# alisher-turubayev/dl-normalizing-flows

Hardware: AMD Instinct MI355X
Metric: images/sec + bits/dim, RealNVP 64x64x3 training (higher is better)
Workload: dtype bf16; 1 GPU; config 1: RealNVP 64x64x3, res-blocks 4, base-dim 32, per-GPU batch 64, train step fwd+bwd+Adam; global_batch=64, image_size=64, res_blocks=4, base_dim=32, n_scales=5, parallelism=dp1, graph=True, side_stream=False

## Files before the change

dl-normalizing-flows_amd/csrc/conv.hip:

```cpp
#include <math.h>
#include <stdlib.h>

#include "common.h"
#include "conv_common.h"

#ifndef RNVP_SHARD_PX
#define RNVP_SHARD_PX 8192
#endif
extern "C" int rnvp_stat_shards(long long M) {
    long long s = M / RNVP_SHARD_PX;
    int r = 1;
    while (r < 32 && r * 2 <= s) r *= 2;
    return r;
}

namespace {

int conv_args_status(const rnvp_conv_args* a) {
    if (!a || !a->x || !a->w || !a->y) return RNVP_E_INVALID;
    if (a->variant < 0 || (a->variant > RNVP_VARIANT_DEEP && a->variant < RNVP_VARIANT_DEEP0) ||
        a->variant >= RNVP_VARIANT_DEEP0 + RNVP_DEEP_CFGS)
        return RNVP_E_INVALID;
    if (a->w_frag && !al16(a->w_frag)) return RNVP_E_INVALID;
    if (a->dtype != RNVP_F32 && a->dtype != RNVP_BF16) return RNVP_E_INVALID;
    if (a->ks != 1 && a->ks != 3) return RNVP_E_UNSUPPORTED;
    if (a->B < 0 || a->H <= 0 || a->W <= 0 || a->n <= 0 || a->cin <= 0) return RNVP_E_INVALID;
    if ((a->cs_in & 7) || (a->cs_out & 7) || a->cs_in < a->cin || a->cs_out < a->n) return RNVP_E_INVALID;
    if ((a->kp & 63) || a->kp < a->ks * a->ks * a->cs_in) return RNVP_E_INVALID;
    if (!al16(a->x) || !al16(a->w)) return RNVP_E_INVALID;
    if (a->epi_relu_bn_bwd && !a->epi_x) return RNVP_E_INVALID;
    auto tab_bad = [](const rnvp_bn_src& s) { return s.tab && (!s.sums || !al16(s.tab)); };
    if ((a->pro_bn_relu && tab_bad(a->pro)) || (a->epi_relu_bn_bwd && tab_bad(a->epi)) || (a->bp && tab_bad(a->bp_bn)))
        return RNVP_E_INVALID;
    if ((long long)a->B * a->H * a->W >= (1ll << 31)) return RNVP_E_UNSUPPORTED;
    if (a->bp) {
        if (!a->bp_x || !al16(a->bp_x) || (a->bp_out && !al16(a->bp_out))) return RNVP_E_INVALID;
        if (a->bp_bn.sums && (!a->bp_sums || a->bp_shards < 1 || a->bp_bn.count <= 0)) return RNVP_E_INVALID;
        if (!a->bp_bn.sums && (!a->bp_bn.mean || !a->bp_bn.var)) return RNVP_E_INVALID;
        if (a->pro_bn_relu) return RNVP_E_INVALID;
    }
    return RNVP_OK;
}

int bp_cfg_of(const rnvp_conv_args* a) {
    if (a->variant >= RNVP_VARIANT_DEEP0) {
        const int cfg = a->variant - RNVP_VARIANT_DEEP0;
        return (cfg == 0 || cfg == 4) ? cfg : -1;
    }
    if (a->variant != 0 && a->variant != RNVP_VARIANT_DEEP) return -1;
    const int cfg = rnvp_deep_auto_cfg(a);
    const long long M = (long long)a->B * a->H * a->W;
    if (cfg == 4 || (cfg == 0 && (a->ks == 3 || M <= 4096))) return cfg;
    return -1;
}

int dispatch_conv(const rnvp_conv_args* a, hipStream_t s, bool dry, int* fam) {
    auto ran = [&](int f, int r) {
        if (fam && r == RNVP_OK) *fam = f;
        return r;
    };
    if (a->variant >= RNVP_VARIANT_DEEP0)
        return ran(RNVP_FAMILY_DEEP, rnvp_deep_launch(a, s, a->variant - RNVP_VARIANT_DEEP0, dry));
    if (a->variant == 0 || a->variant == RNVP_VARIANT_DEEP) {
        const int cfg = rnvp_deep_auto_cfg(a);
        if (cfg >= 0) {
            const int r = rnvp_deep_launch(a, s, cfg, dry);
            if (r != RNVP_E_UNSUPPORTED) return ran(RNVP_FAMILY_DEEP, r);
        }
    }
    const bool tuned = a->variant != 1;
    if (tuned && a->dtype == RNVP_BF16 && a->ks == 1) {
        const int r = rnvp_conv_s1_launch(a, s, dry);
        if (r != RNVP_E_UNSUPPORTED) return ran(RNVP_FAMILY_S1, r);
    }
    if (tuned && rnvp_conv_band_ok(a)) {
        const int r = rnvp_conv_band2_launch(a, s, dry);
        if (r != RNVP_E_UNSUPPORTED) return ran(RNVP_FAMILY_BAND, r);
        if (dry) return ran(RNVP_FAMILY_OTHER, RNVP_OK);
        return rnvp_conv_band1_launch(a, s);
    }
    if (dry) return ran(RNVP_FAMILY_OTHER, RNVP_OK);
    {
        const int r = rnvp_conv_stream_launch(a, s);
        if (r != RNVP_E_UNSUPPORTED) return r;
    }
    if (tuned) {
        const int r = rnvp_conv_halo_launch(a, s);
        if (r != RNVP_E_UNSUPPORTED) return r;
    }
    return rnvp_conv_tiled_launch(a, s);
}

int route_conv(const rnvp_conv_args* a, hipStream_t s, bool dry, int* fam = nullptr) {
    if (a->bp) {
        const int cfg = bp_cfg_of(a);
        int r, f = RNVP_FAMILY_DEEP;
        if (cfg >= 0) {
            r = rnvp_deep_launch(a, s, cfg, dry);
        } else {
            if (a->variant != 0) return RNVP_E_UNSUPPORTED;
            f = RNVP_FAMILY_S1;
            r = rnvp_conv_s1_launch(a, s, dry);
            if (r == RNVP_E_UNSUPPORTED) {
                f = RNVP_FAMILY_BAND;
                r = rnvp_conv_band2_launch(a, s, dry);
            }
        }
        if (fam && r == RNVP_OK) *fam = f;
        return r;
    }
    return dispatch_conv(a, s, dry, fam);
}

}

extern "C" int rnvp_conv2d(const rnvp_conv_args* a, void* stream) {
    const int st = conv_args_status(a);
    if (st != RNVP_OK || a->B == 0) return st;
    return route_conv(a, (hipStream_t)stream, false);
}

extern "C" int rnvp_conv2d_family(const rnvp_conv_args* a) {
    const int st = conv_args_status(a);
    if (st != RNVP_OK) return st;
    int fam = RNVP_FAMILY_OTHER;
    const int r = route_conv(a, nullptr, true, &fam);
    return r == RNVP_OK ? fam : r;
}

extern "C" int rnvp_conv2d_check(const rnvp_conv_args* a) {
    const int st = conv_args_status(a);
    if (st != RNVP_OK || a->B == 0) return st;
    return route_conv(a, nullptr, true);
}
```

dl-normalizing-flows_amd/csrc/conv_band1.hip:

```cpp
#include <math.h>
#include <stdlib.h>

#include "common.h"
#include "conv_common.h"

namespace {

template <typename T>
size_t band_lds_bytes(int cs, int n, int W, int ks) {
    constexpr int CH = Mf<T>::CH, KS = 4 * CH, BM = 256;
    const int nc = n <= 16 ? 16 : (n <= 32 ? 32 : 64);
    const int K = ks * ks * cs;
    const int kpl = lds_mfma_pitch(((K + KS - 1) / KS) * KS, CH);
    const int R = BM + 2 * (ks / 2) * (W + 1);
    const int ntmp = cs > nc ? cs : nc;
    return 16 * (size_t)ntmp + 8 * (size_t)cs + 20 * (size_t)nc + 64 * (size_t)nc +
           ((size_t)nc * kpl + (size_t)(R + 1) * lds_mfma_pitch(cs, CH)) * sizeof(T);
}

template <typename T, int NT, int KSZ, bool PRO, int NH>
__global__ __launch_bounds__(256 * NH) void k_conv_band(rnvp_conv_args a, int shards) {
    constexpr int CH = Mf<T>::CH, KS = 4 * CH;
    constexpr int NC = 16 * NT;
    constexpr int TM = 4, BM = 64 * TM;
    constexpr int PAD = KSZ / 2;
    constexpr int SB = 12 / NH;
    constexpr int NTH = 256 * NH, NTW = NT / NH;
    static_assert(NT % NH == 0, "channel tiles split evenly");
    extern __shared__ double dsm[];
    const int tid = threadIdx.x, lane = tid & 63, g = lane >> 4, li = lane & 15;
    const int wid = (tid >> 6) & 3, hf = tid >> 8;
    const int M = a.B * a.H * a.W, W = a.W, H = a.H;
    const int N = a.n, cs = a.cs_in;
    const int K = KSZ * KSZ * cs;
    const int nsteps = (K + KS - 1) / KS;
    const int kpl = lds_mfma_pitch(nsteps * KS, CH);
    const bool epi_bn = a.epi_relu_bn_bwd != 0;
    const int ntmp = cs > NC ? cs : NC;
    const int hal = PAD * (W + 1), R = BM + 2 * hal;
    const int pitch = lds_mfma_pitch(cs, CH);

    double* tmp = dsm;
    float* bnp = (float*)(dsm + 2 * ntmp);
    float* etab = bnp + 2 * cs;
    float* btab = etab + 4 * NC;
    double* red = (double*)(btab + NC);
    T* Wl = (T*)(red + 8 * NC);
    T* zrow = Wl + NC * kpl;
    T* act = zrow + pitch;

    const int nb = gridDim.x, b = blockIdx.x;
    const int q8 = nb / 8, r8 = nb % 8, xcd = b % 8;
    const int m0 = ((xcd < r8 ? xcd * (q8 + 1) : r8 * (q8 + 1) + (xcd - r8) * q8) + b / 8) * BM;

    const T* __restrict__ X = (const T*)a.x;
    const int cpr = cs / CH;
    const int cfix = tid % cpr, rbase = tid / cpr, rstep = NTH / cpr;
    u32x4 sv[SB];
    auto stage_load = [&](int r0) {
#pragma unroll
        for (int u = 0; u < SB; ++u) {
            if (r0 + u * rstep >= R) break;
            const int r = r0 + rbase + u * rstep;
            const int p = m0 - hal + r;
            const bool ok = (r < R) & (p >= 0) & (p < M);
            sv[u] = *(const u32x4*)(X + (ok ? (long long)p * cs + cfix * CH : 0));
        }
    };
    float scv[CH], shv[CH];
    auto stage_store = [&](int r0) {
#pragma unroll
        for (int u = 0; u < SB; ++u) {
            const int r = r0 + rbase + u * rstep;
            if (r >= R) continue;
            const int p = m0 - hal + r;
            u32x4 w = sv[u];
            if (PRO) {
                if constexpr (sizeof(T) == 2) {
                    w = bn_relu_bf16x8(w, scv, shv);
                } else {
                    float f[CH];
                    unpack(w, f, T());
#pragma unroll
                    for (int e = 0; e < CH; ++e) f[e] = fmaxf(f[e] * scv[e] + shv[e], 0.f);
                    w = pack(f, T());
                }
            }
            const uint32_t keep = (p >= 0 && p < M) ? ~0u : 0u;
            *(u32x4*)(act + r * pitch + cfix * CH) = w & u32x4{keep, keep, keep, keep};
        }
    };
    stage_load(0);

    if (PRO) block_bn_table(a.pro, a.cin, 0, cs, bnp, bnp + cs, nullptr, nullptr, tmp);
    if (epi_bn) block_bn_table(a.epi, N, 0, NC, etab, etab + NC, etab + 2 * NC, etab + 3 * NC, tmp);
    {
        const T* Wg = (const T*)a.w;
        const int wcpr = kpl / CH, wtot = NC * wcpr, kv = nsteps * KS;
        const float rw = 1.0f / (float)wcpr;
        for (int q0 = 0; q0 < wtot; q0 += 4 * NTH) {
            u32x4 v[4];
            unsigned okm = 0;
#pragma unroll
            for (int u = 0; u < 4; ++u) {
                const int q = q0 + u * NTH + tid;
                const int r = fdiv_small(q, rw), c = q - r * wcpr;
                const bool ok = (q < wtot) & (r < N) & (c * CH < kv);
                v[u] = *(const u32x4*)(Wg + (ok ? (long long)r * a.kp + c * CH : 0));
                okm |= (unsigned)ok << u;
            }
#pragma unroll
            for (int u = 0; u < 4; ++u) {
                const int q = q0 + u * NTH + tid;
                if (q < wtot) {
                    const int r = fdiv_small(q, rw), c = q - r * wcpr;
                    const uint32_t keep = ((okm >> u) & 1u) ? ~0u : 0u;
                    *(u32x4*)(Wl + r * kpl + c * CH) = v[u] & u32x4{keep, keep, keep, keep};
                }
            }
        }
        for (int n = tid; n < NC; n += NTH) btab[n] = (a.bias && n < N) ? a.bias[n] : 0.f;
        for (int c = tid * CH; c < pitch; c += NTH * CH) *(u32x4*)(zrow + c) = u32x4{0u, 0u, 0u, 0u};
    }
    __syncthreads();
    if (PRO) {
#pragma unroll
        for (int e = 0; e < CH; ++e) {
            scv[e] = bnp[cfix * CH + e];
            shv[e] = bnp[cs + cfix * CH + e];
        }
    }

    stage_store(0);
    for (int r0 = rstep * SB; r0 < R; r0 += rstep * SB) {
        stage_load(r0);
        stage_store(r0);
    }
    __syncthreads();

    int rowoff[TM];
    unsigned tvm[TM];
    const float rW = 1.0f / (float)W, rH = 1.0f / (float)H;
#pragma unroll
    for (int i = 0; i < TM; ++i) {
        const int lp = wid * 64 + i * 16 + li, m = m0 + lp;
        rowoff[i] = (lp + hal) * pitch;
        const int mm = m < M ? m : 0;
        const int row = fdiv_small(mm, rW);
        const int x = mm - row * W, y = row - fdiv_small(row, rH) * H;
        tvm[i] = tap_mask<KSZ>(x, y, W, H, m < M);
    }

    floatx4 acc[TM][NTW];
#pragma unroll
    for (int i = 0; i < TM; ++i)
#pragma unroll
        for (int j = 0; j < NTW; ++j) acc[i][j] = floatx4{0.f, 0.f, 0.f, 0.f};

    int tap = 0, ci = g * CH;
#pragma unroll
    for (int w = 0; w < 4; ++w)
        if (ci >= cs) { ci -= cs; ++tap; }
    const T* wl = Wl + (hf * NTW * 16 + li) * kpl + g * CH;
    for (int st = 0; st < nsteps; ++st) {
        const int ty = tap / KSZ;
        const int toff = ((ty - PAD) * W + (tap - ty * KSZ - PAD)) * pitch + ci;
        const int tsh = tap < KSZ * KSZ ? tap : 31;
        u32x4 wv[NTW], av[TM];
#pragma unroll
        for (int j = 0; j < NTW; ++j) wv[j] = *(const u32x4*)(wl + j * 16 * kpl + st * KS);
#pragma unroll
        for (int i = 0; i < TM; ++i) {
            const bool ok = (tvm[i] >> tsh) & 1u;
            av[i] = *(const u32x4*)(ok ? act + rowoff[i] + toff : zrow);
        }
#pragma unroll
        for (int i = 0; i < TM; ++i)
#pragma unroll
            for (int j = 0; j < NTW; ++j) Mf<T>::step(wv[j], av[i], acc[i][j]);
        ci += KS;
#pragma unroll
        for (int w = 0; w < 4; ++w)
            if (ci >= cs) { ci -= cs; ++tap; }
    }

    const int cso = a.cs_out;
    double s1[NTW][4], s2[NTW][4];
#pragma unroll
    for (int j = 0; j < NTW; ++j)
#pragma unroll
        for (int r = 0; r < 4; ++r) s1[j][r] = s2[j][r] = 0.0;
#pragma unroll
    for (int i = 0; i < TM; ++i) {
        const int m = m0 + wid * 64 + i * 16 + li;
        if (m >= M) continue;
#pragma unroll
        for (int j = 0; j < NTW; ++j) {
            const int n0 = (hf * NTW + j) * 16 + 4 * g;
            if (n0 >= cso) continue;
            epi4<T>(a, (long long)m * cso + n0, acc[i][j], btab + n0, epi_bn, etab + n0, NC, s1[j], s2[j], N - n0);
        }
    }
    const bool want_sums = a.out_sums || (epi_bn && a.epi_sums);
    if (want_sums) {
#pragma unroll
        for (int j = 0; j < NTW; ++j)
#pragma unroll
            for (int r = 0; r < 4; ++r) {
                const double u1 = row_sum16(s1[j][r]), u2 = row_sum16(s2[j][r]);
                const int col = (hf * NTW + j) * 16 + 4 * g + r;
                if (li == 0) {
                    red[(wid * NC + col) * 2] = u1;
                    red[(wid * NC + col) * 2 + 1] = u2;
                }
            }
        __syncthreads();
        double* sums = shard_ptr(epi_bn ? a.epi_sums : a.out_sums, shards, N);
        for (int n = tid; n < N; n += NTH) {
            double t1 = 0.0, t2 = 0.0;
#pragma unroll
            for (int w = 0; w < 4; ++w) {
                t1 += red[(w * NC + n) * 2];
                t2 += red[(w * NC + n) * 2 + 1];
            }
            atomicAdd(&sums[n], t1);
            atomicAdd(&sums[N + n], t2);
        }
    }
}

template <typename T, int NT, int KSZ>
int launch_band(const rnvp_conv_args* a, hipStream_t s) {
    const long long M = (long long)a->B * a->H * a->W;
    const unsigned grid = (unsigned)((M + 255) / 256);
    const size_t shm = band_lds_bytes<T>(a->cs_in, a->n, a->W, KSZ);
    const int sh = rnvp_stat_shards(M);
    if constexpr ((NT == 4 || NT == 2) && KSZ == 3) {
        if (a->pro_bn_relu) k_conv_band<T, NT, KSZ, true, 2><<<grid, 512, shm, s>>>(*a, sh);
        else k_conv_band<T, NT, KSZ, false, 2><<<grid, 512, shm, s>>>(*a, sh);
    } else {
        if (a->pro_bn_relu) k_conv_band<T, NT, KSZ, true, 1><<<grid, 256, shm, s>>>(*a, sh);
        else k_conv_band<T, NT, KSZ, false, 1><<<grid, 256, shm, s>>>(*a, sh);
    }
    RNVP_LAUNCH_CHECK();
    return RNVP_OK;
}

template <typename T>
bool band_ok(const rnvp_conv_args* a) {
    const long long M = (long long)a->B * a->H * a->W;
    if (a->n > 64 || a->cs_in > 64 || a->ks != 3) return false;
    if (256 % (a->cs_in / Mf<T>::CH) != 0) return false;
    if (M < 32768 || M >= (1ll << 21)) return false;
    return band_lds_bytes<T>(a->cs_in, a->n, a->W, a->ks) <= 150 * 1024;
}

template <typename T>
int dispatch_band(const rnvp_conv_args* a, hipStream_t s) {
    if (a->n <= 16) return launch_band<T, 1, 3>(a, s);
    if (a->n <= 32) return launch_band<T, 2, 3>(a, s);
    return launch_band<T, 4, 3>(a, s);
}

}

bool rnvp_conv_band_ok(const rnvp_conv_args* a) {
    return a->dtype == RNVP_F32 ? band_ok<float>(a) : band_ok<bf16_t>(a);
}

int rnvp_conv_band1_launch(const rnvp_conv_args* a, hipStream_t s) {
    if (!rnvp_conv_band_ok(a)) return RNVP_E_UNSUPPORTED;
    return a->dtype == RNVP_F32 ? dispatch_band<float>(a, s) : dispatch_band<bf16_t>(a, s);
}
```

dl-normalizing-flows_amd/csrc/conv_common.h:

```cpp
#pragma once
#include <math.h>

#include "common.h"

namespace {

template <typename T> struct Mf;
template <> struct Mf<bf16_t> {
    static constexpr int CH = 8;
    __device__ static __forceinline__ void step(const u32x4& a, const u32x4& b, floatx4& c) {
        c = __builtin_amdgcn_mfma_f32_16x16x32_bf16(__builtin_bit_cast(bf16x8, a), __builtin_bit_cast(bf16x8, b), c, 0, 0, 0);
    }
};
template <> struct Mf<float> {
    static constexpr int CH = 4;
    __device__ static __forceinline__ void step(const u32x4& a, const u32x4& b, floatx4& c) {
        c = __builtin_amdgcn_mfma_f32_16x16x4f32(__uint_as_float(a.x), __uint_as_float(b.x), c, 0, 0, 0);
        c = __builtin_amdgcn_mfma_f32_16x16x4f32(__uint_as_float(a.y), __uint_as_float(b.y), c, 0, 0, 0);
        c = __builtin_amdgcn_mfma_f32_16x16x4f32(__uint_as_float(a.z), __uint_as_float(b.z), c, 0, 0, 0);
        c = __builtin_amdgcn_mfma_f32_16x16x4f32(__uint_as_float(a.w), __uint_as_float(b.w), c, 0, 0, 0);
    }
};

__device__ __forceinline__ int sw8(int row, int c) { return row * 8 + (c ^ ((row >> 1) & 7)); }

__device__ __forceinline__ double* shard_ptr(double* sums, int shards, int N) {
    return sums ? sums + (long long)(blockIdx.x % shards) * 2 * N : nullptr;
}

template <typename T>
__device__ __forceinline__ void epi4(const rnvp_conv_args& a, long long o, const floatx4& acc, const float* bias,
                                     bool epi_bn, const float* et, int pitch, double* s1, double* s2, int nvalid) {
    float v[4];
#pragma unroll
    for (int r = 0; r < 4; ++r) v[r] = acc[r] + bias[r];
    if (a.residual) {
        float t[4];
        ld4((const T*)a.residual + o, t);
#pragma unroll
        for (int r = 0; r < 4; ++r) v[r] += t[r];
    }
    if (a.accumulate) {
        float t[4];
        ld4((const T*)a.y + o, t);
#pragma unroll
        for (int r = 0; r < 4; ++r) v[r] += t[r];
    }
    if (epi_bn) {
        float xv[4];
        ld4((const T*)a.epi_x + o, xv);
#pragma unroll
        for (int r = 0; r < 4; ++r) {
            if (xv[r] * et[r] + et[pitch + r] <= 0.f) v[r] = 0.f;
            s1[r] += v[r];
            s2[r] += v[r] * (xv[r] - et[2 * pitch + r]) * et[3 * pitch + r];
        }
    } else {
#pragma unroll
        for (int r = 0; r < 4; ++r) {
            s1[r] += v[r];
            s2[r] += (double)v[r] * v[r];
        }
    }
#pragma unroll
    for (int r = 0; r < 4; ++r)
        if (r >= nvalid) v[r] = 0.f;
    st4((T*)a.y + o, v);
}

struct EpiPre {
    float r[4], y[4], x[4];
};

template <typename T>
__device__ __forceinline__ void epi_prefetch(const rnvp_conv_args& a, long long o, bool live, EpiPre& p) {
    const long long oo = live ? o : 0;
    if (a.residual) ld4((const T*)a.residual + oo, p.r);
    if (a.accumulate) ld4((const T*)a.y + oo, p.y);
    if (a.epi_relu_bn_bwd) ld4((const T*)a.epi_x + oo, p.x);
}

template <typename T>
__device__ __forceinline__ void epi4p(const rnvp_conv_args& a, long long o, const floatx4& acc, const float* bias,
                                      bool epi_bn, const float* et, int pitch, double* s1, double* s2, int nvalid,
                                      const EpiPre& p) {
    float v[4];
#pragma unroll
    for (int r = 0; r < 4; ++r) v[r] = acc[r] + bias[r];
    if (a.residual) {
#pragma unroll
        for (int r = 0; r < 4; ++r) v[r] += p.r[r];
    }
    if (a.accumulate) {
#pragma unroll
        for (int r = 0; r < 4; ++r) v[r] += p.y[r];
    }
    if (epi_bn) {
#pragma unroll
        for (int r = 0; r < 4; ++r) {
            if (p.x[r] * et[r] + et[pitch + r] <= 0.f) v[r] = 0.f;
            s1[r] += v[r];
            s2[r] += v[r] * (p.x[r] - et[2 * pitch + r]) * et[3 * pitch + r];
        }
    } else {
#pragma unroll
        for (int r = 0; r < 4; ++r) {
            s1[r] += v[r];
            s2[r] += (double)v[r] * v[r];
        }
    }
#pragma unroll
    for (int r = 0; r < 4; ++r)
        if (r >= nvalid) v[r] = 0.f;
    st4((T*)a.y + o, v);
}

template <int KSZ>
__device__ __forceinline__ unsigned tap_mask(int x, int y, int W, int H, bool valid) {
    static_assert(KSZ == 1 || KSZ == 3, "1x1 / 3x3");
    if constexpr (KSZ == 1) {
        return valid ? 1u : 0u;
    } else {
        const unsigned cb = (x > 0 ? 1u : 0u) | 2u | (x < W - 1 ? 4u : 0u);
        const unsigned mk = (y > 0 ? cb : 0u) | (cb << 3) | (y < H - 1 ? cb << 6 : 0u);
        return valid ? mk : 0u;
    }
}

typedef float f32x2_t __attribute__((ext_vector_type(2)));
typedef short i16x2_t __attribute__((ext_vector_type(2)));
typedef __bf16 bf16x2_t __attribute__((ext_vector_type(2)));
__device__ __forceinline__ u32x4 bn_relu_bf16x8(const u32x4& c, const float* sc, const float* sh) {
    const uint32_t w[4] = {c.x, c.y, c.z, c.w};
    uint32_t o[4];
#pragma unroll
    for (int i = 0; i < 4; ++i) {
        const f32x2_t x = {__uint_as_float(w[i] << 16), __uint_as_float(w[i] & 0xffff0000u)};
        const f32x2_t y = __builtin_elementwise_fma(x, f32x2_t{sc[2 * i], sc[2 * i + 1]}, f32x2_t{sh[2 * i], sh[2 * i + 1]});
        const uint32_t p = __builtin_bit_cast(uint32_t, __builtin_convertvector(y, bf16x2_t));
        o[i] = __builtin_bit_cast(uint32_t, __builtin_elementwise_max(__builtin_bit_cast(i16x2_t, p), i16x2_t{0, 0}));
    }
    return u32x4{o[0], o[1], o[2], o[3]};
}

__host__ __device__ constexpr int lds_mfma_pitch(int elems, int ch) {
    return (elems / ch + ((2 - elems / ch) & 3)) * ch;
}
template <typename T>
__host__ __device__ constexpr int halo_pitch(int cs) { return lds_mfma_pitch(cs, Mf<T>::CH); }


template <int CPT>
struct BnTab {
    double a1[CPT], a2[CPT], b1[CPT], b2[CPT];
    float gam[CPT], bet[CPT];
};

template <int CPT, int NT = 256>
__device__ __forceinline__ void tab_issue(const rnvp_bn_src& s, int C, int c0, int nc, BnTab<CPT>& t) {
#pragma unroll
    for (int j = 0; j < CPT; ++j) {
        const int c = threadIdx.x + NT * j;
        const int cc = (c < nc && c0 + c < C) ? c0 + c : 0;
        if (s.tab) {
            t.a1[j] = *(const double*)(s.tab + (long long)cc * 4);
            t.a2[j] = t.b1[j] = t.b2[j] = 0.0;
        } else if (s.sums) {
            t.a1[j] = s.sums[cc];
            t.a2[j] = s.sums[C + cc];
            if (s.shards > 1) {
                t.b1[j] = s.sums[2 * (long long)C + cc];
                t.b2[j] = s.sums[3 * (long long)C + cc];
            } else {
                t.b1[j] = t.b2[j] = 0.0;
            }
        } else {
            t.a1[j] = s.mean[cc];
            t.a2[j] = s.var[cc];
            t.b1[j] = t.b2[j] = 0.0;
// ... 127 lines not shown
                    if (var < 0) var = 0;
                } else {
                    mn = a.bn.mean[c];
                    var = a.bn.var[c];
                }
                rstd = (float)(1.0 / sqrt(var + (double)a.bn.eps));
                mean = (float)mn;
                coef = gam * rstd;
            }
            const double g1 = gs[c], g2 = gs[cs + c];
            if (a.bn.sums) {
                k1 = (float)(g1 / cnt);
                k2 = (float)(g2 / cnt);
            }
            if (blk == 0) {
                if (a.dbeta) a.dbeta[c] = (float)g1;
                if (a.dgamma) a.dgamma[c] = (float)g2;
            }
        }
        p[5 * c] = coef; p[5 * c + 1] = k1; p[5 * c + 2] = k2; p[5 * c + 3] = mean; p[5 * c + 4] = rstd;
    };
#pragma unroll
    for (int j = 0; j < 2; ++j) {
        const int c = threadIdx.x + j * blockDim.x;
        if (c < cs) entry(c, gpre[j], epre[j]);
    }
    for (int c = threadIdx.x + 2 * blockDim.x; c < cs; c += blockDim.x)
        entry(c, (GAM && c < C) ? a.bn.gamma[c] : 1.f, btab ? bn_tab_load(a.bn.tab, C, c, BN_TAB_DIV) : bn_f32x2{});
    __syncthreads();
    const bool fixed = qs % cpr == 0;
    int c0 = (int)(q0 % cpr) * CH;
    auto apply = [&](long long o, const u32x4& vg, const u32x4& vx, const u32x4& vr, const u32x4& vd) {
        float g[CH], x[CH], d[CH];
        unpack(vg, g, T());
        unpack(vx, x, T());
#pragma unroll
        for (int j = 0; j < CH; ++j) {
            const float* pp = p + 5 * (c0 + j);
            const float xh = (x[j] - pp[3]) * pp[4];
            d[j] = pp[0] * (g[j] - pp[1] - xh * pp[2]);
        }
        if (R) {
            float r[CH];
            unpack(vr, r, T());
#pragma unroll
            for (int j = 0; j < CH; ++j) d[j] += r[j];
        }
        if (a.accumulate) {
            float r[CH];
            unpack(vd, r, T());
#pragma unroll
            for (int j = 0; j < CH; ++j) d[j] += r[j];
        }
        *(u32x4*)(DX + o) = pack(d, T());
    };
    if (q0 < nch) apply(q0 * CH, fg, fx, fr, fd);
    for (long long q = q0 + qs; q < nch; q += qs) {
        const long long o = q * CH;
        if (!fixed) c0 = (int)(q % cpr) * CH;
        const u32x4 vg = *(const u32x4*)(G + o), vx = *(const u32x4*)(X + o);
        const u32x4 vr = R ? *(const u32x4*)(R + o) : vg;
        const u32x4 vd = a.accumulate ? *(const u32x4*)(DX + o) : vg;
        apply(o, vg, vx, vr, vd);
    }
}

template <typename T>
__device__ __forceinline__ void bn_bwd_body(const rnvp_bn_bwd_args& a, double* dsm, int blk, int nblk) {
    if (a.bn.gamma) bn_bwd_run<T, true>(a, dsm, blk, nblk);
    else bn_bwd_run<T, false>(a, dsm, blk, nblk);
}

inline bool al16(const void* p) { return (((uintptr_t)p) & 15) == 0; }

}

int rnvp_conv_tiled_launch(const rnvp_conv_args* a, hipStream_t s);

int rnvp_conv_stream_launch(const rnvp_conv_args* a, hipStream_t s);

int rnvp_conv_halo_launch(const rnvp_conv_args* a, hipStream_t s);

bool rnvp_conv_band_ok(const rnvp_conv_args* a);
int rnvp_conv_band1_launch(const rnvp_conv_args* a, hipStream_t s);

constexpr int RNVP_DEEP_CFGS = 7;
int rnvp_deep_launch(const rnvp_conv_args* a, hipStream_t s, int cfg, bool dry = false);
int rnvp_deep_auto_cfg(const rnvp_conv_args* a);

int rnvp_wgrad_tap_launch(rnvp_wgrad_group* g, hipStream_t s);
int rnvp_wgrad_tap_prepare(rnvp_wgrad_group* g);
int rnvp_wgrad_tap_multi_plan(const rnvp_wgrad_group* groups, int n_groups, int cls, rnvp_wgrad_multi_conv* convs,
                              int conv_cap, int* xcd_start, int* tasks, int task_cap, rnvp_wgrad_multi* m);
int rnvp_wgrad_tap_multi_launch(const rnvp_wgrad_multi* m, hipStream_t s);

int rnvp_conv_s1_launch(const rnvp_conv_args* a, hipStream_t s, bool dry = false);

struct rnvp_group_kargs {
    rnvp_conv_args conv[RNVP_NET_GROUP_MAX];
    int shards[RNVP_NET_GROUP_MAX], tiles[RNVP_NET_GROUP_MAX], xa[RNVP_NET_GROUP_MAX], xb[RNVP_NET_GROUP_MAX];
    int n;
};
rnvp_group_kargs group_kargs(const rnvp_net_step* steps, int n);

using GroupKernel = void (*)(const rnvp_group_kargs);
template <typename T, int CFG> int rnvp_deep_cfg_launch(const rnvp_conv_args* a, hipStream_t s, bool dry);
template <typename T, int CFG> GroupKernel rnvp_deep_cfg_group(int nc, bool fm);
int rnvp_s1_fanout_prepare(rnvp_net_step* steps, int n, int* klass, int* grid, int* lds_bytes);
int rnvp_s1_fanout_launch(const rnvp_group_kargs& g, int klass, int grid, int lds_bytes, hipStream_t s);

int rnvp_conv_band2_launch(const rnvp_conv_args* a, hipStream_t s, bool dry = false);
```

dl-normalizing-flows_amd/csrc/conv_deep.h:

```cpp
#pragma once
#include <stdlib.h>

#include "common.h"
#include "conv_common.h"

namespace {

constexpr int DEEP_BM = 64;

#ifdef RNVP_DEEP_STAMPS
__device__ unsigned long long* g_deep_stamps;
#define DEEP_STAMP(i) \
    do { if (threadIdx.x == 0) g_deep_stamps[blockIdx.x * 8 + (i)] = wall_clock64(); } while (0)
#else
#define DEEP_STAMP(i) do {} while (0)
#endif
constexpr int DEEP_MAX_CS = 1024;

template <typename T>
__host__ __device__ constexpr int deep_pitch(int cs) { return lds_mfma_pitch(cs, Mf<T>::CH); }

template <typename T, int BN, int NW, int WK, int BM = DEEP_BM>
size_t deep_lds_bytes(int cs, int W, int ks, bool bp = false) {
    constexpr int TM = BM / 16, WM = NW / WK;
    constexpr int G = WK > 1 ? TM : WM;
    const int hal = (ks / 2) * (W + 1), R = BM + 2 * hal;
    const size_t head = 4 * (5 * (size_t)BN) + 8 * (2 * (size_t)G * BN) + 4 * (bp ? 3 : 2) * (size_t)cs;
    const size_t zrow = (size_t)deep_pitch<T>(cs) * sizeof(T);
    size_t act = (size_t)R * deep_pitch<T>(cs) * sizeof(T);
    const size_t red = WK > 1 ? (size_t)WK * BM * (BN + 4) * 4 : 0;
    return head + zrow + (act > red ? act : red);
}

template <typename T, int BN, int KSZ, bool PRO, int NW, int WK, int DK, int NC, bool FM = false, int BM = DEEP_BM,
          bool BP = false>
__device__ __forceinline__ void deep_tile(const rnvp_conv_args& a, int shards, int xa, int xb, int vb, int nvb,
                                          char* lds) {
    constexpr int NT = 64 * NW;
    constexpr int CH = Mf<T>::CH, KS = 4 * CH;
    constexpr int TM = BM / 16, TN = BN / 16;
    constexpr int WM = NW / WK;
    constexpr int TMW = TM / WM;
    static_assert(WM * WK == NW && TMW * WM == TM, "wave layout");
    constexpr int PAD = KSZ / 2;
    constexpr int RP = BN + 4;
    constexpr int G = WK > 1 ? TM : WM;
    constexpr int FR = WK > 1 ? (TM * TN) / NW : 1;
    static_assert(WK == 1 || FR * NW == TM * TN, "final tiles");
    constexpr bool TALL = WK > 1 && TM > NW;
    static_assert(!TALL || TM % NW == 0, "row groups per wave");
    constexpr int CPT = (NC * WK * KS + NT - 1) / NT;
    static_assert(!(BP && PRO), "BatchNorm-backward prologue: data gradients only");
    constexpr int NSTEP = KSZ * KSZ * NC;
    const int tid = threadIdx.x, lane = tid & 63, g = lane >> 4, li = lane & 15;
    const int wid = __builtin_amdgcn_readfirstlane(tid >> 6);
    const int wk = wid % WK, wm = wid / WK;
    const int M = a.B * a.H * a.W, W = a.W, H = a.H;
    const int N = a.n, cs = a.cs_in;
    const int gm = (M + BM - 1) / BM;
    const int nb = nvb, b = vb;
    const int q8 = nb / 8, r8 = nb % 8, xcd = b % 8;
    const int t = (xcd < r8 ? xcd * (q8 + 1) : r8 * (q8 + 1) + (xcd - r8) * q8) + b / 8;
    int mt, nt;
    if (xa > 0) {
        const int per = xa * xb, bi = t / per, w = t - bi * per, gmb = gm / xa;
        const int bm = bi % gmb, bn = bi / gmb;
        mt = bm * xa + w % xa;
        nt = bn * xb + w / xa;
    } else if (xa == 0) {
        nt = t / gm;
        mt = t - nt * gm;
    } else {
        const int gn = nvb / gm;
        mt = t / gn;
        nt = t - mt * gn;
    }
    const int m0 = mt * BM, n0 = nt * BN;
    const T* __restrict__ X = (const T*)a.x;
    const T* __restrict__ Wt = (const T*)(FM ? a.w_frag : a.w);
    const bool epi_bn = a.epi_relu_bn_bwd != 0;
    static_assert(BN <= NT, "bias / table loads: one channel per thread");

    const int hal = PAD * (W + 1);
    const int R = BM + 2 * hal;
    const int pitch = deep_pitch<T>(cs);
    float* etab = (float*)lds;
    float* btab = etab + 4 * BN;
    double* sred = (double*)(btab + BN);
    float* bnp = (float*)(sred + G * BN * 2);
    T* zrow = (T*)(bnp + (BP ? 3 : 2) * cs);
    T* act = zrow + pitch;

    constexpr int CPR = NC * WK * 4;
    static_assert(NT % CPR == 0, "fixed chunk column per thread");
    constexpr int RSTEP = NT / CPR;
    constexpr int SBP = KSZ == 1 ? (BM + RSTEP - 1) / RSTEP : (BM + 2 * 17 + RSTEP - 1) / RSTEP;
    constexpr int SBC = NT == 256 ? 8 : 12;
    constexpr int SB = BP ? (SBP < SBC ? SBP : SBC) : 20 * 256 / NT;
    const int cfix = tid % CPR, rbase = tid / CPR;
    u32x4 sv[SB];
    u32x4 sx[BP ? SB : 1];
    const T* __restrict__ XT = (const T*)a.bp_x;
    auto stage_load = [&](int r0) {
#pragma unroll
        for (int u = 0; u < SB; ++u) {
            if (r0 + u * RSTEP >= R) break;
            const int r = r0 + rbase + u * RSTEP;
            const int p = m0 - hal + r;
            const bool ok = (r < R) & (p >= 0) & (p < M);
            const long long o = ok ? (long long)p * cs + cfix * CH : 0;
            sv[u] = *(const u32x4*)(X + o);
            if constexpr (BP) sx[u] = *(const u32x4*)(XT + o);
        }
    };
    float scv[CH], shv[CH];
    float bca[BP ? CH : 1], bcb[BP ? CH : 1], bcc[BP ? CH : 1];
    T* __restrict__ BPO = (T*)a.bp_out;
    const bool bp_store = BP && BPO != nullptr && nt == 0;
    auto stage_store = [&](int r0) {
#pragma unroll
        for (int u = 0; u < SB; ++u) {
            const int r = r0 + rbase + u * RSTEP;
            if (r >= R) continue;
            const int p = m0 - hal + r;
            u32x4 w = sv[u];
            if (PRO) {
                if constexpr (sizeof(T) == 2) {
                    w = bn_relu_bf16x8(w, scv, shv);
                } else {
                    float f[CH];
                    unpack(w, f, T());
#pragma unroll
                    for (int e = 0; e < CH; ++e) f[e] = fmaxf(f[e] * scv[e] + shv[e], 0.f);
                    w = pack(f, T());
                }
            }
            if constexpr (BP) {
                float gv[CH], xv[CH], d[CH];
                unpack(w, gv, T());
                unpack(sx[u], xv, T());
#pragma unroll
                for (int e = 0; e < CH; ++e) d[e] = fmaf(bca[e], gv[e], -fmaf(bcb[e], xv[e], bcc[e]));
                w = pack(d, T());
                if (bp_store && r >= hal && r < hal + BM && p < M)
                    *(u32x4*)(BPO + (long long)p * cs + cfix * CH) = w;
            }
            const uint32_t keep = (p >= 0 && p < M) ? ~0u : 0u;
            *(u32x4*)(act + r * pitch + cfix * CH) = w & u32x4{keep, keep, keep, keep};
        }
    };
    DEEP_STAMP(0);
    constexpr int NE = WK > 1 ? FR : TMW * TN;
    auto elem = [&](int e, int& m, int& col) {
        if constexpr (TALL) {
            m = m0 + (wid + NW * (e / TN)) * 16 + li;
            col = (e % TN) * 16 + 4 * g;
        } else if constexpr (WK > 1) {
            m = m0 + (wid % TM) * 16 + li;
            col = ((wid / TM) * FR + e) * 16 + 4 * g;
        } else {
            m = m0 + (wm * TMW + e / TN) * 16 + li;
            col = (e % TN) * 16 + 4 * g;
        }
    };
    const int cso = a.cs_out;
    BnTab<CPT> ptab;
    BnTab<1> etb;
    if (PRO) tab_issue<CPT, NT>(a.pro, a.cin, 0, cs, ptab);
    BnTab<BP ? CPT : 1> btb, gtb;
    rnvp_bn_src gsrc = {};
    if constexpr (BP) {
        gsrc.sums = a.bp_sums;
        gsrc.count = a.bp_bn.count;
        gsrc.shards = a.bp_shards;
        rnvp_bn_src bsrc = a.bp_bn;
        if (bsrc.tab) bsrc.tab += 2 * BN_TAB_DIV;
        tab_issue<CPT, NT>(bsrc, a.cin, 0, cs, btb);
        tab_issue<CPT, NT>(gsrc, a.cin, 0, cs, gtb);
    }
    if (epi_bn) tab_issue<1, NT>(a.epi, N, n0, BN, etb);
    const float bval = (tid < BN && a.bias && n0 + tid < N) ? a.bias[n0 + tid] : 0.f;
    EpiPre pre[NE];
#pragma unroll
    for (int e = 0; e < NE; ++e) {
        int m, col;
        elem(e, m, col);
        epi_prefetch<T>(a, (long long)m * cso + n0 + col, m < M && n0 + col < cso, pre[e]);
    }
    stage_load(0);
    const T* wrow[TN];
#pragma unroll
    for (int j = 0; j < TN; ++j) {
        if constexpr (FM) {
            static_assert(sizeof(T) == 2 && KS == 32, "fragment-major images are bf16");
            const int nb = (n0 >> 4) + j, nbl = (N + 15) >> 4;
            wrow[j] = Wt + (long long)(nb < nbl ? nb : 0) * (a.kp >> 5) * 512 + (li + 16 * g) * CH;
        } else {
            const int row = n0 + j * 16 + li;
            wrow[j] = Wt + (long long)(row < N ? row : 0) * a.kp + g * CH;
        }
    }
    u32x4 rb[DK][TN];
    auto bload = [&](int st) {
        const int tp = st / NC, ch = st - (st / NC) * NC;
        const int k = tp * cs + (ch * WK + wk) * KS;
#pragma unroll
        for (int j = 0; j < TN; ++j) rb[st % DK][j] = *(const u32x4*)(wrow[j] + (FM ? (k >> 5) * 512 : k));
    };
#pragma unroll
    for (int u = 0; u < DK; ++u)
        if (u < NSTEP) bload(u);
    if (PRO) tab_finish<CPT, NT>(a.pro, a.cin, 0, cs, ptab, bnp, bnp + cs, nullptr, nullptr);
    if constexpr (BP) {
#pragma unroll
        for (int j = 0; j < CPT; ++j) {
            const int c = tid + NT * j;
            if (c >= cs) continue;
            float coef = 0.f, k1 = 0.f, k2 = 0.f, mo = 0.f, ro = 1.f;
            if (c < a.cin) {
                if (a.bp_bn.tab) {
                    const unsigned long long u = (unsigned long long)__double_as_longlong(btb.a1[j]);
                    mo = __uint_as_float((unsigned)u);
                    ro = __uint_as_float((unsigned)(u >> 32));
                    coef = btb.gam[j] * ro;
                } else {
                    double mean, var;
                    if (a.bp_bn.sums) {
                        const double s1 = btb.a1[j] + (a.bp_bn.shards > 1 ? btb.b1[j] : 0.0);
                        const double s2 = btb.a2[j] + (a.bp_bn.shards > 1 ? btb.b2[j] : 0.0);
                        mean = s1 / a.bp_bn.count;
                        var = s2 / a.bp_bn.count - mean * mean;
                        if (var < 0) var = 0;
                    } else {
                        mean = btb.a1[j];
                        var = btb.a2[j];
                    }
                    ro = (float)(1.0 / sqrt(var + (double)a.bp_bn.eps));
                    mo = (float)mean;
                    coef = btb.gam[j] * ro;
                }
                const double g1 = gtb.a1[j] + (a.bp_shards > 1 ? gtb.b1[j] : 0.0);
                const double g2 = gtb.a2[j] + (a.bp_shards > 1 ? gtb.b2[j] : 0.0);
                if (a.bp_bn.sums) {
                    k1 = (float)(g1 / a.bp_bn.count);
                    k2 = (float)(g2 / a.bp_bn.count);
                }
                if (vb == 0) {
                    if (a.bp_dbeta) a.bp_dbeta[c] = (float)g1;
                    if (a.bp_dgamma) a.bp_dgamma[c] = (float)g2;
                }
            }
            const double rk2 = (double)ro * (double)k2;
            bnp[c] = coef;
            bnp[cs + c] = (float)((double)coef * rk2);
            bnp[2 * cs + c] = (float)((double)coef * ((double)k1 - rk2 * (double)mo));
        }
    }
    if (epi_bn) tab_finish<1, NT>(a.epi, N, n0, BN, etb, etab, etab + BN, etab + 2 * BN, etab + 3 * BN);
    if (tid < BN) btab[tid] = bval;
    for (int c = tid * CH; c < pitch; c += NT * CH) *(u32x4*)(zrow + c) = u32x4{0u, 0u, 0u, 0u};
    __syncthreads();
    DEEP_STAMP(1);
    if (PRO) {
#pragma unroll
        for (int e = 0; e < CH; ++e) {
            scv[e] = bnp[cfix * CH + e];
            shv[e] = bnp[cs + cfix * CH + e];
        }
    }
    if constexpr (BP) {
#pragma unroll
        for (int e = 0; e < CH; ++e) {
            bca[e] = bnp[cfix * CH + e];
            bcb[e] = bnp[cs + cfix * CH + e];
            bcc[e] = bnp[2 * cs + cfix * CH + e];
        }
    }

    stage_store(0);
    for (int r0 = RSTEP * SB; r0 < R; r0 += RSTEP * SB) {
        stage_load(r0);
        stage_store(r0);
    }
    __syncthreads();
    DEEP_STAMP(2);

    int rowoff[TMW];
    unsigned tvm[TMW];
    const float rW = 1.0f / (float)W, rH = 1.0f / (float)H;
#pragma unroll
    for (int i = 0; i < TMW; ++i) {
        const int lp = (wm * TMW + i) * 16 + li, m = m0 + lp;
        rowoff[i] = (lp + hal) * pitch + g * CH;
        const int mm = m < M ? m : 0;
        const int row = fdiv_small(mm, rW);
        const int x = mm - row * W, y = row - fdiv_small(row, rH) * H;
        tvm[i] = tap_mask<KSZ>(x, y, W, H, m < M);
    }
    floatx4 acc[TMW][TN];
#pragma unroll
    for (int i = 0; i < TMW; ++i)
#pragma unroll
        for (int j = 0; j < TN; ++j) acc[i][j] = floatx4{0.f, 0.f, 0.f, 0.f};

    constexpr bool DBUF = KSZ == 1 || (NW == 4 ? (BN == 32 || NC <= 4) : (BN == 32 ? NC <= 2 : NC == 1));
    auto aload = [&](int st, u32x4* dst) {
        const int tp = st / NC, ch = st - (st / NC) * NC;
        const int toff = ((tp / KSZ - PAD) * W + (tp % KSZ - PAD)) * pitch + wk * KS + ch * WK * KS;
#pragma unroll
        for (int i = 0; i < TMW; ++i)
            dst[i] = *(const u32x4*)(((tvm[i] >> tp) & 1u) ? act + rowoff[i] + toff : zrow + ch * WK * KS);
    };
    if constexpr (DBUF) {
        u32x4 avb[2][TMW];
        aload(0, avb[0]);
#pragma unroll
        for (int st = 0; st < NSTEP; ++st) {
            if (st + 1 < NSTEP) aload(st + 1, avb[(st + 1) & 1]);
            __builtin_amdgcn_sched_barrier(0);
#pragma unroll
            for (int i = 0; i < TMW; ++i)
#pragma unroll
                for (int j = 0; j < TN; ++j) Mf<T>::step(rb[st % DK][j], avb[st & 1][i], acc[i][j]);
            if (st + DK < NSTEP) bload(st + DK);
            __builtin_amdgcn_sched_barrier(0);
        }
    } else {
#pragma unroll
        for (int st = 0; st < NSTEP; ++st) {
            u32x4 av[TMW];
            aload(st, av);
#pragma unroll
            for (int i = 0; i < TMW; ++i)
#pragma unroll
                for (int j = 0; j < TN; ++j) Mf<T>::step(rb[st % DK][j], av[i], acc[i][j]);
            if (st + DK < NSTEP) bload(st + DK);
        }
    }

    DEEP_STAMP(3);
    const bool want_sums = a.out_sums || (epi_bn && a.epi_sums);
    constexpr int NS = (WK > 1 && !TALL) ? FR : TN;
    double s1[NS][4], s2[NS][4];
#pragma unroll
    for (int f = 0; f < NS; ++f)
#pragma unroll
        for (int r = 0; r < 4; ++r) s1[f][r] = s2[f][r] = 0.0;
    const int grp = TALL ? wid : (WK > 1 ? wid % TM : wm);
    constexpr int GU = TALL ? NW : G;
    if constexpr (WK > 1) {
        float* red = (float*)act;
        __syncthreads();
#pragma unroll
        for (int i = 0; i < TMW; ++i)
#pragma unroll
            for (int j = 0; j < TN; ++j)
                *(floatx4*)&red[(wk * BM + (wm * TMW + i) * 16 + li) * RP + j * 16 + 4 * g] = acc[i][j];
        __syncthreads();
        const int fi = wid % TM;
#pragma unroll
        for (int f = 0; f < FR; ++f) {
            int m, col;
            elem(f, m, col);
            const int n = n0 + col;
            if (m >= M || n >= cso) continue;
            const int ri = TALL ? wid + NW * (f / TN) : fi;
            const int sl = TALL ? f % TN : f;
            floatx4 v = *(const floatx4*)&red[(ri * 16 + li) * RP + col];
#pragma unroll
            for (int w = 1; w < WK; ++w) v += *(const floatx4*)&red[(w * BM + ri * 16 + li) * RP + col];
            epi4p<T>(a, (long long)m * cso + n, v, btab + col, epi_bn, etab + col, BN, s1[sl], s2[sl], N - n, pre[f]);
        }
    } else {
#pragma unroll
        for (int e = 0; e < NE; ++e) {
            int m, col;
            elem(e, m, col);
            const int n = n0 + col;
            if (m >= M || n >= cso) continue;
            epi4p<T>(a, (long long)m * cso + n, acc[e / TN][e % TN], btab + col, epi_bn, etab + col, BN, s1[e % TN],
                     s2[e % TN], N - n, pre[e]);
        }
    }
    DEEP_STAMP(4);
    if (want_sums) {
#pragma unroll
        for (int f = 0; f < NS; ++f)
#pragma unroll
            for (int r = 0; r < 4; ++r) {
                const double u1 = row_sum16(s1[f][r]), u2 = row_sum16(s2[f][r]);
                if (li == 0) {
                    const int cb = ((WK > 1 && !TALL) ? ((wid / TM) * FR + f) : f) * 16 + 4 * g;
                    sred[(grp * BN + cb + r) * 2] = u1;
                    sred[(grp * BN + cb + r) * 2 + 1] = u2;
                }
            }
        __syncthreads();
        double* sums = (epi_bn ? a.epi_sums : a.out_sums) + (long long)(vb % shards) * 2 * N;
        for (int col = tid; col < BN; col += NT) {
            const int n = n0 + col;
            if (n >= N) continue;
            double t1 = 0.0, t2 = 0.0;
#pragma unroll
            for (int q = 0; q < GU; ++q) {
                t1 += sred[(q * BN + col) * 2];
                t2 += sred[(q * BN + col) * 2 + 1];
            }
            atomicAdd(&sums[n], t1);
            atomicAdd(&sums[N + n], t2);
        }
    }
    DEEP_STAMP(5);
}

inline void xcd_blocks(const rnvp_conv_args* a, int gm, int gn, int bn, int esz, int* xa, int* xb, int bm = DEEP_BM) {
    *xa = -1;
    *xb = 1;
    const long long per = (long long)gm * gn / 8;
    const int hal = (a->ks / 2) * (a->W + 1);
    const double act = (double)(bm + 2 * hal) * a->cs_in * esz;
    const double wsl = (double)bn * a->ks * a->ks * a->cs_in * esz;
    double best = 1e300;
    for (int x = 1; x <= gm; ++x) {
        if (gm % x || per % x) continue;
        const long long y = per / x;
        if (y < 1 || gn % y) continue;
        const double bytes = x * act + y * wsl;
        if (bytes < best) { best = bytes; *xa = x; *xb = (int)y; }
    }
}

}
```

dl-normalizing-flows_amd/csrc/conv_deep_launch.h:

```cpp
#pragma once
#include "conv_deep.h"

namespace {

template <typename T, int BN, int KSZ, bool PRO, int NW, int WK, int DK, int NC, bool FM = false, int BM = DEEP_BM,
          bool BP = false>
__global__ __launch_bounds__(64 * NW) void k_conv_deep(rnvp_conv_args a, int shards, int xa, int xb) {
    extern __shared__ __attribute__((aligned(16))) char lds[];
    deep_tile<T, BN, KSZ, PRO, NW, WK, DK, NC, FM, BM, BP>(a, shards, xa, xb, blockIdx.x, gridDim.x, lds);
}

template <int BN, int NW, int WK, int BM>
constexpr bool bp_cfg() { return BN == 32 && WK == NW && BM == DEEP_BM; }

template <typename T, int BN, int NW, int WK, int DK, int NC, int KSZ, int BM = DEEP_BM>
int launch_deep_nc(const rnvp_conv_args* a, hipStream_t s, bool dry) {
    const long long M = (long long)a->B * a->H * a->W;
    const size_t shm = deep_lds_bytes<T, BN, NW, WK, BM>(a->cs_in, a->W, a->ks, a->bp != 0);
    if (shm > 160 * 1024) return RNVP_E_UNSUPPORTED;
    const long long gm = (M + BM - 1) / BM, gn = (a->n + BN - 1) / BN;
    const unsigned grid = (unsigned)(gm * gn);
    const int sh = rnvp_stat_shards(M);
    const dim3 blk(64 * NW);
    int xa, xb;
    xcd_blocks(a, (int)gm, (int)gn, BN, sizeof(T), &xa, &xb, BM);
    if (a->bp) {
        if constexpr (bp_cfg<BN, NW, WK, BM>()) {
            if (dry) return RNVP_OK;
            if constexpr (sizeof(T) == 2 && NC <= 4) {
                if (a->w_frag) {
                    k_conv_deep<T, BN, KSZ, false, NW, WK, DK, NC, true, BM, true><<<grid, blk, shm, s>>>(*a, sh, xa, xb);
                    RNVP_LAUNCH_CHECK();
                    return RNVP_OK;
                }
            }
            k_conv_deep<T, BN, KSZ, false, NW, WK, DK, NC, false, BM, true><<<grid, blk, shm, s>>>(*a, sh, xa, xb);
            RNVP_LAUNCH_CHECK();
            return RNVP_OK;
        } else {
            return RNVP_E_UNSUPPORTED;
        }
    }
    if (dry) return RNVP_OK;
    if constexpr (sizeof(T) == 2 && NC <= 4) {
        if (a->w_frag) {
            if (a->pro_bn_relu) k_conv_deep<T, BN, KSZ, true, NW, WK, DK, NC, true, BM><<<grid, blk, shm, s>>>(*a, sh, xa, xb);
            else k_conv_deep<T, BN, KSZ, false, NW, WK, DK, NC, true, BM><<<grid, blk, shm, s>>>(*a, sh, xa, xb);
            RNVP_LAUNCH_CHECK();
            return RNVP_OK;
        }
    }
    if (a->pro_bn_relu) k_conv_deep<T, BN, KSZ, true, NW, WK, DK, NC, false, BM><<<grid, blk, shm, s>>>(*a, sh, xa, xb);
    else k_conv_deep<T, BN, KSZ, false, NW, WK, DK, NC, false, BM><<<grid, blk, shm, s>>>(*a, sh, xa, xb);
    RNVP_LAUNCH_CHECK();
    return RNVP_OK;
}

template <typename T, int BN, int NW, int WK, int DK>
int launch_deep(const rnvp_conv_args* a, hipStream_t s, bool dry) {
    constexpr int KS = 4 * Mf<T>::CH;
    const long long M = (long long)a->B * a->H * a->W;
    if (M > 65536 || a->n < BN / 2 || a->cs_in % (WK * KS)) return RNVP_E_UNSUPPORTED;
    if (a->pro_bn_relu && a->pro.sums && a->pro.shards > 2) return RNVP_E_UNSUPPORTED;
    if (a->epi_relu_bn_bwd && a->epi.sums && a->epi.shards > 2) return RNVP_E_UNSUPPORTED;
    if (a->cs_in > DEEP_MAX_CS) return RNVP_E_UNSUPPORTED;
    if (a->bp && (a->pro_bn_relu || (a->bp_bn.sums && a->bp_bn.shards > 2) || a->bp_shards > 2)) return RNVP_E_UNSUPPORTED;
    const int nc = a->cs_in / (WK * KS);
    if (a->ks == 1) {
        switch (nc) {
            case 1: return launch_deep_nc<T, BN, NW, WK, DK, 1, 1>(a, s, dry);
            case 2: return launch_deep_nc<T, BN, NW, WK, DK, 2, 1>(a, s, dry);
            case 4: return launch_deep_nc<T, BN, NW, WK, DK, 4, 1>(a, s, dry);
            case 8: return launch_deep_nc<T, BN, NW, WK, DK, 8, 1>(a, s, dry);
            case 16: return launch_deep_nc<T, BN, NW, WK, DK, 16, 1>(a, s, dry);
        }
        return RNVP_E_UNSUPPORTED;
    }
    if constexpr (WK == NW) {
        switch (nc) {
            case 1: return launch_deep_nc<T, BN, NW, WK, DK, 1, 3>(a, s, dry);
            case 2: return launch_deep_nc<T, BN, NW, WK, DK, 2, 3>(a, s, dry);
            case 4: return launch_deep_nc<T, BN, NW, WK, DK, 4, 3>(a, s, dry);
            case 8: return launch_deep_nc<T, BN, NW, WK, DK, 8, 3>(a, s, dry);
        }
    }
    return RNVP_E_UNSUPPORTED;
}

template <typename T, int BN, int NW, int WK, int DK>
int launch_deep_tall(const rnvp_conv_args* a, hipStream_t s, bool dry) {
    constexpr int KS = 4 * Mf<T>::CH;
    if constexpr (sizeof(T) != 2) {
        return RNVP_E_UNSUPPORTED;
    } else {
        const long long M = (long long)a->B * a->H * a->W;
        if (a->ks != 3 || M > 65536 || a->n < BN / 2 || a->cs_in % (WK * KS)) return RNVP_E_UNSUPPORTED;
        if (a->pro_bn_relu && a->pro.sums && a->pro.shards > 2) return RNVP_E_UNSUPPORTED;
        if (a->epi_relu_bn_bwd && a->epi.sums && a->epi.shards > 2) return RNVP_E_UNSUPPORTED;
        switch (a->cs_in / (WK * KS)) {
            case 1: return launch_deep_nc<T, BN, NW, WK, DK, 1, 3, 128>(a, s, dry);
            case 2: return launch_deep_nc<T, BN, NW, WK, DK, 2, 3, 128>(a, s, dry);
            case 4: return launch_deep_nc<T, BN, NW, WK, DK, 4, 3, 128>(a, s, dry);
        }
        return RNVP_E_UNSUPPORTED;
    }
}

template <typename T, int BN, int NW, int WK, int DK, int NC, bool FM = false>
// ... 59 lines not shown
```

dl-normalizing-flows_amd/csrc/coupling.hip:

```cpp
#include "coupling_common.h"

namespace {

__global__ __launch_bounds__(256) void k_in_stats(rnvp_coupling_args a, int TP, int seg) {
    extern __shared__ double red[];
    const Geo g = geo(a);
    const Tile t = tile_of(g, TP);
    const int lane = threadIdx.x & 63;
    const int total = g.Cb * t.tp;
    auto xidx = [&](int e) {
        const int cb = e / t.tp, p = t.p0 + (e - cb * t.tp);
        const int c = (g.kind == 0) ? cb : g.off_base + cb;
        return ((long long)t.b * g.C + c) * g.HW + p;
    };
    float xp[CP_K];
#pragma unroll
    for (int k = 0; k < CP_K; ++k) {
        const int e = k * 256 + threadIdx.x;
        { const float v = a.x[xidx(e < total ? e : 0)]; xp[k] = e < total ? v : 0.f; }
    }
    lds_zero(red, 2 * g.Cb);
    __syncthreads();
    auto body = [&](int e0, float xv) {
        const int e = e0 + threadIdx.x;
// ... 441 lines not shown
#pragma unroll
    for (int k = 0; k < CP_K; ++k) {
        const int e = k * 256 + threadIdx.x;
        const long long idx = eidx(e < total ? e : 0);
        gzp[k] = a.gz[idx];
        up[k] = a.u[idx];
        xp[k] = a.x[idx];
        glp[k] = gl_ld(glo, idx, t.b);
    }
    for (int cb = threadIdx.x; cb < g.Cb; cb += blockDim.x) {
        float fm = 0.f, rstd = 1.f, kA = 0.f, kB = 0.f;
        if (a.coupling_bn) {
            out_bn_stats(a, g, cb, fm, rstd);
            if (a.training) {
                kA = (float)(csum(a.bwd_sums, 3 * g.Cb, cb) / cnt);
                kB = (float)((csum(a.bwd_sums, 3 * g.Cb, g.Cb + cb) + csum(a.bwd_sums, 3 * g.Cb, 2 * g.Cb + cb)) / cnt);
            }
        }
        tab[cb] = fm; tab[g.Cb + cb] = rstd; tab[2 * g.Cb + cb] = kA; tab[3 * g.Cb + cb] = kB;
    }
    tile_copy_in<T>(a.st, t.m0, t.tp, a.cs_st, st);
    for (int e = threadIdx.x; e < t.tp * a.cs_gst; e += blockDim.x) stv(&gs[e], 0.f);
    __syncthreads();
    const float sc = a.scale[0], ss = a.scale_shift[0];
    double gsc = 0.0, gss = 0.0;
    auto body = [&](int e, float gz, float uv, float xv, float glv) {
        const int c = e / t.tp, pl = e - c * t.tp, p = t.p0 + pl;
        const long long idx = ((long long)t.b * g.C + c) * g.HW + p;
        const bool chan_on = g.kind == 1 && c >= g.on_base && c < g.on_base + g.Cb;
        const int cb = g.kind == 0 ? c : c - g.on_base;
        const bool has_bn_chan = g.kind == 0 || chan_on;
        const bool tr = g.kind == 0 ? !ckbd_m(g, p) : chan_on;
        float gu;
        if (!a.coupling_bn || !has_bn_chan) {
            gu = gz;
        } else {
            const float fm = tab[cb], rstd = tab[g.Cb + cb], kA = tab[2 * g.Cb + cb], kB = tab[3 * g.Cb + cb];
            if (!tr) {
                gu = gz;
                if (a.training) gu += rstd * (-kA - (uv - fm) * rstd * kB);
            } else {
                gu = rstd * gz;
                if (a.training) gu = rstd * (gz - kA - (uv - fm) * rstd * kB);
            }
        }
        if (tr) {
            const float r = ldv(&st[pl * a.cs_st + g.Cb + cb]);
            const float th = tanhf(r);
            const float ex = expf(sc * th + ss);
            a.gx[idx] = gu * ex;
            const float glr = gu * xv * ex + glv;
            stv(&gs[pl * a.cs_gst + cb], gu);
            stv(&gs[pl * a.cs_gst + g.Cb + cb], glr * sc * (1.f - th * th));
            gsc += (double)glr * th;
            gss += glr;
        } else {
            a.gx[idx] = gu;
        }
    };
#pragma unroll
    for (int k = 0; k < CP_K; ++k) {
        const int e = k * 256 + threadIdx.x;
        if (e < total) body(e, gzp[k], up[k], xp[k], glp[k]);
    }
    for (int e = CP_K * 256 + threadIdx.x; e < total; e += 256) {
        const long long idx = eidx(e);
        body(e, a.gz[idx], a.u[idx], a.x[idx], gl_ld(glo, idx, t.b));
    }
    const float dsc = (float)block_sum(gsc, redl);
    const float dss = (float)block_sum(gss, redl);
    tile_copy_out<T>(gs, t.m0, t.tp, a.cs_gst, a.gst);
    if (threadIdx.x == 0 && (dsc != 0.f || dss != 0.f)) {
        if (a.gscale_part) {
            double* sp = a.gscale_part + 2 * (blockIdx.x % RNVP_COUPLING_SHARDS);
            atomicAdd(sp, (double)dsc);
            atomicAdd(sp + 1, (double)dss);
        } else {
            atomicAdd(a.g_scale, dsc);
            atomicAdd(a.g_scale_shift, dss);
        }
    }
}

__device__ __forceinline__ void fold_gscale(const rnvp_coupling_args& a) {
    const int l = threadIdx.x;
    double v0 = 0.0, v1 = 0.0;
    if (l < RNVP_COUPLING_SHARDS) {
        v0 = a.gscale_part[2 * l];
        v1 = a.gscale_part[2 * l + 1];
        a.gscale_part[2 * l] = 0.0;
        a.gscale_part[2 * l + 1] = 0.0;
    }
    v0 = wave_sum(v0);
    v1 = wave_sum(v1);
    if (l == 0) {
        *a.g_scale += (float)v0;
        *a.g_scale_shift += (float)v1;
    }
}

template <typename T>
__device__ __forceinline__ void in_bwd_vals(const rnvp_coupling_args& a, const Geo& g, const Tile& t, const T* gh,
                                            const float* tab, int cb, int pl, float v, float& gxa, float& xh) {
    const int p = t.p0 + pl;
    if (g.kind == 0 && !ckbd_m(g, p)) v = 0.f;
    const float xa = v * tab[cb] + tab[g.Cb + cb];
    const float g1 = ldv(&gh[pl * a.cs_gh0 + cb]);
    const float g2 = ldv(&gh[pl * a.cs_gh0 + g.Cb + cb]);
    gxa = (xa > 0.f ? g1 : 0.f) - (xa < 0.f ? g2 : 0.f);
    xh = (v - tab[2 * g.Cb + cb]) * tab[3 * g.Cb + cb];
}

template <typename T>
__global__ __launch_bounds__(256) void k_in_bwd_red(rnvp_coupling_args a, int TP, int seg) {
    extern __shared__ double dsm[];
    const Geo g = geo(a);
    const Tile t = tile_of(g, TP);
    const int lane = threadIdx.x & 63;
    const bool ext = a.in_bwd_ext != nullptr;
    double* red = dsm;
    float* tab = (float*)(dsm + (ext ? 4 : 2) * g.Cb);
    T* gh = (T*)(tab + 4 * ((g.Cb + 3) / 4 * 4));
    const int total = g.Cb * t.tp;
    auto xidx = [&](int e) {
        const int cb = e / t.tp, p = t.p0 + (e - cb * t.tp);
        const int c = (g.kind == 0) ? cb : g.off_base + cb;
        return ((long long)t.b * g.C + c) * g.HW + p;
    };
    float xp[CP_K];
#pragma unroll
    for (int k = 0; k < CP_K; ++k) {
        const int e = k * 256 + threadIdx.x;
        { const float v = a.x[xidx(e < total ? e : 0)]; xp[k] = e < total ? v : 0.f; }
    }
    tile_copy_in<T>(a.gh0, t.m0, t.tp, a.cs_gh0, gh);
    lds_zero(red, (ext ? 4 : 2) * g.Cb);
    if (a.training && a.in_tab) {
        for (int i = threadIdx.x; i < 4 * g.Cb; i += blockDim.x) tab[i] = a.in_tab[i];
    } else {
        in_bn_table(a, g, tab);
    }
    if (blockIdx.x == 0 && a.gscale_part && threadIdx.x < 64) fold_gscale(a);
    __syncthreads();
    auto body = [&](int e0, float xv) {
        const int e = e0 + threadIdx.x;
        const bool ok = e < total;
        const int cb = ok ? e / t.tp : 0, pl = ok ? e - cb * t.tp : 0;
        float gxa = 0.f, xh = 0.f;
        if (ok) in_bwd_vals<T>(a, g, t, gh, tab, cb, pl, xv, gxa, xh);
        const double s1 = seg_red((double)gxa, seg), s2 = seg_red((double)gxa * xh, seg);
        if (ok && (lane & seg_mask(seg)) == 0) {
            atomicAdd(&red[cb], s1);
            atomicAdd(&red[g.Cb + cb], s2);
        }
        if (ext) {
            const bool kept = ok && (g.kind != 0 || ckbd_m(g, t.p0 + pl));
            const double e1 = seg_red(kept ? (double)gxa : 0.0, seg), e2 = seg_red(kept ? (double)gxa * xv : 0.0, seg);
            if (ok && (lane & seg_mask(seg)) == 0) {
                atomicAdd(&red[2 * g.Cb + cb], e1);
                atomicAdd(&red[3 * g.Cb + cb], e2);
            }
        }
    };
#pragma unroll
    for (int k = 0; k < CP_K; ++k)
        if (k * 256 < total) body(k * 256, xp[k]);
    for (int e0 = CP_K * 256; e0 < total; e0 += 256) {
        const int e = e0 + threadIdx.x;
        { const float v = a.x[xidx(e < total ? e : 0)]; body(e0, e < total ? v : 0.f); }
    }
    __syncthreads();
    double* dst = cshard(a.in_bwd_sums, 2 * g.Cb);
    for (int c = threadIdx.x; c < 2 * g.Cb; c += blockDim.x) atomicAdd(&dst[c], red[c]);
    if (ext) {
        double* dx = cshard(a.in_bwd_ext, 2 * g.Cb);
        for (int c = threadIdx.x; c < 2 * g.Cb; c += blockDim.x) atomicAdd(&dx[c], red[2 * g.Cb + c]);
    }
}

template <typename T>
__global__ __launch_bounds__(256) void k_in_bwd_apply(rnvp_coupling_args a, int TP, int seg) {
    extern __shared__ double dsm[];
    const Geo g = geo(a);
    const Tile t = tile_of(g, TP);
    float* tab = (float*)dsm;
    const int tabn = 8 * ((g.Cb + 3) / 4 * 4);
    T* gh = (T*)(tab + tabn);
    const int total = g.Cb * t.tp;
    auto xidx = [&](int e) {
        const int cb = e / t.tp, p = t.p0 + (e - cb * t.tp);
        const int c = (g.kind == 0) ? cb : g.off_base + cb;
        return ((long long)t.b * g.C + c) * g.HW + p;
    };
    float xp[CP_K], gxp[CP_K];
#pragma unroll
    for (int k = 0; k < CP_K; ++k) {
        const int e = k * 256 + threadIdx.x;
        const long long idx = xidx(e < total ? e : 0);
        xp[k] = a.x[idx];
        gxp[k] = a.gx[idx];
    }
    in_bn_table(a, g, tab);
    const double cnt = (double)g.B * g.HW;
    for (int cb = threadIdx.x; cb < g.Cb; cb += blockDim.x) {
        const float gam = a.in_gamma ? a.in_gamma[cb] : 1.f;
        tab[4 * g.Cb + cb] = gam * tab[3 * g.Cb + cb];
        const double s1 = a.in_bwd_sums ? csum(a.in_bwd_sums, 2 * g.Cb, cb) : 0.0;
        const double s2 = a.in_bwd_sums ? csum(a.in_bwd_sums, 2 * g.Cb, g.Cb + cb) : 0.0;
        tab[5 * g.Cb + cb] = a.training ? (float)(s1 / cnt) : 0.f;
        tab[6 * g.Cb + cb] = a.training ? (float)(s2 / cnt) : 0.f;
        if (blockIdx.x == 0) {
            if (a.g_in_beta) a.g_in_beta[cb] = (float)s1;
            if (a.g_in_gamma) a.g_in_gamma[cb] = (float)s2;
        }
    }
    if (blockIdx.x == 0 && a.gscale_part && threadIdx.x < 64) fold_gscale(a);
    tile_copy_in<T>(a.gh0, t.m0, t.tp, a.cs_gh0, gh);
    __syncthreads();
    auto body = [&](int e, float xv, float gxv) {
        const int cb = e / t.tp, pl = e - cb * t.tp, p = t.p0 + pl;
        const int c = (g.kind == 0) ? cb : g.off_base + cb;
        const long long idx = ((long long)t.b * g.C + c) * g.HW + p;
        float gxa, xh;
        in_bwd_vals<T>(a, g, t, gh, tab, cb, pl, xv, gxa, xh);
        float gxm = tab[4 * g.Cb + cb] * (gxa - tab[5 * g.Cb + cb] - xh * tab[6 * g.Cb + cb]);
        if (g.kind == 0 && !ckbd_m(g, p)) gxm = 0.f;
        a.gx[idx] = gxv + gxm;
    };
#pragma unroll
    for (int k = 0; k < CP_K; ++k) {
        const int e = k * 256 + threadIdx.x;
        if (e < total) body(e, xp[k], gxp[k]);
    }
    for (int e = CP_K * 256 + threadIdx.x; e < total; e += 256) {
        const long long idx = xidx(e);
        body(e, a.x[idx], a.gx[idx]);
    }
}

int check(const rnvp_coupling_args* a) {
    if (!a || !a->x || a->B < 0 || a->C <= 0 || a->H <= 0 || a->W <= 0) return RNVP_E_INVALID;
    if (a->kind != 0 && a->kind != 1) return RNVP_E_INVALID;
    if (a->kind == 1 && (a->C & 1)) return RNVP_E_INVALID;
    if (a->dtype != RNVP_F32 && a->dtype != RNVP_BF16) return RNVP_E_INVALID;
    return RNVP_OK;
}

inline int cb_of(const rnvp_coupling_args* a) { return a->kind == 0 ? a->C : a->C / 2; }

struct TileCfg {
    int TP, seg, grid;
};
inline TileCfg tile_cfg(const rnvp_coupling_args* a) {
    const int HW = a->H * a->W;
    const int esz = a->dtype == RNVP_F32 ? 4 : 2;
    int cs = a->cs_h0;
    if (a->cs_st + a->cs_gst > cs) cs = a->cs_st + a->cs_gst;
    if (a->cs_gh0 > cs) cs = a->cs_gh0;
    if (cs < 8) cs = 8;
    TileCfg c;
    c.TP = HW < 256 ? HW : 256;
    while (c.TP > 16 && (long long)c.TP * cs * esz > 32 * 1024) c.TP /= 2;
    while (c.TP > 4 && c.TP % 2 == 0 && (long long)a->B * ((HW + c.TP - 1) / c.TP) < 512) c.TP /= 2;
    int seg = 1;
    while (seg < 64 && c.TP % (2 * seg) == 0 && HW % (2 * seg) == 0) seg *= 2;
    c.seg = seg;
    c.grid = a->B * ((HW + c.TP - 1) / c.TP);
    return c;
}
}

extern "C" int rnvp_coupling_in_fwd(const rnvp_coupling_args* a, void* stream) {
    int st = check(a);
    if (st) return st;
    if (!a->h0 || (a->training && !a->in_sums) || (!a->training && (!a->in_rmean || !a->in_rvar))) return RNVP_E_INVALID;
    const int Cb = cb_of(a);
    if (a->cs_h0 < (a->kind == 0 ? 2 * Cb + 1 : 2 * Cb)) return RNVP_E_INVALID;
    if (a->B == 0) return RNVP_OK;
    hipStream_t s = (hipStream_t)stream;
    const TileCfg tc = tile_cfg(a);
    const int esz = a->dtype == RNVP_F32 ? 4 : 2;
    if (a->training) {
        k_in_stats<<<tc.grid, 256, 16 * Cb, s>>>(*a, tc.TP, tc.seg);
        RNVP_LAUNCH_CHECK();
    }
    const size_t shm = 16 * r4(Cb) + (size_t)tc.TP * a->cs_h0 * esz;
    if (a->dtype == RNVP_F32) k_in_apply<float><<<tc.grid, 256, shm, s>>>(*a, tc.TP, tc.seg);
    else k_in_apply<bf16_t><<<tc.grid, 256, shm, s>>>(*a, tc.TP, tc.seg);
    RNVP_LAUNCH_CHECK();
    return RNVP_OK;
}

extern "C" int rnvp_coupling_in_apply(const rnvp_coupling_args* a, void* stream) {
    int st = check(a);
    if (st) return st;
    if (!a->h0 || (a->training && !a->in_sums) || (!a->training && (!a->in_rmean || !a->in_rvar))) return RNVP_E_INVALID;
    const int Cb = cb_of(a);
    if (a->cs_h0 < (a->kind == 0 ? 2 * Cb + 1 : 2 * Cb)) return RNVP_E_INVALID;
    if (a->B == 0) return RNVP_OK;
// ... 12 lines not shown
    if (st) return st;
    if (!a->st || !a->u || !a->z || !a->ldj_sample || !a->scale || !a->scale_shift) return RNVP_E_INVALID;
    if (a->coupling_bn && ((a->training && !a->out_sums) || (!a->training && (!a->out_rmean || !a->out_rvar))))
        return RNVP_E_INVALID;
    const int Cb = cb_of(a);
    if (a->cs_st < 2 * Cb) return RNVP_E_INVALID;
    if (a->B == 0) return RNVP_OK;
    hipStream_t s = (hipStream_t)stream;
    const TileCfg tc = tile_cfg(a);
    const int esz = a->dtype == RNVP_F32 ? 4 : 2;
    const size_t shm1 = 16 * ((Cb + 1) / 2 * 2) + (size_t)tc.TP * a->cs_st * esz;
    if (a->dtype == RNVP_F32) k_out1<float><<<tc.grid, 256, shm1, s>>>(*a, tc.TP, tc.seg);
    else k_out1<bf16_t><<<tc.grid, 256, shm1, s>>>(*a, tc.TP, tc.seg);
    RNVP_LAUNCH_CHECK();
    long long n = (long long)a->B * a->C * a->H * a->W;
    size_t shm = 3 * Cb * sizeof(float);
    const int nrun = (a->training && a->net_running) ? a->n_net_running : 0;
    if (nrun < 0 || (nrun > 0 && a->net_running_cmax <= 0)) return RNVP_E_INVALID;
    if (nrun > 0 && 16 * (size_t)a->net_running_cmax > shm) shm = 16 * (size_t)a->net_running_cmax;
    const int g2 = rnvp_grid(n, 256, 2048);
    if (a->dtype == RNVP_F32) k_out2<float><<<g2 + nrun, 256, shm, s>>>(*a, g2);
    else k_out2<bf16_t><<<g2 + nrun, 256, shm, s>>>(*a, g2);
    RNVP_LAUNCH_CHECK();
    return RNVP_OK;
}

extern "C" int rnvp_coupling_reverse(const rnvp_coupling_args* a, void* stream) {
    int st = check(a);
    if (st) return st;
    if (!a->st || !a->z || !a->scale || !a->scale_shift) return RNVP_E_INVALID;
    if (a->coupling_bn && (!a->out_rmean || !a->out_rvar)) return RNVP_E_INVALID;
    if (a->cs_st < 2 * cb_of(a)) return RNVP_E_INVALID;
    if (a->B == 0) return RNVP_OK;
    long long n = (long long)a->B * a->C * a->H * a->W;
    hipStream_t s = (hipStream_t)stream;
    if (a->dtype == RNVP_F32) k_reverse<float><<<rnvp_grid(n, 256, 2048), 256, 0, s>>>(*a);
    else k_reverse<bf16_t><<<rnvp_grid(n, 256, 2048), 256, 0, s>>>(*a);
    RNVP_LAUNCH_CHECK();
    return RNVP_OK;
}

extern "C" int rnvp_coupling_reverse_bwd(const rnvp_coupling_args* a, void* stream) {
    int st = check(a);
    if (st) return st;
    if (!a->st || !a->gz || !a->gx || !a->gst || !a->gscale_part || !a->scale || !a->scale_shift) return RNVP_E_INVALID;
    const int Cb = cb_of(a);
    if (a->cs_gst < 2 * Cb || a->cs_st < 2 * Cb) return RNVP_E_INVALID;
    if (a->coupling_bn && (!a->out_rmean || !a->out_rvar)) return RNVP_E_INVALID;
    if (a->B == 0) return RNVP_OK;
    const TileCfg tc = tile_cfg(a);
    const int esz = a->dtype == RNVP_F32 ? 4 : 2;
    const size_t shm = (size_t)tc.TP * (a->cs_st + a->cs_gst) * esz;
    hipStream_t s = (hipStream_t)stream;
    if (a->dtype == RNVP_F32) k_reverse_bwd<float><<<tc.grid, 256, shm, s>>>(*a, tc.TP);
    else k_reverse_bwd<bf16_t><<<tc.grid, 256, shm, s>>>(*a, tc.TP);
    RNVP_LAUNCH_CHECK();
    return RNVP_OK;
}

extern "C" int rnvp_coupling_out_bwd(const rnvp_coupling_args* a, void* stream) {
    int st = check(a);
    if (st) return st;
    if (!a->st || !a->u || !a->gz || !a->gx || !a->gst || !a->g_scale || !a->g_scale_shift) return RNVP_E_INVALID;
    const int Cb = cb_of(a);
    if (a->cs_gst < 2 * Cb || a->cs_st < 2 * Cb) return RNVP_E_INVALID;
    const bool stats = a->coupling_bn && a->training;
    if (stats && (!a->out_sums || !a->bwd_sums)) return RNVP_E_INVALID;
    if (a->coupling_bn && !a->training && (!a->out_rmean || !a->out_rvar)) return RNVP_E_INVALID;
    if (a->B == 0) return RNVP_OK;
    hipStream_t s = (hipStream_t)stream;
    const TileCfg tc = tile_cfg(a);
    const int esz = a->dtype == RNVP_F32 ? 4 : 2;
    if (stats) {
        k_out_bwd_red<<<tc.grid, 256, 24 * Cb + 8 * Cb, s>>>(*a, tc.TP, tc.seg);
        RNVP_LAUNCH_CHECK();
    }
    const size_t shm = 16 * r4(Cb) + (size_t)tc.TP * (a->cs_st + a->cs_gst) * esz;
    if (a->dtype == RNVP_F32) k_out_bwd_apply<float><<<tc.grid, 256, shm, s>>>(*a, tc.TP, tc.seg);
    else k_out_bwd_apply<bf16_t><<<tc.grid, 256, shm, s>>>(*a, tc.TP, tc.seg);
    RNVP_LAUNCH_CHECK();
    return RNVP_OK;
}

extern "C" int rnvp_coupling_in_bwd(const rnvp_coupling_args* a, void* stream) {
    int st = check(a);
    if (st) return st;
    if (!a->gh0 || (!a->gx && !(a->in_bwd_ext && a->training))) return RNVP_E_INVALID;
    if (a->training && (!a->in_sums || !a->in_bwd_sums)) return RNVP_E_INVALID;
    if (!a->training && (!a->in_rmean || !a->in_rvar)) return RNVP_E_INVALID;
    const int Cb = cb_of(a);
    if (a->cs_gh0 < 2 * Cb) return RNVP_E_INVALID;
    if (a->B == 0) return RNVP_OK;
    hipStream_t s = (hipStream_t)stream;
    const TileCfg tc = tile_cfg(a);
    const int esz = a->dtype == RNVP_F32 ? 4 : 2;
    const size_t gsh = (size_t)tc.TP * a->cs_gh0 * esz;
    if (a->training || a->g_in_gamma || a->g_in_beta) {
        if (!a->in_bwd_sums) return RNVP_E_INVALID;
        const size_t shm = (a->in_bwd_ext ? 32 : 16) * Cb + 16 * r4(Cb) + gsh;
        if (a->dtype == RNVP_F32) k_in_bwd_red<float><<<tc.grid, 256, shm, s>>>(*a, tc.TP, tc.seg);
        else k_in_bwd_red<bf16_t><<<tc.grid, 256, shm, s>>>(*a, tc.TP, tc.seg);
        RNVP_LAUNCH_CHECK();
    }
    if (!a->gx) return RNVP_OK;
    const size_t shm = 32 * r4(Cb) + gsh;
    if (a->dtype == RNVP_F32) k_in_bwd_apply<float><<<tc.grid, 256, shm, s>>>(*a, tc.TP, tc.seg);
    else k_in_bwd_apply<bf16_t><<<tc.grid, 256, shm, s>>>(*a, tc.TP, tc.seg);
    RNVP_LAUNCH_CHECK();
    return RNVP_OK;
}
```

dl-normalizing-flows_amd/csrc/coupling_common.h:

```cpp
#pragma once
#include <math.h>

#include "common.h"

namespace {

struct Geo {
    int kind, B, C, H, W, HW, Cb, cfg, on_base, off_base;
};

__device__ __forceinline__ Geo geo(const rnvp_coupling_args& a) {
    Geo g;
    g.kind = a.kind; g.B = a.B; g.C = a.C; g.H = a.H; g.W = a.W; g.HW = a.H * a.W;
    g.cfg = a.mask_config ? 1 : 0;
    if (a.kind == 0) {
        g.Cb = a.C; g.on_base = 0; g.off_base = 0;
    } else {
        g.Cb = a.C / 2;
        g.on_base = g.cfg ? 0 : g.Cb;
        g.off_base = g.cfg ? g.Cb : 0;
    }
    return g;
}

// ... 35 lines not shown
    return v;
}

__device__ __forceinline__ double seg_red(double v, int seg) { return seg >= 16 ? row_sum16(v) : seg_sum(v, seg); }
__device__ __forceinline__ int seg_mask(int seg) { return seg >= 16 ? 15 : seg - 1; }

template <typename T>
__device__ __forceinline__ void tile_copy_in(const void* src, long long m0, int tp, int cs, T* lds) {
    const int n16 = tp * cs * (int)sizeof(T) / 16;
    const u32x4* s = (const u32x4*)((const T*)src + m0 * cs);
    u32x4* d = (u32x4*)lds;
    for (int i = threadIdx.x; i < n16; i += blockDim.x) d[i] = s[i];
}

template <typename T>
__device__ __forceinline__ void tile_copy_out(const T* lds, long long m0, int tp, int cs, void* dst) {
    const int n16 = tp * cs * (int)sizeof(T) / 16;
    const u32x4* s = (const u32x4*)lds;
    u32x4* d = (u32x4*)((T*)dst + m0 * cs);
    for (int i = threadIdx.x; i < n16; i += blockDim.x) d[i] = s[i];
}

template <int R>
struct TileRegs {
    u32x4 v[R];
    int n16;
};
template <typename T, int R>
__device__ __forceinline__ void tile_issue(const void* src, long long m0, int tp, int cs, TileRegs<R>& r) {
    r.n16 = tp * cs * (int)sizeof(T) / 16;
    const u32x4* s = (const u32x4*)((const T*)src + m0 * cs);
#pragma unroll
    for (int k = 0; k < R; ++k) {
        const int i = (int)threadIdx.x + k * (int)blockDim.x;
        r.v[k] = s[i < r.n16 ? i : 0];
    }
}
template <typename T, int R>
__device__ __forceinline__ void tile_commit(const TileRegs<R>& r, const void* src, long long m0, int cs, T* lds) {
    u32x4* d = (u32x4*)lds;
#pragma unroll
    for (int k = 0; k < R; ++k) {
        const int i = (int)threadIdx.x + k * (int)blockDim.x;
        if (i < r.n16) d[i] = r.v[k];
    }
    const u32x4* s = (const u32x4*)((const T*)src + m0 * cs);
    for (int i = (int)threadIdx.x + R * (int)blockDim.x; i < r.n16; i += blockDim.x) d[i] = s[i];
}

__device__ __forceinline__ void lds_zero(double* p, int n) {
    for (int i = threadIdx.x; i < n; i += blockDim.x) p[i] = 0.0;
}

__device__ __forceinline__ double* cshard(double* sums, int width) {
    return sums + (long long)(blockIdx.x % RNVP_COUPLING_SHARDS) * width;
}
__device__ __forceinline__ double csum(const double* sums, int width, int i) {
    double v[RNVP_COUPLING_SHARDS];
#pragma unroll
    for (int h = 0; h < RNVP_COUPLING_SHARDS; ++h) v[h] = sums[(long long)h * width + i];
    double t = 0.0;
#pragma unroll
    for (int h = 0; h < RNVP_COUPLING_SHARDS; ++h) t += v[h];
    return t;
}

__device__ __forceinline__ void in_bn_table(const rnvp_coupling_args& a, const Geo& g, float* t) {
    for (int cb = threadIdx.x; cb < g.Cb; cb += blockDim.x) {
        rnvp_bn_src s;
        s.shards = RNVP_COUPLING_SHARDS;
        s.sums = a.training ? a.in_sums : nullptr;
        s.count = (double)g.B * g.HW;
        s.mean = a.in_rmean; s.var = a.in_rvar;
        s.gamma = a.in_gamma; s.beta = a.in_beta; s.eps = a.eps;
        float sc, sf, mean, rstd;
        bn_affine(s, g.Cb, cb, sc, sf, &mean, &rstd);
        t[cb] = sc;
        t[g.Cb + cb] = sf;
        t[2 * g.Cb + cb] = mean;
        t[3 * g.Cb + cb] = rstd;
    }
}

__device__ __forceinline__ float coupling_u(float x, float sh, float r, float sc, float ss, float& lr, float& th,
                                            float& ex) {
    th = tanhf(r);
    lr = fmaf(sc, th, ss);
    ex = expf(lr);
    return fmaf(x, ex, sh);
}

__host__ __device__ inline int r4(int x) { return (x + 3) / 4 * 4; }

}
```

dl-normalizing-flows_amd/csrc/coupling_link.hip:

```cpp
#include "coupling_common.h"

#ifdef RNVP_LINK_STAMPS
__device__ unsigned long long* g_link_stamps;
#define LINK_STAMP(i) \
    do { if (threadIdx.x == 0) g_link_stamps[blockIdx.x * 8 + (i)] = wall_clock64(); } while (0)
#else
#define LINK_STAMP(i) do {} while (0)
#endif

namespace {

constexpr float LOG_SQRT_2PI = 0.91893853320467274178f;

__device__ __forceinline__ int pcls(int nc, const Geo& g, int p) {
    if (nc == 1) return 0;
    const int i = p / g.W, j = p - i * g.W;
    return nc == 2 ? ((i + j) & 1) : ((i & 1) * 2 + (j & 1));
}

__device__ __forceinline__ double cls_count(int nc, const Geo& g, int q) {
    const long long H = g.H, W = g.W;
    if (nc == 1) return (double)(H * W);
    if (nc == 2) {
        const long long even = ((H & 1) && (W & 1)) ? (H * W + 1) / 2 : H * W / 2;
// ... 438 lines not shown
    double* red = isn + 2 * Cbn;
    float* ta = (float*)(red + 4 * ga.C);
    float* tn = ta + 4 * Cra;
    T* sta = (T*)(tn + 6 * Crn);
    T* gs = sta + TP * a.cs_st;
    T* gh = gs + TP * a.cs_gst;
    const int pn0 = LT == RNVP_LINK_SQUEEZE ? t.p0 / 4 : t.p0;
    const int tpn = LT == RNVP_LINK_SQUEEZE ? t.tp / 4 : t.tp;
    const int csg = TO_N ? n.cs_gh0 : 0;
    const int total = ga.C * t.tp;
    const double cnt_a = (double)ga.B * ga.HW, cnt_n = (double)gn.B * gn.HW;
    auto aidx = [&](int e) {
        const int c = e / t.tp, pl = e - c * t.tp;
        return ((long long)t.b * ga.C + c) * ga.HW + t.p0 + pl;
    };
    auto gn_ld = [&](int e) -> float {
        if (!TO_N) return 0.f;
        const int c = e / t.tp, pl = e - c * t.tp;
        const Dst d = link_dst<LT>(ga, gn, c, t.p0 + pl);
        const long long i = ((long long)t.b * gn.C + (d.to_prior ? 0 : d.c)) * gn.HW + (d.to_prior ? 0 : d.p);
        const float v = n.gx[i];
        return d.to_prior ? 0.f : v;
    };
    float xp[CP_K], gp[CP_K];
#pragma unroll
    for (int k = 0; k < CP_K; ++k) {
        const int e = k * 256 + threadIdx.x;
        const int ec = e < total ? e : 0;
        xp[k] = a.x[aidx(ec)];
        gp[k] = gn_ld(ec);
    }
    const int tid = (int)threadIdx.x;
    const float glp = a.gl_sample ? a.gl_sample[t.b] : 0.f;
    const float gpr = (PRIOR && l.g_lp) ? l.g_lp[t.b] : 0.f;
    const float sc = a.scale[0], ss = a.scale_shift[0];
    float glv[4];
#pragma unroll
    for (int k = 0; k < 4; ++k) {
        const int b = tid + 64 * k;
        const float v = a.gl_sample ? a.gl_sample[b < ga.B ? b : 0] : 0.f;
        glv[k] = (tid < 64 && b < ga.B) ? v : 0.f;
    }
    const int nta = 2 * Cba, ntn = 4 * Cbn, nsn = 2 * Cbn;
    float tav[2], tnv[2];
    double snv[2];
#pragma unroll
    for (int k = 0; k < 2; ++k) {
        const int i = tid + 256 * k;
        tav[k] = a.out_tab[i < nta ? i : 0];
        tnv[k] = TO_N ? n.in_tab[i < ntn ? i : 0] : 0.f;
        snv[k] = TO_N ? n.in_sums[i < nsn ? i : 0] : 0.0;
    }
    TileRegs<2> rst, rgh;
    tile_issue<T, 2>(a.st, t.m0, t.tp, a.cs_st, rst);
    if (TO_N) tile_issue<T, 2>(n.gh0, (long long)t.b * gn.HW + pn0, tpn, csg, rgh);
    {
        const ShardArr arrs[4] = {{PRIOR ? a.prior_sums : a.cls_sums, W2p, psa},
                                  {TO_N ? n.outp_sums : a.cls_sums, 4 * Cn, osn},
                                  {TO_N ? n.in_bwd_sums : a.cls_sums, 2 * Cbn, ibn},
                                  {TO_N ? n.in_bwd_ext : a.cls_sums, 2 * Cbn, iex}};
        lds_shard_reduce_multi(arrs);
    }
    tile_commit<T, 2>(rst, a.st, t.m0, a.cs_st, sta);
    if (TO_N) tile_commit<T, 2>(rgh, n.gh0, (long long)t.b * gn.HW + pn0, csg, gh);
#pragma unroll
    for (int k = 0; k < 2; ++k) {
        const int i = tid + 256 * k;
        if (i < nta) ta[(i / Cba) * Cra + i % Cba] = tav[k];
        if constexpr (TO_N) {
            if (i < ntn) tn[(i / Cbn) * Crn + i % Cbn] = tnv[k];
        }
        if (i < nsn) isn[i] = snv[k];
    }
    if constexpr (TO_N) {
        for (int i = tid + 512; i < ntn; i += blockDim.x) tn[(i / Cbn) * Crn + i % Cbn] = n.in_tab[i];
    }
    if (tid < 64) {
        double s = (double)glv[0] + (double)glv[1] + (double)glv[2] + (double)glv[3];
        if (a.gl_sample)
            for (int b = tid + 256; b < ga.B; b += 64) s += (double)a.gl_sample[b];
        s = wave_sum(s);
        if (tid == 0) gls_sh = s;
    }
    lds_zero(red, 4 * ga.C);
    for (int e = tid; e < t.tp * a.cs_gst; e += blockDim.x) stv(&gs[e], 0.f);
    __syncthreads();
    LINK_STAMP(1);
    for (int cb = tid; cb < Cbn; cb += blockDim.x) {
        tn[4 * Crn + cb] = (float)(ibn[cb] / cnt_n);
        tn[5 * Crn + cb] = (float)(ibn[Cbn + cb] / cnt_n);
        if (blockIdx.x == 0) {
            if (n.g_in_beta) n.g_in_beta[cb] = (float)ibn[cb];
            if (n.g_in_gamma) n.g_in_gamma[cb] = (float)ibn[Cbn + cb];
        }
    }
    for (int cb = tid; cb < Cba; cb += blockDim.x) {
        const int ca = ga.kind == 0 ? cb : ga.on_base + cb;
        double A = 0.0, Bs = 0.0;
        for (int q = 0; q < nc; ++q) {
            if (!cls_tr(ga, nc, ca, q)) continue;
            const Dst d = link_dst<LT>(ga, gn, ca, 0);
            const bool prior_cls = PRIOR && (LT == RNVP_LINK_FINAL || d.to_prior);
            if (prior_cls) {
                A += psa[(2 * q) * ga.C + ca];
                Bs += psa[(2 * q + 1) * ga.C + ca];
                continue;
            }
            int cn, qn;
            if (LT == RNVP_LINK_SAME) {
                cn = ca;
                qn = gn.kind == 0 ? q : -1;
            } else if (LT == RNVP_LINK_SQUEEZE) {
                cn = 4 * ca + q;
                qn = -1;
            } else {
                cn = (ca & 3) == 0 ? (ca >> 2) : gn.C / 2 + (ca >> 2);
                qn = q;
            }
            for (int k = 0; k < 2; ++k)
                if (qn < 0 || qn == k) {
                    A += osn[(2 * k) * Cn + cn];
                    Bs += osn[(2 * k + 1) * Cn + cn];
                }
            const int cbn = in_bn_channel(gn, cn);
            if (cbn >= 0 && (gn.kind == 1 || qn == ((gn.cfg + 1) & 1))) {
                const double NS = (double)gn.B * (gn.kind == 0 ? (double)gn.HW - n_transformed(gn) : (double)gn.HW);
                const double GA = iex[cbn], GAV = iex[Cbn + cbn], SV = isn[cbn], SV2 = isn[Cbn + cbn];
                const double coef = tn[cbn], mi = tn[2 * Crn + cbn], ri = tn[3 * Crn + cbn];
                const double k1 = (float)(ibn[cbn] / cnt_n), k2 = (float)(ibn[Cbn + cbn] / cnt_n);
                const double Sxh = ri * (SV - NS * mi), Sxhv = ri * (SV2 - mi * SV);
                A += coef * (GA - NS * k1 - k2 * Sxh);
                Bs += coef * (GAV - k1 * SV - k2 * Sxhv);
            }
        }
        const double G = gls_sh * n_transformed(ga);
        ta[2 * Cra + cb] = (float)(A / cnt_a);
        ta[3 * Cra + cb] = (float)((Bs + G) / cnt_a);
    }
    __syncthreads();
    LINK_STAMP(2);
    double gsc = 0.0, gss = 0.0;
    auto body = [&](int e0, float xv, float gnv) {
        const int e = e0 + threadIdx.x;
        const bool ok = e < total;
        const int c = ok ? e / t.tp : 0, pl = ok ? e - c * t.tp : 0, p = t.p0 + pl;
        const bool chan_on = ga.kind == 1 && c >= ga.on_base && c < ga.on_base + Cba;
        const int cb = ga.kind == 0 ? c : (chan_on ? c - ga.on_base : 0);
        const bool has_bn = ga.kind == 0 || chan_on;
        const bool tr = ok && (ga.kind == 0 ? !ckbd_m(ga, p) : chan_on);
        float v = xv, th = 0.f, ex = 1.f;
        if (tr) {
            float lr;
            const float u = coupling_u(xv, ldv(&sta[pl * a.cs_st + cb]), ldv(&sta[pl * a.cs_st + Cba + cb]), sc, ss, lr,
                                       th, ex);
            v = (u - ta[cb]) * ta[Cra + cb];
        }
        float gz = 0.f;
        if (ok) {
            const Dst d = link_dst<LT>(ga, gn, c, p);
            if (d.to_prior) {
                gz = -v * gpr;
            } else {
                gz = gnv;
                const int cbn = in_bn_channel(gn, d.c);
                if (cbn >= 0 && (gn.kind != 0 || ckbd_m(gn, d.p))) {
                    const int pnl = d.p - pn0;
// ... 226 lines not shown
```

dl-normalizing-flows_amd/csrc/flow_ops.hip:

```cpp
#include <math.h>

#include "coupling_common.h"

extern "C" int rnvp_version(void) { return 112; }

extern "C" int rnvp_struct_size(int which) {
    switch (which) {
        case 0: return (int)sizeof(rnvp_bn_src);
        case 1: return (int)sizeof(rnvp_bn_running);
        case 2: return (int)sizeof(rnvp_conv_args);
        case 3: return (int)sizeof(rnvp_wgrad_conv);
        case 4: return (int)sizeof(rnvp_wgrad_group);
        case 5: return (int)sizeof(rnvp_bn_bwd_args);
        case 6: return (int)sizeof(rnvp_wn_desc);
        case 7: return (int)sizeof(rnvp_adam_args);
        case 8: return (int)sizeof(rnvp_coupling_args);
        case 9: return (int)sizeof(rnvp_net_step);
        case 10: return (int)sizeof(rnvp_range);
        case 11: return (int)sizeof(rnvp_link_args);
        case 12: return (int)sizeof(rnvp_step_ctl);
    }
    return -1;
}

extern "C" const char* rnvp_status_string(int s) {
    if (s == RNVP_OK) return "ok";
    if (s == RNVP_E_INVALID) return "invalid argument";
    if (s == RNVP_E_UNSUPPORTED) return "unsupported configuration";
    return hipGetErrorString((hipError_t)s);
}

__global__ void k_marker(int tag) { (void)tag; }

extern "C" int rnvp_marker(int tag, void* stream) {
    k_marker<<<1, 1, 0, (hipStream_t)stream>>>(tag);
    RNVP_LAUNCH_CHECK();
    return RNVP_OK;
}

__global__ void k_mask(float* m, int S, int cfg) {
    int i = blockIdx.x * blockDim.x + threadIdx.x;
    if (i < S * S) m[i] = (float)((cfg + i / S + i % S) & 1);
}

extern "C" int rnvp_checkerboard_mask(float* mask, int size, int config, void* stream) {
    if (!mask || size <= 0) return RNVP_E_INVALID;
    k_mask<<<rnvp_grid((long long)size * size, 256, 1 << 20), 256, 0, (hipStream_t)stream>>>(mask, size, config & 1);
    RNVP_LAUNCH_CHECK();
    return RNVP_OK;
}

__global__ void k_squeeze(const float* __restrict__ x, float* __restrict__ y, int C, int H, int W, long long n) {
    const int h2 = H >> 1, w2 = W >> 1;
    for (long long e = blockIdx.x * (long long)blockDim.x + threadIdx.x; e < n; e += (long long)gridDim.x * blockDim.x) {
        int xx = (int)(e % W);
        long long t = e / W;
        int yy = (int)(t % H);
        t /= H;
        int c = (int)(t % C);
        long long b = t / C;
        int i = yy & 1, j = xx & 1;
        long long o = (((b * 4 * C + 4 * c + 2 * i + j) * h2 + (yy >> 1)) * w2 + (xx >> 1));
        y[o] = x[e];
    }
}
__global__ void k_undo_squeeze(const float* __restrict__ y, float* __restrict__ x, int C, int H, int W, long long n) {
    const int h2 = H >> 1, w2 = W >> 1;
    for (long long e = blockIdx.x * (long long)blockDim.x + threadIdx.x; e < n; e += (long long)gridDim.x * blockDim.x) {
        int xx = (int)(e % W);
        long long t = e / W;
        int yy = (int)(t % H);
        t /= H;
        int c = (int)(t % C);
        long long b = t / C;
        int i = yy & 1, j = xx & 1;
        x[e] = y[(((b * 4 * C + 4 * c + 2 * i + j) * h2 + (yy >> 1)) * w2 + (xx >> 1))];
    }
}

extern "C" int rnvp_squeeze(const float* x, float* y, int B, int C, int H, int W, void* stream) {
    if (!x || !y || B < 0 || C <= 0 || (H & 1) || (W & 1)) return RNVP_E_INVALID;
    long long n = (long long)B * C * H * W;
    if (n == 0) return RNVP_OK;
    k_squeeze<<<rnvp_grid(n, 256), 256, 0, (hipStream_t)stream>>>(x, y, C, H, W, n);
    RNVP_LAUNCH_CHECK();
    return RNVP_OK;
}
// ... 484 lines not shown
```

dl-normalizing-flows_amd/realnvp_hip/_lib.py:

```python
import ctypes as C
import os

_HERE = os.path.dirname(os.path.abspath(__file__))
LIB_PATH = os.environ.get("RNVP_LIB_PATH") or os.path.join(_HERE, "librealnvp_hip.so")
if os.environ.get("RNVP_LIB_PATH"):
    import sys as _sys
    print("realnvp_hip: RNVP_LIB_PATH=%s replaces the in-tree library" % LIB_PATH, file=_sys.stderr)

RNVP_F32, RNVP_BF16 = 0, 1

vp = C.c_void_p
i32 = C.c_int
i64 = C.c_longlong
f32 = C.c_float
f64 = C.c_double


class BNSrc(C.Structure):
    _fields_ = [("sums", vp), ("count", f64), ("mean", vp), ("var", vp), ("gamma", vp), ("beta", vp), ("eps", f32),
                ("shards", i32), ("tab", vp)]


def bn_tab_floats(c):
    return 4 * int(c)


class BNRunning(C.Structure):
    _fields_ = [("sums", vp), ("count", f64), ("C", i32), ("shards", i32), ("rmean", vp), ("rvar", vp), ("nbt", vp),
                ("eps", f32), ("tab", vp)]


class ConvArgs(C.Structure):
    _fields_ = [("dtype", i32), ("B", i32), ("H", i32), ("W", i32), ("ks", i32),
                ("x", vp), ("cs_in", i32), ("cin", i32),
                ("w", vp), ("kp", i32),
                ("y", vp), ("cs_out", i32), ("n", i32),
                ("bias", vp), ("residual", vp), ("accumulate", i32),
                ("pro_bn_relu", i32), ("pro", BNSrc),
                ("out_sums", vp),
                ("epi_relu_bn_bwd", i32), ("epi_x", vp), ("epi", BNSrc), ("epi_sums", vp),
                ("ws", vp), ("ws_elems", i64), ("variant", i32), ("w_frag", vp),
                ("bp", i32), ("bp_x", vp), ("bp_bn", BNSrc), ("bp_sums", vp), ("bp_shards", i32),
                ("bp_out", vp), ("bp_dgamma", vp), ("bp_dbeta", vp)]


class BNBwdArgs(C.Structure):
    _fields_ = [("dtype", i32), ("M", i64), ("C", i32), ("cs", i32),
                ("g", vp), ("x", vp), ("bn", BNSrc), ("sums", vp), ("sum_shards", i32),
                ("dx", vp), ("residual", vp), ("accumulate", i32),
                ("dgamma", vp), ("dbeta", vp)]


RNVP_STEP_CONV, RNVP_STEP_BN_BWD = 0, 1
NET_GROUP_MAX = 8


class NetStep(C.Structure):
    _fields_ = [("kind", i32), ("conv", ConvArgs), ("bn", BNBwdArgs), ("dgamma_off", i64), ("dbeta_off", i64),
                ("cfg", i32), ("nc", i32), ("shards", i32), ("xa", i32), ("xb", i32), ("tiles", i32)]


class WNDesc(C.Structure):
    _fields_ = [("v", vp), ("g", vp), ("wf", vp), ("wd", vp), ("norm", vp),
                ("dw", vp), ("dv_off", i64), ("dg_off", i64),
                ("cout", i32), ("cin", i32), ("ks", i32), ("cs_in", i32), ("kp_f", i32),
                ("cs_out", i32), ("kp_d", i32), ("row0", i32), ("tile0", i32),
                ("nz", i32), ("dbp", vp), ("db_off", i64), ("zero_after", i32), ("blk0", i32),
                ("wf_frag", vp), ("wd_frag", vp)]


class Range(C.Structure):
    _fields_ = [("p", vp), ("bytes", i64)]


RNVP_DECAY_NONE, RNVP_DECAY_EXP, RNVP_DECAY_COSINE = 0, 1, 2


class StepCtl(C.Structure):
    _fields_ = [("base_lr", f32), ("warmup_start", f32), ("warmup_steps", i64),
                ("decay", i32), ("decay_rate", f64), ("decay_steps", i64),
                ("max_norm", f32),
                ("lr", f32), ("grad_scale", f32), ("grad_norm", f32), ("skip", i32),
                ("n_clipped", i64), ("n_skipped", i64),
                ("accum_steps", i32), ("micro", i32), ("hold", i32)]


class AdamArgs(C.Structure):
    _fields_ = [("param", vp), ("grad", vp), ("exp_avg", vp), ("exp_avg_sq", vp), ("mask", vp),
                ("step", vp), ("step_add", i64),
                ("lr", f32), ("beta1", f32), ("beta2", f32), ("eps", f32), ("weight_decay", f32),
                ("reg_coef", f32), ("ctl", vp)]


class EmaCtl(C.Structure):
    _fields_ = [("decay", f32), ("warmup", i32), ("applied", f32), ("pad", i32), ("n_updates", i64)]


WGRAD_GROUP_MAX = 24


class WgradConv(C.Structure):
    _fields_ = [("x", vp), ("dy", vp), ("ws", vp), ("wsb", vp), ("pro", BNSrc),
                ("cs_in", i32), ("cin", i32), ("ks", i32), ("cs_dy", i32), ("n", i32), ("kp", i32),
                ("pro_bn_relu", i32), ("nz", i32), ("nrep", i32), ("m_per_slab", i64), ("task0", i32),
                ("tk", i32), ("cls", i32)]


class WgradGroup(C.Structure):
    _fields_ = [("dtype", i32), ("B", i32), ("H", i32), ("W", i32), ("n_conv", i32),
                ("conv", WgradConv * WGRAD_GROUP_MAX)]


class WgradMultiConv(C.Structure):
    _fields_ = [("x", vp), ("dy", vp), ("ws", vp), ("wsb", vp), ("pro", BNSrc),
                ("cs_in", i32), ("cin", i32), ("cs_dy", i32), ("n", i32), ("kp", i32), ("pro_bn_relu", i32),
                ("nz", i32), ("nrep", i32), ("B", i32), ("H", i32), ("W", i32), ("cls", i32),
                ("tco", i32), ("tci", i32), ("m_per_slab", i64)]


class WgradMulti(C.Structure):
    _fields_ = [("cls", i32), ("ko", i32), ("n_conv", i32), ("n_task", i32), ("grid", i32), ("lds_bytes", i32),
                ("xcd_cost", i64 * 8), ("convs", vp), ("xcd_start", vp), ("tasks", vp)]


class CouplingArgs(C.Structure):
    _fields_ = [("kind", i32), ("B", i32), ("C", i32), ("H", i32), ("W", i32), ("mask_config", i32),
                ("coupling_bn", i32), ("training", i32), ("dtype", i32),
                ("momentum", f32), ("eps", f32),
                ("x", vp),
                ("in_gamma", vp), ("in_beta", vp), ("in_rmean", vp), ("in_rvar", vp), ("in_nbt", vp),
                ("in_sums", vp),
                ("h0", vp), ("cs_h0", i32),
                ("st", vp), ("cs_st", i32),
                ("scale", vp), ("scale_shift", vp),
                ("u", vp), ("z", vp), ("out_sums", vp),
                ("out_rmean", vp), ("out_rvar", vp), ("out_nbt", vp),
                ("ldj_sample", vp), ("ldj_full", vp),
                ("gz", vp), ("gl_full", vp), ("gl_sample", vp), ("gx", vp),
                ("gst", vp), ("cs_gst", i32),
                ("bwd_sums", vp), ("g_scale", vp), ("g_scale_shift", vp),
                ("gh0", vp), ("cs_gh0", i32),
                ("in_bwd_sums", vp), ("g_in_gamma", vp), ("g_in_beta", vp),
                ("net_running", vp), ("n_net_running", i32), ("net_running_cmax", i32),
                ("gscale_part", vp),
                ("nclass", i32), ("cls_sums", vp), ("prior_sums", vp), ("outp_sums", vp), ("in_bwd_ext", vp),
                ("out_tab", vp), ("in_tab", vp)]


RNVP_LINK_SAME, RNVP_LINK_SQUEEZE, RNVP_LINK_UNFACTOR, RNVP_LINK_FINAL = 0, 1, 2, 3


class LinkArgs(C.Structure):
    _fields_ = [("type", i32), ("g_lp", vp), ("prior", vp), ("off", vp), ("z", vp)]


class TensorRef(C.Structure):
    _fields_ = [("p", vp), ("g", vp), ("n", i64)]


_SIGS = {
    "rnvp_version": (i32, []),
    "rnvp_struct_size": (i32, [i32]),
    "rnvp_status_string": (C.c_char_p, [i32]),
    "rnvp_marker": (i32, [i32, vp]),
    "rnvp_checkerboard_mask": (i32, [vp, i32, i32, vp]),
    "rnvp_squeeze": (i32, [vp, vp, i32, i32, i32, i32, vp]),
    "rnvp_undo_squeeze": (i32, [vp, vp, i32, i32, i32, i32, vp]),
    "rnvp_factor_out": (i32, [vp, vp, vp, i32, i32, i32, i32, vp]),
    "rnvp_restore": (i32, [vp, vp, vp, i32, i32, i32, i32, vp]),
    "rnvp_logit_fwd": (i32, [vp, vp, C.c_uint64, C.c_uint64, vp, f32, vp, vp, i32, i32, vp]),
    "rnvp_logit_inv": (i32, [vp, vp, f32, i64, vp]),
    "rnvp_u8_to_unit": (i32, [vp, vp, i64, vp]),
    "rnvp_nchw_to_nhwc": (i32, [vp, vp, i32, i32, i32, i32, i32, i32, vp]),
    "rnvp_nhwc_to_nchw": (i32, [vp, vp, i32, i32, i32, i32, i32, i32, vp]),
    "rnvp_prior_logprob": (i32, [vp, vp, vp, i32, i32, vp]),
    "rnvp_prior_logprob_bwd": (i32, [vp, vp, vp, i32, i32, vp]),
    "rnvp_bn_running_update": (i32, [vp, i32, i32, f32, vp]),
    "rnvp_stat_shards": (i32, [i64]),
    "rnvp_conv2d": (i32, [C.POINTER(ConvArgs), vp]),
    "rnvp_conv2d_check": (i32, [C.POINTER(ConvArgs)]),
    "rnvp_conv2d_family": (i32, [C.POINTER(ConvArgs)]),
    "rnvp_wgrad_slabs": (i32, [i64]),
    "rnvp_wgrad_replicas": (i32, [i32]),
    "rnvp_conv2d_wgrad_grouped": (i32, [C.POINTER(WgradGroup), vp]),
    "rnvp_wgrad_class": (i32, [C.POINTER(WgradGroup), i32]),
    "rnvp_wgrad_multi_plan": (i32, [C.POINTER(WgradGroup), i32, i32, C.POINTER(WgradMultiConv), i32, C.POINTER(i32),
                                    C.POINTER(i32), i32, C.POINTER(WgradMulti)]),
    "rnvp_conv2d_wgrad_multi": (i32, [C.POINTER(WgradMulti), vp]),
    "rnvp_wgrad_multi_struct_size": (i32, [i32]),
    "rnvp_bn_bwd_apply": (i32, [C.POINTER(BNBwdArgs), vp]),
    "rnvp_weight_norm_fwd": (i32, [vp, i32, i32, i32, i32, vp]),
    "rnvp_weight_norm_tiles": (i32, [i32, i32, i32]),
    "rnvp_weight_norm_bwd": (i32, [vp, i32, i32, vp, vp, i64, vp, i64, vp]),
    "rnvp_weight_norm_opt_blocks": (i32, [i32, i32, i32]),
    "rnvp_weight_norm_bwd_adam": (i32, [vp, i32, i32, i32, i32, C.POINTER(AdamArgs), vp, i64, vp, i64, vp]),
    "rnvp_adam_gather": (i32, [C.POINTER(AdamArgs), vp, i64, vp]),
    "rnvp_weight_norm_transpose": (i32, [vp, i32, i32, i32, vp]),
    "rnvp_zero_ranges": (i32, [vp, i32, i64, vp]),
    "rnvp_coupling_in_fwd": (i32, [C.POINTER(CouplingArgs), vp]),
    "rnvp_coupling_out_fwd": (i32, [C.POINTER(CouplingArgs), vp]),
    "rnvp_coupling_reverse": (i32, [C.POINTER(CouplingArgs), vp]),
    "rnvp_coupling_reverse_bwd": (i32, [C.POINTER(CouplingArgs), vp]),
    "rnvp_coupling_out_bwd": (i32, [C.POINTER(CouplingArgs), vp]),
    "rnvp_coupling_in_bwd": (i32, [C.POINTER(CouplingArgs), vp]),
    "rnvp_link_nclass": (i32, [i32, i32]),
    "rnvp_coupling_out_u": (i32, [C.POINTER(CouplingArgs), vp]),
    "rnvp_coupling_link_fwd": (i32, [C.POINTER(CouplingArgs), C.POINTER(CouplingArgs), C.POINTER(LinkArgs), vp]),
    "rnvp_coupling_link_bwd": (i32, [C.POINTER(CouplingArgs), C.POINTER(CouplingArgs), C.POINTER(LinkArgs), vp]),
    "rnvp_coupling_in_apply": (i32, [C.POINTER(CouplingArgs), vp]),
    "rnvp_flow_in_fwd": (i32, [vp, C.c_uint64, vp, f32, vp, vp, C.POINTER(CouplingArgs), i32, i32, i32, i32, vp]),
    "rnvp_flow_lp_finish": (i32, [vp, vp, vp, i32, vp, vp, i32, vp]),
    "rnvp_sumsq_multi": (i32, [vp, i32, vp, vp]),
    "rnvp_sumsq_bwd_multi": (i32, [vp, i32, vp, f32, vp]),
    "rnvp_adam_step": (i32, [vp, vp, vp, vp, i64, vp, f32, f32, f32, f32, f32, vp, f32, vp]),
    "rnvp_adam_update": (i32, [vp, vp, vp, vp, i64, vp, i64, f32, f32, f32, f32, f32, vp, f32, vp]),
    "rnvp_step_increment": (i32, [vp, vp]),
    "rnvp_grad_sumsq_parts": (i32, [i64]),
    "rnvp_grad_sumsq": (i32, [C.POINTER(AdamArgs), i64, vp, i32, vp]),
    "rnvp_grad_accumulate": (i32, [C.POINTER(AdamArgs), vp, i64, vp, vp, i32, vp]),
    "rnvp_step_control": (i32, [vp, vp, vp, i32, vp]),
    "rnvp_adam_range": (i32, [C.POINTER(AdamArgs), i64, vp]),
    "rnvp_step_advance": (i32, [vp, vp, vp]),
    "rnvp_ema_struct_size": (i32, []),
    "rnvp_ema_update": (i32, [vp, vp, i64, vp, vp, i64, vp, vp]),
    "rnvp_ema_swap": (i32, [vp, vp, i64, vp]),
    "rnvp_fill_f64": (i32, [vp, i64, f64, vp]),
    "rnvp_net_group_prepare": (i32, [vp, i32, C.POINTER(i32), C.POINTER(i32), C.POINTER(i32)]),
    "rnvp_net_group": (i32, [vp, i32, i32, i32, i32, i32, vp]),
}

EXPORTED = sorted(_SIGS)


class _Lib:
    def __init__(self, path=LIB_PATH):
        if not os.path.exists(path):
            raise RuntimeError("librealnvp_hip.so not built (%s); run __graft_entry__.build()" % path)
        self.dll = C.CDLL(path)
        for name, (res, args) in _SIGS.items():
            fn = getattr(self.dll, name)
            fn.restype = res
            fn.argtypes = args
            raw = name in ("rnvp_version", "rnvp_struct_size", "rnvp_stat_shards", "rnvp_wgrad_slabs", "rnvp_wgrad_replicas",
                           "rnvp_link_nclass", "rnvp_conv2d_check", "rnvp_conv2d_family", "rnvp_wgrad_class", "rnvp_wgrad_multi_plan", "rnvp_wgrad_multi_struct_size",
                           "rnvp_grad_sumsq_parts", "rnvp_ema_struct_size",
                           "rnvp_weight_norm_tiles", "rnvp_weight_norm_opt_blocks",
                           "rnvp_net_group_prepare") or res is not i32
            setattr(self, name[len("rnvp_"):], fn if raw else self._wrap(name, fn))
        mirrors = (BNSrc, BNRunning, ConvArgs, WgradConv, WgradGroup, BNBwdArgs, WNDesc, AdamArgs, CouplingArgs,
                   NetStep, Range, LinkArgs, StepCtl)
        for i, m in enumerate(mirrors):
            if self.dll.rnvp_struct_size(i) != C.sizeof(m):
                raise RuntimeError("%s: struct %s is %d bytes in the library, %d in the binding (stale build?)"
                                   % (path, m.__name__, self.dll.rnvp_struct_size(i), C.sizeof(m)))
        for i, m in enumerate((WgradMultiConv, WgradMulti)):
            if self.dll.rnvp_wgrad_multi_struct_size(i) != C.sizeof(m):
                raise RuntimeError("%s: struct %s is %d bytes in the library, %d in the binding (stale build?)"
                                   % (path, m.__name__, self.dll.rnvp_wgrad_multi_struct_size(i), C.sizeof(m)))
        if self.dll.rnvp_ema_struct_size() != C.sizeof(EmaCtl):
            raise RuntimeError("%s: struct %s is %d bytes in the library, %d in the binding (stale build?)"
                               % (path, EmaCtl.__name__, self.dll.rnvp_ema_struct_size(), C.sizeof(EmaCtl)))

    def _wrap(self, name, fn):
        dll = self.dll

        def call(*args):
            st = fn(*args)
            if st != 0:
                msg = dll.rnvp_status_string(st)
                raise RuntimeError("%s failed: status %d (%s)" % (name, st, msg.decode() if msg else "?"))
        call.__name__ = name
        return call


_lib = None


def lib() -> _Lib:
    global _lib
    if _lib is None:
        _lib = _Lib()
    return _lib
```

dl-normalizing-flows_amd/realnvp_hip/engine.py:

```python
import ctypes as C
from collections import OrderedDict

import torch

from . import _lib
from ._lib import (BNBwdArgs, BNRunning, BNSrc, ConvArgs, CouplingArgs, NetStep, WgradConv, WgradGroup, WgradMulti,
                   WgradMultiConv, WNDesc, bn_tab_floats, NET_GROUP_MAX, RNVP_BF16, RNVP_F32, RNVP_STEP_BN_BWD,
                   RNVP_STEP_CONV, WGRAD_GROUP_MAX)
from .net import backward_program, build_program, chan_stride, round_up

BN_EPS = 1e-5
COUPLING_SHARDS = 16
BN_MOMENTUM = 0.1

DTYPES = {"fp32": (RNVP_F32, 4, torch.float32), "bf16": (RNVP_BF16, 2, torch.bfloat16)}
CONV_VARIANT = 0
NET_GROUP = True
FOLD_BN = True
BN_TABLES = True
WGRAD_MULTI = True


def stream_ptr():
    return torch.cuda.current_stream().cuda_stream


def upload(raw, device):
    host = torch.frombuffer(bytearray(raw), dtype=torch.uint8)
    device = torch.device(device)
    if device.type != "cuda":
        return host
    return host.pin_memory().to(device, non_blocking=True)


PROFILE = None
MARKERS = False
MARKER_FAMILIES = []


def _launch(family, nbytes, flops, fn, *args):
    if PROFILE is None and not MARKERS:
        return fn(*args)
    if MARKERS:
        _lib.lib().marker(len(MARKER_FAMILIES), stream_ptr())
        MARKER_FAMILIES.append(family)
    if PROFILE is None:
        fn(*args)
    else:
        e0 = torch.cuda.Event(enable_timing=True)
        e1 = torch.cuda.Event(enable_timing=True)
        e0.record()
        fn(*args)
        e1.record()
        PROFILE.append((family, nbytes, flops, e0, e1))
    if MARKERS:
        _lib.lib().marker(-1, stream_ptr())


def plan_wgrad_multi(groups, device):
    L = _lib.lib()
    arr = (WgradGroup * len(groups))()
    for i, g in enumerate(groups):
        C.memmove(C.addressof(arr[i]), C.addressof(g), C.sizeof(WgradGroup))
    out = []
    for cls in range(4):
        m = WgradMulti()
        if L.wgrad_multi_plan(arr, len(groups), cls, None, 0, None, None, 0, C.byref(m)) != 0:
            return None
        if m.n_conv == 0:
            continue
        convs = (WgradMultiConv * m.n_conv)()
        xs = (C.c_int * 9)()
        tasks = (C.c_int * (2 * m.n_task))()
        if L.wgrad_multi_plan(arr, len(groups), cls, convs, m.n_conv, xs, tasks, m.n_task, C.byref(m)) != 0:
            return None
        raw = bytes(convs)
        o_x = round_up(len(raw), 64)
        raw += b"\0" * (o_x - len(raw)) + bytes(xs) + b"\0" * (64 - 36) + bytes(tasks)
        t = upload(raw, device)
        m.convs, m.xcd_start, m.tasks = t.data_ptr(), t.data_ptr() + o_x, t.data_ptr() + o_x + 64
        out.append((m, t))
    return out


class Arena:

    def __init__(self):
        self.slots = OrderedDict()
        self.total = 0
        self.buf = None

    def add(self, name, nbytes):
        assert name not in self.slots, name
        self.slots[name] = (self.total, int(nbytes))
        self.total = round_up(self.total + int(nbytes), 256)

    def alloc(self, device, zero=False):
        n = max(self.total, 256)
        self.buf = (torch.zeros if zero else torch.empty)(n, dtype=torch.uint8, device=device)
        self.base = self.buf.data_ptr()
        return self

    def ptr(self, name):
# ... 401 lines not shown
            if op.pro_bn:
                a.pro_bn_relu = 1
                a.pro = self._bn(T, op.pro_bn, training, ar.ptr("s:" + op.pro_bn), M)
            a.out_sums = ar.ptr("s:" + op.stats_bn) if (op.stats_bn and training) else None
            if sc["ws"] is not None:
                a.ws, a.ws_elems = sc["ws"].data_ptr(), sc["ws_elems"]
            a.variant = CONV_VARIANT
            esz = DTYPES[sv["dtype"]][1]
            nb = esz * (M * cs_in + spec.cout * kp_f + M * cs_out * (1 + int(bool(op.residual)) + int(op.accumulate)))
            out.append((a, nb, 2.0 * M * spec.cout * spec.ks * spec.ks * spec.cin))
        return out

    def chains_into(self, nxt):
        return (nxt.kind == self.kind and nxt.C == self.C and nxt.cfg != self.cfg and
                bool(self.hp.coupling_bn))

    def forward(self, x, training, dtype, full_ldj, saved=None, prepare=True, ldj_sample=None, z_out=None,
                zero_sums=True):
        L = _lib.lib()
        B, Cc, H, W = x.shape
        assert Cc == self.C, "channel mismatch"
        dev = x.device
        s = stream_ptr()
        ws = self.prepare_weights(dtype) if prepare else self.weights(dtype)
        sv = saved if saved is not None else self.alloc_saved(B, H, W, dtype, dev, training)
        ar = sv["arena"]
        T = self._tensors()
        z = torch.empty_like(x) if z_out is None else z_out
        if ldj_sample is None:
            ldj_sample = torch.zeros(B, device=dev, dtype=torch.float32)
        ldj_full = torch.empty_like(x) if full_ldj else None
        if training and zero_sums:
            s0, e0 = ar.range_bytes("in_sums", list(ar.slots)[-1])
            ar.buf[s0:e0].zero_()
        a = self._coupling_args(T, x, B, H, W, dtype, training)
        a.in_sums = ar.ptr("in_sums")
        a.h0 = ar.ptr("h0")
        n_el, esz = x.numel(), DTYPES[dtype][1]
        cs_h0, cs_st = chan_stride(self.P.buf_ch["h0"]), chan_stride(self.P.buf_ch["st"])
        _launch("coupling", (8 if training else 4) * n_el + esz * B * H * W * cs_h0, 0.0, L.coupling_in_fwd,
                C.byref(a), s)
        self._net_forward(T, sv, ws, training, s)
        if training and "bn_table" in sv:
            a.net_running, a.n_net_running, a.net_running_cmax = (sv["bn_table"].data_ptr(), sv["bn_n"],
                                                                  sv["bn_cmax"])
        a.st = ar.ptr("st")
        a.u, a.z = ar.ptr("u"), z.data_ptr()
        a.out_sums = ar.ptr("out_sums")
        a.ldj_sample = ldj_sample.data_ptr()
        a.ldj_full = ldj_full.data_ptr() if full_ldj else None
        _launch("coupling", 16 * n_el + esz * B * H * W * cs_st, 0.0, L.coupling_out_fwd, C.byref(a), s)
        sv["x"] = x
        return z, (ldj_full if full_ldj else ldj_sample), sv

    def reverse(self, x, training, dtype, saved=None, out=None, want_ldj=True, prepare=True):
        L = _lib.lib()
        B, Cc, H, W = x.shape
        s = stream_ptr()
        ws = self.prepare_weights(dtype) if prepare else self.weights(dtype)
        sv = saved if saved is not None else self.alloc_saved(B, H, W, dtype, x.device, training)
        ar = sv["arena"]
        T = self._tensors()
        if training:
            s0, e0 = ar.range_bytes("in_sums", list(ar.slots)[-1])
            ar.buf[s0:e0].zero_()
        a = self._coupling_args(T, x, B, H, W, dtype, training)
        a.in_sums = ar.ptr("in_sums")
        a.h0 = ar.ptr("h0")
        L.coupling_in_fwd(C.byref(a), s)
        self._net_forward(T, sv, ws, training, s)
        if training and "bn_table" in sv:
            L.bn_running_update(sv["bn_table"].data_ptr(), sv["bn_n"], sv["bn_cmax"], BN_MOMENTUM, s)
        if out is None:
            out = torch.empty_like(x)
        ldj = torch.empty_like(x) if want_ldj else None
        a.st = ar.ptr("st")
        a.z = out.data_ptr()
        a.ldj_full = ldj.data_ptr() if want_ldj else None
        L.coupling_reverse(C.byref(a), s)
        sv["x"] = x
        return out, ldj


    def _net_backward(self, sv, sc, ws, T, training, gp, s):
        L = _lib.lib()
        x = sv["x"]
        dt = DTYPES[sv["dtype"]][0]
        key = (ws["key"], id(sc), bool(training), FOLD_BN, BN_TABLES)
        plan = sv.get("bwd_plan")
        if plan is None or plan[0] != key:
            plan = (key, self._bwd_args(T, sv, sc, ws, training))
            sv["bwd_plan"] = plan
        items, groups, wg_bytes, wg_flops = plan[1]
        if len(plan) < 3:
            steps = []
            for kind, c, nb, fl, bn, rw in items:
                st = NetStep()
                st.dgamma_off = st.dbeta_off = -1
                if kind == "dgrad":
                    st.kind = RNVP_STEP_CONV
                    st.conv = c
                else:
                    st.kind = RNVP_STEP_BN_BWD
                    st.bn = c
                    st.dgamma_off = self.layout[bn + "weight"][0]
                    st.dbeta_off = self.layout[bn + "bias"][0]
                steps.append(st)
            plan = plan + (plan_launches(steps, x.device, [it[5] for it in items]),)
            sv["bwd_plan"] = plan
        for g in plan[2]:
            if g[0] == "single":
                kind, c, nb, fl, bn, _ = items[g[1]]
                if kind == "dgrad":
                    if bn is not None:
                        c.bp_dgamma, c.bp_dbeta = gp(bn + "weight"), gp(bn + "bias")
                    _launch("conv_dgrad", nb, fl, L.conv2d, C.byref(c), s)
                else:
                    c.dgamma, c.dbeta = gp(bn + "weight"), gp(bn + "bias")
                    _launch("bn_bwd", nb, 0.0, L.bn_bwd_apply, C.byref(c), s)
            else:
                _, i0, i1, klass, grid, lds, tab = g
                nb = sum(items[i][2] for i in range(i0, i1))
                fl = sum(items[i][3] for i in range(i0, i1))
                _launch("conv_dgrad", nb, fl, L.net_group, C.addressof(tab), i1 - i0, dt, klass, grid, lds, s)

    def _wgrad_multi_ok(self, sv, sc, groups, multi):
        if not WGRAD_MULTI or sv["dtype"] != "bf16" or any(it[4] == id(sc) for it in multi):
            return False
        key = sv["bwd_plan"][0]
        ok = sv.get("wg_multi_ok")
        if ok is None or ok[0] != key:
            L = _lib.lib()
            m = WgradMulti()
            ok = (key, all(L.wgrad_multi_plan(C.byref(g), 1, 0, None, 0, None, None, 0, C.byref(m)) == 0
                           for g in groups))
            sv["wg_multi_ok"] = ok
        return ok[1]

    def _weight_grads(self, sv, sc, ws, zero_at_end, opt, after, gbase, multi=None):
        L = _lib.lib()
        ar, sar = sv["arena"], sc["arena"]
        z0, z1 = sc["zero"]
        dt = DTYPES[sv["dtype"]][0]
        items, groups, wg_bytes, wg_flops = sv["bwd_plan"][1]

        def weight_grads():
            ss = stream_ptr()
            if multi is not None and opt == "defer" and self._wgrad_multi_ok(sv, sc, groups, multi):
                multi.append((groups, wg_bytes, wg_flops, (sv["bwd_plan"][0], ar.base), id(sc)))
            else:
                for grp in groups:
                    _launch("conv_wgrad", wg_bytes / len(groups), wg_flops / len(groups), L.conv2d_wgrad_grouped,
                            C.byref(grp), ss)
            if zero_at_end:
                f0, f1 = ar.range_bytes("in_sums", list(ar.slots)[-1])
                zr = (ar.base + f0, f1 - f0, sar.base + z0, z1 - z0)
            else:
                zr = (None, 0, sar.base + z0, z1 - z0)
            if isinstance(opt, str):
                pass
            elif opt is not None:
                L.weight_norm_bwd_adam(sc["wn_table"].data_ptr(), sc["n_wn"], sc["wn_blocks"], 1, dt, C.byref(opt),
                                       *zr, ss)
            else:
                L.weight_norm_bwd(sc["wn_table"].data_ptr(), sc["n_wn"], sc["wn_rows"], gbase, *zr, ss)
            if after is not None:
                after()

        return weight_grads

    def _bwd_args(self, T, sv, sc, ws, training):
        B, H, W, dtype = sv["B"], sv["H"], sv["W"], sv["dtype"]
        M = B * H * W
        dt = DTYPES[dtype][0]
        esz = DTYPES[dtype][1]
        ar, sar, war = sv["arena"], sc["arena"], ws["arena"]
        items, groups = [], []

        def tab(bn):
            ok = BN_TABLES and training and "bn_table" in sv and ar.has("t:" + bn)
            return ar.ptr("t:" + bn) if ok else None

        ent = []
        wg_bytes = wg_flops = 0.0
        wbase = sc["wg_ws"].data_ptr()
        for st in self.steps:
            op = st.op
            spec = self.P.convs[op.conv]
            cs_in, cs_out, kp_f, kp_d = ws["geo"][op.conv]
            if st.kind == "dgrad":
                c = ConvArgs()
                c.dtype, c.B, c.H, c.W, c.ks = dt, B, H, W, spec.ks
                c.x, c.cs_in, c.cin = sar.ptr(st.gy), cs_out, spec.cout
                c.w, c.kp = war.ptr("wd:" + op.conv), kp_d
                c.w_frag = war.ptr("wdf:" + op.conv) if war.has("wdf:" + op.conv) else None
                c.y = sar.ptr(st.tmp if st.tmp else st.gx)
                c.cs_out, c.n = cs_in, spec.cin
                c.residual = sar.ptr(st.residual) if st.residual else None
                c.accumulate = int(st.accumulate)
                if op.pro_bn:
                    c.epi_relu_bn_bwd = 1
                    c.epi_x = ar.ptr(op.x)
                    c.epi = self._bn(T, op.pro_bn, training, ar.ptr("s:" + op.pro_bn), M, tab(op.pro_bn))
                    c.epi_sums = sar.ptr("e:" + op.pro_bn)
                if sc["ws"] is not None:
                    c.ws, c.ws_elems = sc["ws"].data_ptr(), sc["ws_elems"]
                c.variant = CONV_VARIANT
# ... 140 lines not shown
            weight_grads()
        else:
            ev = torch.cuda.Event()
            ev.record()
            side.wait_event(ev)
            with torch.cuda.stream(side):
                weight_grads()

    def link_args(self, sv, x, grad_block=None, gx=None):
        B, H, W, dtype = sv["B"], sv["H"], sv["W"], sv["dtype"]
        T = self._tensors()
        ar = sv["arena"]
        sar = self.scratch_checked(B, H, W, dtype, x.device)["arena"]
        a = self._coupling_args(T, x, B, H, W, dtype, True)
        a.in_sums, a.h0, a.st = ar.ptr("in_sums"), ar.ptr("h0"), ar.ptr("st")
        a.cls_sums, a.prior_sums = ar.ptr("cls_sums"), ar.ptr("prior_sums")
        a.out_tab, a.in_tab = ar.ptr("out_tab"), ar.ptr("in_tab")
        a.gst, a.cs_gst = sar.ptr("g:st"), chan_stride(self.P.buf_ch["st"])
        a.gh0, a.cs_gh0 = sar.ptr("g:h0"), chan_stride(self.P.buf_ch["h0"])
        a.in_bwd_sums, a.in_bwd_ext = sar.ptr("in_bwd_sums"), sar.ptr("in_bwd_ext")
        a.outp_sums, a.gscale_part = sar.ptr("outp_sums"), sar.ptr("gscale_part")
        if grad_block is not None:
            gb = grad_block.data_ptr()
            gp = lambda n: gb + 4 * self.layout[n][0]
            a.g_scale, a.g_scale_shift = gp("scale"), gp("scale_shift")
            a.g_in_gamma, a.g_in_beta = gp("in_bn.weight"), gp("in_bn.bias")
        if gx is not None:
            a.gx = gx.data_ptr()
        return a

    def forward_link(self, x, sv, ldj_sample, link):
        L = _lib.lib()
        s = stream_ptr()
        dtype = sv["dtype"]
        ws = self.weights(dtype)
        T = self._tensors()
        B, H, W = sv["B"], sv["H"], sv["W"]
        self._net_forward(T, sv, ws, True, s)
        a = self.link_args(sv, x)
        a.nclass = link["nclass"]
        a.ldj_sample = ldj_sample.data_ptr()
        a.gl_sample = link["args"].g_lp
        if "bn_table" in sv:
            a.net_running, a.n_net_running, a.net_running_cmax = sv["bn_table"].data_ptr(), sv["bn_n"], sv["bn_cmax"]
        n_el, esz = x.numel(), DTYPES[dtype][1]
        cs_st = chan_stride(self.P.buf_ch["st"])
        _launch("coupling", 4 * n_el + esz * B * H * W * cs_st, 0.0, L.coupling_out_u, C.byref(a), s)
        nb = 8 * n_el + esz * B * H * W * cs_st
        if link["nxt"] is not None:
            neng, nsv, nx = link["nxt"]
            n = neng.link_args(nsv, nx)
            nb += esz * nsv["B"] * nsv["H"] * nsv["W"] * chan_stride(neng.P.buf_ch["h0"])
            _launch("coupling", nb, 0.0, L.coupling_link_fwd, C.byref(a), C.byref(n), C.byref(link["args"]), s)
        else:
            _launch("coupling", nb, 0.0, L.coupling_link_fwd, C.byref(a), None, C.byref(link["args"]), s)
        sv["x"] = x

    def backward_link(self, sv, link, grad_block, gx, gl_sample, first, defer, opt=None, after=None, multi=None):
        L = _lib.lib()
        x = sv["x"]
        B, H, W, dtype = sv["B"], sv["H"], sv["W"], sv["dtype"]
        s = stream_ptr()
        T = self._tensors()
        ws = self.weights(dtype)
        sc = self.scratch_checked(B, H, W, dtype, x.device)
        gbase = grad_block.data_ptr()

        def gp(name):
            return gbase + 4 * self.layout[name][0]

        a = self.link_args(sv, x, grad_block, gx)
        a.nclass = link["nclass"]
        a.gl_sample = gl_sample.data_ptr()
        n_el, esz = x.numel(), DTYPES[dtype][1]
        cs_st = chan_stride(self.P.buf_ch["st"])
        nb = 12 * n_el + 2 * esz * B * H * W * cs_st
        if link["nxt"] is not None:
            neng, nsv, nx, ngx, nblock = link["nxt"]
            n = neng.link_args(nsv, nx, nblock, ngx)
            nb += esz * nsv["B"] * nsv["H"] * nsv["W"] * chan_stride(neng.P.buf_ch["h0"])
            _launch("coupling", nb, 0.0, L.coupling_link_bwd, C.byref(a), C.byref(n), C.byref(link["args"]), s)
        else:
            _launch("coupling", nb, 0.0, L.coupling_link_bwd, C.byref(a), None, C.byref(link["args"]), s)
        self._net_backward(sv, sc, ws, T, True, gp, s)
        if not first:
            a.gx = None
        cs_h0 = chan_stride(self.P.buf_ch["h0"])
        _launch("coupling", (8 if first else 4) * n_el + (2 if first else 1) * esz * B * H * W * cs_h0, 0.0,
                L.coupling_in_bwd, C.byref(a), s)
        self._issue_weight_grads(self._weight_grads(sv, sc, ws, True, opt, after, gbase, multi), defer, None)
```

include/realnvp_hip.h:

```cpp
#ifndef REALNVP_HIP_H
#define REALNVP_HIP_H

#include <stdint.h>

#ifdef __cplusplus
extern "C" {
#endif

enum { RNVP_F32 = 0, RNVP_BF16 = 1 };
enum { RNVP_OK = 0, RNVP_E_INVALID = -1, RNVP_E_UNSUPPORTED = -2 };

int rnvp_version(void);
int rnvp_struct_size(int which);
const char* rnvp_status_string(int status);
int rnvp_marker(int tag, void* stream);

int rnvp_checkerboard_mask(float* mask, int size, int config, void* stream);
int rnvp_squeeze(const float* x, float* y, int B, int C, int H, int W, void* stream);
int rnvp_undo_squeeze(const float* y, float* x, int B, int C, int H, int W, void* stream);
int rnvp_factor_out(const float* x, float* on, float* off, int B, int C, int H, int W, void* stream);
int rnvp_restore(const float* on, const float* off, float* x, int B, int C, int H, int W, void* stream);

int rnvp_logit_fwd(const float* x, const float* noise, uint64_t seed, uint64_t offset, const long long* epoch,
                   float constraint, float* y, float* logdet, int B, int n_per_sample, void* stream);
int rnvp_logit_inv(const float* x, float* y, float constraint, long long n, void* stream);

int rnvp_u8_to_unit(const uint8_t* x, float* y, long long n, void* stream);

int rnvp_nchw_to_nhwc(const float* x, void* y, int B, int C, int H, int W, int cs, int dtype, void* stream);
int rnvp_nhwc_to_nchw(const void* x, float* y, int B, int C, int H, int W, int cs, int dtype, void* stream);

int rnvp_prior_logprob(const float* z, const float* ldj, float* out, int B, int n_per_sample, void* stream);
int rnvp_prior_logprob_bwd(const float* z, const float* gout, float* gz, int B, int n_per_sample, void* stream);

typedef struct rnvp_bn_src {
    const double* sums;
    double count;
    const float* mean;
    const float* var;
    const float* gamma;
    const float* beta;
    float eps;
    int shards;
    const float* tab;
} rnvp_bn_src;
#define RNVP_BN_TAB_FLOATS(C) (4 * (C))
int rnvp_stat_shards(long long M);

typedef struct rnvp_bn_running {
    const double* sums; double count; int C; int shards;
    float* rmean; float* rvar; long long* nbt;
    float eps; float* tab;
} rnvp_bn_running;
int rnvp_bn_running_update(const rnvp_bn_running* descs_device, int n, int max_c, float momentum, void* stream);

#define RNVP_VARIANT_DEEP 2
#define RNVP_VARIANT_DEEP0 16
typedef struct rnvp_conv_args {
    int dtype;
    int B, H, W, ks;
    const void* x; int cs_in; int cin;
    const void* w; int kp;
    void* y; int cs_out; int n;
    const float* bias;
    const void* residual;
    int accumulate;
    int pro_bn_relu; rnvp_bn_src pro;
    double* out_sums;
    int epi_relu_bn_bwd; const void* epi_x; rnvp_bn_src epi; double* epi_sums;
    float* ws; long long ws_elems;
    int variant;
    const void* w_frag;
    int bp; const void* bp_x; rnvp_bn_src bp_bn; const double* bp_sums; int bp_shards;
    void* bp_out; float* bp_dgamma; float* bp_dbeta;
} rnvp_conv_args;
int rnvp_conv2d(const rnvp_conv_args* a, void* stream);
int rnvp_conv2d_check(const rnvp_conv_args* a);
enum { RNVP_FAMILY_OTHER = 0, RNVP_FAMILY_DEEP = 1, RNVP_FAMILY_S1 = 2, RNVP_FAMILY_BAND = 3 };
int rnvp_conv2d_family(const rnvp_conv_args* a);

#define RNVP_WGRAD_GROUP_MAX 24
typedef struct rnvp_wgrad_conv {
    const void* x; const void* dy;
    float* ws;
    float* wsb;
    rnvp_bn_src pro;
    int cs_in, cin, ks, cs_dy, n, kp, pro_bn_relu, nz, nrep;
    long long m_per_slab;
    int task0, tk, cls;
} rnvp_wgrad_conv;
typedef struct rnvp_wgrad_group {
    int dtype, B, H, W, n_conv;
    rnvp_wgrad_conv conv[RNVP_WGRAD_GROUP_MAX];
} rnvp_wgrad_group;
int rnvp_wgrad_slabs(long long M);
int rnvp_wgrad_replicas(int nz);
int rnvp_conv2d_wgrad_grouped(const rnvp_wgrad_group* g, void* stream);
int rnvp_wgrad_class(const rnvp_wgrad_group* g, int c);

typedef struct rnvp_wgrad_multi_conv {
    const void* x; const void* dy; float* ws; float* wsb;
    rnvp_bn_src pro;
    int cs_in, cin, cs_dy, n, kp, pro_bn_relu, nz, nrep;
    int B, H, W, cls;
    int tco, tci;
    long long m_per_slab;
} rnvp_wgrad_multi_conv;
typedef struct rnvp_wgrad_multi {
    int cls, ko, n_conv, n_task, grid, lds_bytes;
    long long xcd_cost[8];
    const rnvp_wgrad_multi_conv* convs;
    const int* xcd_start;
    const int* tasks;
} rnvp_wgrad_multi;
int rnvp_wgrad_multi_plan(const rnvp_wgrad_group* groups, int n_groups, int cls, rnvp_wgrad_multi_conv* convs,
                          int conv_cap, int* xcd_start, int* tasks, int task_cap, rnvp_wgrad_multi* m);
int rnvp_conv2d_wgrad_multi(const rnvp_wgrad_multi* m, void* stream);
int rnvp_wgrad_multi_struct_size(int which);

typedef struct rnvp_bn_bwd_args {
    int dtype; long long M; int C; int cs;
    const void* g; const void* x; rnvp_bn_src bn;
    const double* sums; int sum_shards;
    void* dx; const void* residual; int accumulate;
    float* dgamma; float* dbeta;
} rnvp_bn_bwd_args;
int rnvp_bn_bwd_apply(const rnvp_bn_bwd_args* a, void* stream);

typedef struct rnvp_wn_desc {
    const float* v; const float* g;
    void* wf; void* wd; float* norm;
    float* dw;
    long long dv_off; long long dg_off;
    int cout, cin, ks, cs_in, kp_f, cs_out, kp_d;
    int row0;
    int tile0;
    int nz;
    float* dbp;
    long long db_off;
    int zero_after;
    int blk0;
    void* wf_frag; void* wd_frag;
} rnvp_wn_desc;
int rnvp_weight_norm_tiles(int cout, int cin, int ks);
int rnvp_weight_norm_fwd(const rnvp_wn_desc* descs_device, int n_desc, int total_rows, int total_tiles, int dtype,
                         void* stream);
int rnvp_weight_norm_bwd(const rnvp_wn_desc* descs_device, int n_desc, int total_rows, float* grad_base,
                         void* zero0, long long zero0_bytes, void* zero1, long long zero1_bytes, void* stream);

enum { RNVP_DECAY_NONE = 0, RNVP_DECAY_EXP = 1, RNVP_DECAY_COSINE = 2 };
typedef struct rnvp_step_ctl {
    float base_lr; float warmup_start; long long warmup_steps;
    int decay; double decay_rate; long long decay_steps;
    float max_norm;
    float lr, grad_scale, grad_norm; int skip;
    long long n_clipped, n_skipped;
    int accum_steps;
    int micro;
    int hold;
} rnvp_step_ctl;
typedef struct rnvp_adam_args {
    float* param; float* grad; float* exp_avg; float* exp_avg_sq; const uint8_t* mask;
    const long long* step; long long step_add;
    float lr, beta1, beta2, eps, weight_decay, reg_coef;
    const rnvp_step_ctl* ctl;
} rnvp_adam_args;
int rnvp_weight_norm_opt_blocks(int cout, int cin, int ks);
int rnvp_weight_norm_bwd_adam(const rnvp_wn_desc* descs_device, int n_desc, int total_blocks, int from_slabs,
                              int dtype, const rnvp_adam_args* adam, void* zero0, long long zero0_bytes,
                              void* zero1, long long zero1_bytes, void* stream);
int rnvp_weight_norm_transpose(const rnvp_wn_desc* descs_device, int n_desc, int total_tiles, int dtype,
                               void* stream);
typedef struct rnvp_range { void* p; long long bytes; } rnvp_range;
int rnvp_zero_ranges(const rnvp_range* ranges_device, int n, long long max_bytes, void* stream);
int rnvp_adam_gather(const rnvp_adam_args* adam, const long long* idx, long long n, void* stream);

#ifndef RNVP_COUPLING_SHARDS
#define RNVP_COUPLING_SHARDS 16
#endif
typedef struct rnvp_coupling_args {
    int kind, B, C, H, W, mask_config, coupling_bn, training, dtype;
    float momentum, eps;
    const float* x;
    const float* in_gamma; const float* in_beta;
    float* in_rmean; float* in_rvar; long long* in_nbt;
    double* in_sums;
    void* h0; int cs_h0;
    const void* st; int cs_st;
    const float* scale; const float* scale_shift;
    float* u;
    float* z;
    double* out_sums;
    float* out_rmean; float* out_rvar; long long* out_nbt;
    float* ldj_sample;
    float* ldj_full;
    const float* gz;
    const float* gl_full;
    const float* gl_sample;
    float* gx;
    void* gst; int cs_gst;
    double* bwd_sums;
    float* g_scale; float* g_scale_shift;
    const void* gh0; int cs_gh0;
    double* in_bwd_sums;
    float* g_in_gamma; float* g_in_beta;
    const rnvp_bn_running* net_running; int n_net_running; int net_running_cmax;
    double* gscale_part;
    int nclass;
    double* cls_sums;
    double* prior_sums;
    double* outp_sums;
    double* in_bwd_ext;
    float* out_tab;
    float* in_tab;
} rnvp_coupling_args;
int rnvp_coupling_in_fwd(const rnvp_coupling_args* a, void* stream);
int rnvp_coupling_out_fwd(const rnvp_coupling_args* a, void* stream);
int rnvp_coupling_reverse(const rnvp_coupling_args* a, void* stream);
int rnvp_coupling_reverse_bwd(const rnvp_coupling_args* a, void* stream);
int rnvp_coupling_out_bwd(const rnvp_coupling_args* a, void* stream);
int rnvp_coupling_in_bwd(const rnvp_coupling_args* a, void* stream);

enum { RNVP_LINK_SAME = 0, RNVP_LINK_SQUEEZE = 1, RNVP_LINK_UNFACTOR = 2, RNVP_LINK_FINAL = 3 };
typedef struct rnvp_link_args {
    int type;
    const float* g_lp;
    double* prior;
    float* off;
    float* z;
} rnvp_link_args;
int rnvp_link_nclass(int type, int kind);
int rnvp_coupling_out_u(const rnvp_coupling_args* a, void* stream);
int rnvp_coupling_link_fwd(const rnvp_coupling_args* a, const rnvp_coupling_args* n, const rnvp_link_args* l,
                           void* stream);
int rnvp_coupling_link_bwd(const rnvp_coupling_args* a, const rnvp_coupling_args* n, const rnvp_link_args* l,
                           void* stream);
int rnvp_coupling_in_apply(const rnvp_coupling_args* a, void* stream);
int rnvp_flow_in_fwd(const float* x, uint64_t seed, const long long* epoch, float constraint, float* y,
                     float* logdet, const rnvp_coupling_args* first, int B, int C, int H, int W, void* stream);
int rnvp_flow_lp_finish(double* prior, float* ldj, float* logdet, int zero_logdet, float* lp, double* ll_acc, int B,
                        void* stream);

typedef struct rnvp_tensor_ref { float* p; float* g; long long n; } rnvp_tensor_ref;
int rnvp_sumsq_multi(const rnvp_tensor_ref* refs_device, int n_refs, float* out, void* stream);
int rnvp_sumsq_bwd_multi(const rnvp_tensor_ref* refs_device, int n_refs, const float* gout, float coef, void* stream);

int rnvp_adam_step(float* param, float* grad, float* exp_avg, float* exp_avg_sq, long long n,
                   long long* step, float lr, float beta1, float beta2, float eps, float weight_decay,
                   const uint8_t* mask, float reg_coef, void* stream);

int rnvp_adam_update(float* param, float* grad, float* exp_avg, float* exp_avg_sq, long long n,
                     const long long* step, long long step_add, float lr, float beta1, float beta2, float eps,
                     float weight_decay, const uint8_t* mask, float reg_coef, void* stream);
int rnvp_step_increment(long long* step, void* stream);

int rnvp_grad_sumsq_parts(long long n);
int rnvp_grad_sumsq(const rnvp_adam_args* ad, long long n, double* partials, int n_parts, void* stream);
int rnvp_grad_accumulate(const rnvp_adam_args* ad, float* acc, long long n, const rnvp_step_ctl* ctl,
                         double* partials, int n_parts, void* stream);
int rnvp_step_control(rnvp_step_ctl* ctl, const long long* step, const double* partials, int n_parts, void* stream);
int rnvp_adam_range(const rnvp_adam_args* ad, long long n, void* stream);
int rnvp_step_advance(long long* step, const rnvp_step_ctl* ctl, void* stream);

typedef struct rnvp_ema_ctl {
    float decay;
    int warmup;
    float applied;
    int pad;
    long long n_updates;
} rnvp_ema_ctl;
int rnvp_ema_struct_size(void);
int rnvp_ema_update(float* ema, const float* param, long long n, rnvp_ema_ctl* ectl, const long long* step,
                    long long step_add, const rnvp_step_ctl* ctl , void* stream);
int rnvp_ema_swap(float* a, float* b, long long n, void* stream);

enum { RNVP_STEP_CONV = 0, RNVP_STEP_BN_BWD = 1 };
typedef struct rnvp_net_step {
    int kind;
    rnvp_conv_args conv;
    rnvp_bn_bwd_args bn;
    long long dgamma_off, dbeta_off;
    int cfg, nc, shards, xa, xb, tiles;
} rnvp_net_step;

#define RNVP_NET_GROUP_MAX 8
int rnvp_net_group_prepare(rnvp_net_step* steps_host, int n, int* klass, int* grid, int* lds_bytes);
int rnvp_net_group(const rnvp_net_step* steps_host, int n, int dtype, int klass, int grid, int lds_bytes,
                   void* stream);

int rnvp_fill_f64(double* p, long long n, double v, void* stream);

#ifdef __cplusplus
}
#endif
#endif
```

Before: 3474 images/sec.

## Fuse coupling input-BN backward statistics into the final data-gradient conv epilogue

```diff
diff --git a/dl-normalizing-flows_amd/csrc/conv.hip b/dl-normalizing-flows_amd/csrc/conv.hip
--- a/dl-normalizing-flows_amd/csrc/conv.hip
+++ b/dl-normalizing-flows_amd/csrc/conv.hip
@@ -38,6 +38,13 @@
         if (a->bp_bn.sums && (!a->bp_sums || a->bp_shards < 1 || a->bp_bn.count <= 0)) return RNVP_E_INVALID;
         if (!a->bp_bn.sums && (!a->bp_bn.mean || !a->bp_bn.var)) return RNVP_E_INVALID;
         if (a->pro_bn_relu) return RNVP_E_INVALID;
+    }
+    if (a->ib) {
+        if (!a->ib_x || !a->ib_tab || !a->ib_sums) return RNVP_E_INVALID;
+        if ((a->ib_kind != 0 && a->ib_kind != 1) || a->ib_C <= 0 || (a->ib_kind == 1 && (a->ib_C & 1))) return RNVP_E_INVALID;
+        const int Cb = a->ib_kind == 0 ? a->ib_C : a->ib_C / 2;
+        if (a->n != (a->ib_kind == 0 ? 2 * Cb + 1 : 2 * Cb)) return RNVP_E_INVALID;
+        if (a->bp || a->pro_bn_relu || a->epi_relu_bn_bwd || a->out_sums) return RNVP_E_INVALID;
     }
     return RNVP_OK;
 }
@@ -92,6 +99,23 @@
 }
 
 int route_conv(const rnvp_conv_args* a, hipStream_t s, bool dry, int* fam = nullptr) {
+    if (a->ib) {
+        rnvp_conv_args p = *a;
+        p.ib = 0;
+        int f = RNVP_FAMILY_OTHER;
+        int r = dispatch_conv(&p, nullptr, true, &f);
+        if (r != RNVP_OK) return r;
+        if (f == RNVP_FAMILY_DEEP) {
+            const int cfg = a->variant >= RNVP_VARIANT_DEEP0 ? a->variant - RNVP_VARIANT_DEEP0 : rnvp_deep_auto_cfg(a);
+            r = rnvp_deep_launch(a, s, cfg, dry);
+        } else if (f == RNVP_FAMILY_OTHER && a->variant != 1 && rnvp_conv_band_ok(a)) {
+            r = rnvp_conv_band1_launch(a, s, dry);
+        } else {
+            r = RNVP_E_UNSUPPORTED;
+        }
+        if (fam && r == RNVP_OK) *fam = f;
+        return r;
+    }
     if (a->bp) {
         const int cfg = bp_cfg_of(a);
         int r, f = RNVP_FAMILY_DEEP;
diff --git a/dl-normalizing-flows_amd/csrc/conv_band1.hip b/dl-normalizing-flows_amd/csrc/conv_band1.hip
--- a/dl-normalizing-flows_amd/csrc/conv_band1.hip
+++ b/dl-normalizing-flows_amd/csrc/conv_band1.hip
@@ -3,22 +3,23 @@
 
 #include "common.h"
 #include "conv_common.h"
+#include "conv_in_bwd.h"
 
 namespace {
 
 template <typename T>
-size_t band_lds_bytes(int cs, int n, int W, int ks) {
+size_t band_lds_bytes(int cs, int n, int W, int ks, bool ib = false) {
     constexpr int CH = Mf<T>::CH, KS = 4 * CH, BM = 256;
     const int nc = n <= 16 ? 16 : (n <= 32 ? 32 : 64);
     const int K = ks * ks * cs;
     const int kpl = lds_mfma_pitch(((K + KS - 1) / KS) * KS, CH);
     const int R = BM + 2 * (ks / 2) * (W + 1);
     const int ntmp = cs > nc ? cs : nc;
-    return 16 * (size_t)ntmp + 8 * (size_t)cs + 20 * (size_t)nc + 64 * (size_t)nc +
+    return 16 * (size_t)ntmp + 8 * (size_t)cs + 20 * (size_t)nc + (ib ? 128 : 64) * (size_t)nc +
            ((size_t)nc * kpl + (size_t)(R + 1) * lds_mfma_pitch(cs, CH)) * sizeof(T);
 }
 
-template <typename T, int NT, int KSZ, bool PRO, int NH>
+template <typename T, int NT, int KSZ, bool PRO, int NH, bool IB = false>
 __global__ __launch_bounds__(256 * NH) void k_conv_band(rnvp_conv_args a, int shards) {
     constexpr int CH = Mf<T>::CH, KS = 4 * CH;
     constexpr int NC = 16 * NT;
@@ -27,6 +28,8 @@
     constexpr int SB = 12 / NH;
     constexpr int NTH = 256 * NH, NTW = NT / NH;
     static_assert(NT % NH == 0, "channel tiles split evenly");
+    static_assert(!IB || (!PRO && NH == 1), "in-part sums: the in conv's plain data gradient, four waves");
+    constexpr int SW = IB ? 4 : 2;
     extern __shared__ double dsm[];
     const int tid = threadIdx.x, lane = tid & 63, g = lane >> 4, li = lane & 15;
     const int wid = (tid >> 6) & 3, hf = tid >> 8;
@@ -45,7 +48,7 @@
     float* etab = bnp + 2 * cs;
     float* btab = etab + 4 * NC;
     double* red = (double*)(btab + NC);
-    T* Wl = (T*)(red + 8 * NC);
+    T* Wl = (T*)(red + 4 * SW * NC);
     T* zrow = Wl + NC * kpl;
     T* act = zrow + pitch;
 
@@ -91,6 +94,16 @@
         }
     };
     stage_load(0);
+    float xq[IB ? TM : 1][IB ? NTW : 1][4];
+    floatx4 ibt = {};
+    if constexpr (IB) {
+#pragma unroll
+        for (int i = 0; i < TM; ++i)
+#pragma unroll
+            for (int j = 0; j < NTW; ++j)
+                ib_prefetch(a, m0 + wid * 64 + i * 16 + li, M, (hf * NTW + j) * 16 + 4 * g, xq[i][j]);
+        ibt = ib_tab_load(a, tid < NC ? tid : 0);
+    }
 
     if (PRO) block_bn_table(a.pro, a.cin, 0, cs, bnp, bnp + cs, nullptr, nullptr, tmp);
     if (epi_bn) block_bn_table(a.epi, N, 0, NC, etab, etab + NC, etab + 2 * NC, etab + 3 * NC, tmp);
@@ -120,6 +133,11 @@
             }
         }
         for (int n = tid; n < NC; n += NTH) btab[n] = (a.bias && n < N) ? a.bias[n] : 0.f;
+        if constexpr (IB) {
+            if (tid < NC) {
+                etab[tid] = ibt.x; etab[NC + tid] = ibt.y; etab[2 * NC + tid] = ibt.z; etab[3 * NC + tid] = ibt.w;
+            }
+        }
         for (int c = tid * CH; c < pitch; c += NTH * CH) *(u32x4*)(zrow + c) = u32x4{0u, 0u, 0u, 0u};
     }
     __syncthreads();
@@ -190,6 +208,13 @@
     for (int j = 0; j < NTW; ++j)
 #pragma unroll
         for (int r = 0; r < 4; ++r) s1[j][r] = s2[j][r] = 0.0;
+    double x1[IB ? NTW : 1][4], x2[IB ? NTW : 1][4];
+    if constexpr (IB) {
+#pragma unroll
+        for (int j = 0; j < NTW; ++j)
+#pragma unroll
+            for (int r = 0; r < 4; ++r) x1[j][r] = x2[j][r] = 0.0;
+    }
 #pragma unroll
     for (int i = 0; i < TM; ++i) {
         const int m = m0 + wid * 64 + i * 16 + li;
@@ -198,11 +223,52 @@
         for (int j = 0; j < NTW; ++j) {
             const int n0 = (hf * NTW + j) * 16 + 4 * g;
             if (n0 >= cso) continue;
-            epi4<T>(a, (long long)m * cso + n0, acc[i][j], btab + n0, epi_bn, etab + n0, NC, s1[j], s2[j], N - n0);
+            if constexpr (IB) {
+                const long long o = (long long)m * cso + n0;
+                EpiPre pre;
+                if (a.residual) ld4((const T*)a.residual + o, pre.r);
+                if (a.accumulate) ld4((const T*)a.y + o, pre.y);
+#pragma unroll
+                for (int r = 0; r < 4; ++r) pre.x[r] = xq[i][j][r];
+                epi4p_ib<T>(a, o, acc[i][j], btab + n0, etab + n0, NC, s1[j], s2[j], x1[j], x2[j], n0, m, M, pre);
+            } else {
+                epi4<T>(a, (long long)m * cso + n0, acc[i][j], btab + n0, epi_bn, etab + n0, NC, s1[j], s2[j], N - n0);
+            }
         }
     }
     const bool want_sums = a.out_sums || (epi_bn && a.epi_sums);
-    if (want_sums) {
+    if constexpr (IB) {
+        const int Cb = ib_cb(a);
+#pragma unroll
+        for (int j = 0; j < NTW; ++j)
+#pragma unroll
+            for (int r = 0; r < 4; ++r) {
+                const double u1 = row_sum16(s1[j][r]), u2 = row_sum16(s2[j][r]);
+                const double u3 = a.ib_kind == 0 ? row_sum16(x1[j][r]) : u1, u4 = row_sum16(x2[j][r]);
+                const int col = (hf * NTW + j) * 16 + 4 * g + r;
+                if (li == 0) {
+                    double* d = red + (wid * NC + col) * 4;
+                    d[0] = u1; d[1] = u2; d[2] = u3; d[3] = u4;
+                }
+            }
+        __syncthreads();
+        double* sums = ib_shard(a.ib_sums, blockIdx.x, Cb);
+        double* ext = a.ib_ext ? ib_shard(a.ib_ext, blockIdx.x, Cb) : nullptr;
+        for (int n = tid; n < 2 * Cb && n < NC; n += NTH) {
+            double t[4] = {0.0, 0.0, 0.0, 0.0};
+#pragma unroll
+            for (int w = 0; w < 4; ++w)
+#pragma unroll
+                for (int k = 0; k < 4; ++k) t[k] += red[(w * NC + n) * 4 + k];
+            const int cb = ib_chan(n, Cb);
+            atomicAdd(&sums[cb], t[0]);
+            atomicAdd(&sums[Cb + cb], t[1]);
+            if (ext) {
+                atomicAdd(&ext[cb], t[2]);
+                atomicAdd(&ext[Cb + cb], t[3]);
+            }
+        }
+    } else if (want_sums) {
 #pragma unroll
         for (int j = 0; j < NTW; ++j)
 #pragma unroll
@@ -230,11 +296,24 @@
 }
 
 template <typename T, int NT, int KSZ>
-int launch_band(const rnvp_conv_args* a, hipStream_t s) {
+int launch_band(const rnvp_conv_args* a, hipStream_t s, bool dry) {
     const long long M = (long long)a->B * a->H * a->W;
     const unsigned grid = (unsigned)((M + 255) / 256);
-    const size_t shm = band_lds_bytes<T>(a->cs_in, a->n, a->W, KSZ);
+    const size_t shm = band_lds_bytes<T>(a->cs_in, a->n, a->W, KSZ, a->ib != 0);
     const int sh = rnvp_stat_shards(M);
+    if (a->ib) {
+        if constexpr (NT == 1) {
+            if (a->bp || a->pro_bn_relu || a->epi_relu_bn_bwd || a->out_sums || shm > 150 * 1024) return RNVP_E_UNSUPPORTED;
+            if (M > 65536) return RNVP_E_UNSUPPORTED;
+            if (dry) return RNVP_OK;
+            k_conv_band<T, NT, KSZ, false, 1, true><<<grid, 256, shm, s>>>(*a, sh);
+            RNVP_LAUNCH_CHECK();
+            return RNVP_OK;
+        } else {
+            return RNVP_E_UNSUPPORTED;
+        }
+    }
+    if (dry) return RNVP_OK;
     if constexpr ((NT == 4 || NT == 2) && KSZ == 3) {
         if (a->pro_bn_relu) k_conv_band<T, NT, KSZ, true, 2><<<grid, 512, shm, s>>>(*a, sh);
         else k_conv_band<T, NT, KSZ, false, 2><<<grid, 512, shm, s>>>(*a, sh);
@@ -256,10 +335,10 @@
 }
 
 template <typename T>
-int dispatch_band(const rnvp_conv_args* a, hipStream_t s) {
-    if (a->n <= 16) return launch_band<T, 1, 3>(a, s);
-    if (a->n <= 32) return launch_band<T, 2, 3>(a, s);
-    return launch_band<T, 4, 3>(a, s);
+int dispatch_band(const rnvp_conv_args* a, hipStream_t s, bool dry) {
+    if (a->n <= 16) return launch_band<T, 1, 3>(a, s, dry);
+    if (a->n <= 32) return launch_band<T, 2, 3>(a, s, dry);
+    return launch_band<T, 4, 3>(a, s, dry);
 }
 
 }
@@ -268,7 +347,7 @@
     return a->dtype == RNVP_F32 ? band_ok<float>(a) : band_ok<bf16_t>(a);
 }
 
-int rnvp_conv_band1_launch(const rnvp_conv_args* a, hipStream_t s) {
+int rnvp_conv_band1_launch(const rnvp_conv_args* a, hipStream_t s, bool dry) {
     if (!rnvp_conv_band_ok(a)) return RNVP_E_UNSUPPORTED;
-    return a->dtype == RNVP_F32 ? dispatch_band<float>(a, s) : dispatch_band<bf16_t>(a, s);
-}
+    return a->dtype == RNVP_F32 ? dispatch_band<float>(a, s, dry) : dispatch_band<bf16_t>(a, s, dry);
+}
diff --git a/dl-normalizing-flows_amd/csrc/conv_common.h b/dl-normalizing-flows_amd/csrc/conv_common.h
--- a/dl-normalizing-flows_amd/csrc/conv_common.h
+++ b/dl-normalizing-flows_amd/csrc/conv_common.h
@@ -80,21 +80,26 @@
     if (a.epi_relu_bn_bwd) ld4((const T*)a.epi_x + oo, p.x);
 }
 
+__device__ __forceinline__ void epi_vals(const rnvp_conv_args& a, const floatx4& acc, const float* bias, const EpiPre& p,
+                                         float* v) {
+#pragma unroll
+    for (int r = 0; r < 4; ++r) v[r] = acc[r] + bias[r];
+    if (a.residual) {
+#pragma unroll
+        for (int r = 0; r < 4; ++r) v[r] += p.r[r];
+    }
+    if (a.accumulate) {
+#pragma unroll
+        for (int r = 0; r < 4; ++r) v[r] += p.y[r];
+    }
+}
+
 template <typename T>
 __device__ __forceinline__ void epi4p(const rnvp_conv_args& a, long long o, const floatx4& acc, const float* bias,
                                       bool epi_bn, const float* et, int pitch, double* s1, double* s2, int nvalid,
                                       const EpiPre& p) {
     float v[4];
-#pragma unroll
-    for (int r = 0; r < 4; ++r) v[r] = acc[r] + bias[r];
-    if (a.residual) {
-#pragma unroll
-        for (int r = 0; r < 4; ++r) v[r] += p.r[r];
-    }
-    if (a.accumulate) {
-#pragma unroll
-        for (int r = 0; r < 4; ++r) v[r] += p.y[r];
-    }
+    epi_vals(a, acc, bias, p, v);
     if (epi_bn) {
 #pragma unroll
         for (int r = 0; r < 4; ++r) {
@@ -388,7 +393,7 @@
 int rnvp_conv_halo_launch(const rnvp_conv_args* a, hipStream_t s);
 
 bool rnvp_conv_band_ok(const rnvp_conv_args* a);
-int rnvp_conv_band1_launch(const rnvp_conv_args* a, hipStream_t s);
+int rnvp_conv_band1_launch(const rnvp_conv_args* a, hipStream_t s, bool dry = false);
 
 constexpr int RNVP_DEEP_CFGS = 7;
 int rnvp_deep_launch(const rnvp_conv_args* a, hipStream_t s, int cfg, bool dry = false);
diff --git a/dl-normalizing-flows_amd/csrc/conv_deep.h b/dl-normalizing-flows_amd/csrc/conv_deep.h
--- a/dl-normalizing-flows_amd/csrc/conv_deep.h
+++ b/dl-normalizing-flows_amd/csrc/conv_deep.h
@@ -3,6 +3,7 @@
 
 #include "common.h"
 #include "conv_common.h"
+#include "conv_in_bwd.h"
 
 namespace {
 
@@ -21,11 +22,11 @@
 __host__ __device__ constexpr int deep_pitch(int cs) { return lds_mfma_pitch(cs, Mf<T>::CH); }
 
 template <typename T, int BN, int NW, int WK, int BM = DEEP_BM>
-size_t deep_lds_bytes(int cs, int W, int ks, bool bp = false) {
+size_t deep_lds_bytes(int cs, int W, int ks, bool bp = false, bool ib = false) {
     constexpr int TM = BM / 16, WM = NW / WK;
     constexpr int G = WK > 1 ? TM : WM;
     const int hal = (ks / 2) * (W + 1), R = BM + 2 * hal;
-    const size_t head = 4 * (5 * (size_t)BN) + 8 * (2 * (size_t)G * BN) + 4 * (bp ? 3 : 2) * (size_t)cs;
+    const size_t head = 4 * (5 * (size_t)BN) + 8 * ((ib ? 4 : 2) * (size_t)G * BN) + 4 * (bp ? 3 : 2) * (size_t)cs;
     const size_t zrow = (size_t)deep_pitch<T>(cs) * sizeof(T);
     size_t act = (size_t)R * deep_pitch<T>(cs) * sizeof(T);
     const size_t red = WK > 1 ? (size_t)WK * BM * (BN + 4) * 4 : 0;
@@ -33,7 +34,7 @@
 }
 
 template <typename T, int BN, int KSZ, bool PRO, int NW, int WK, int DK, int NC, bool FM = false, int BM = DEEP_BM,
-          bool BP = false>
+          bool BP = false, bool IB = false>
 __device__ __forceinline__ void deep_tile(const rnvp_conv_args& a, int shards, int xa, int xb, int vb, int nvb,
                                           char* lds) {
     constexpr int NT = 64 * NW;
@@ -51,6 +52,8 @@
     static_assert(!TALL || TM % NW == 0, "row groups per wave");
     constexpr int CPT = (NC * WK * KS + NT - 1) / NT;
     static_assert(!(BP && PRO), "BatchNorm-backward prologue: data gradients only");
+    static_assert(!(IB && (PRO || BP)), "in-part sums: the in conv's plain data gradient");
+    constexpr int SW = IB ? 4 : 2;
     constexpr int NSTEP = KSZ * KSZ * NC;
     const int tid = threadIdx.x, lane = tid & 63, g = lane >> 4, li = lane & 15;
     const int wid = __builtin_amdgcn_readfirstlane(tid >> 6);
@@ -87,7 +90,7 @@
     float* etab = (float*)lds;
     float* btab = etab + 4 * BN;
     double* sred = (double*)(btab + BN);
-    float* bnp = (float*)(sred + G * BN * 2);
+    float* bnp = (float*)(sred + G * BN * SW);
     T* zrow = (T*)(bnp + (BP ? 3 : 2) * cs);
     T* act = zrow + pitch;
 
@@ -186,7 +189,10 @@
         int m, col;
         elem(e, m, col);
         epi_prefetch<T>(a, (long long)m * cso + n0 + col, m < M && n0 + col < cso, pre[e]);
-    }
+        if constexpr (IB) ib_prefetch(a, m, M, n0 + col, pre[e].x);
+    }
+    floatx4 ibt = {};
+    if constexpr (IB) ibt = ib_tab_load(a, n0 + (tid < BN ? tid : 0));
     stage_load(0);
     const T* wrow[TN];
 #pragma unroll
@@ -258,6 +264,11 @@
     }
     if (epi_bn) tab_finish<1, NT>(a.epi, N, n0, BN, etb, etab, etab + BN, etab + 2 * BN, etab + 3 * BN);
     if (tid < BN) btab[tid] = bval;
+    if constexpr (IB) {
+        if (tid < BN) {
+            etab[tid] = ibt.x; etab[BN + tid] = ibt.y; etab[2 * BN + tid] = ibt.z; etab[3 * BN + tid] = ibt.w;
+        }
+    }
     for (int c = tid * CH; c < pitch; c += NT * CH) *(u32x4*)(zrow + c) = u32x4{0u, 0u, 0u, 0u};
     __syncthreads();
     DEEP_STAMP(1);
@@ -342,10 +353,17 @@
     const bool want_sums = a.out_sums || (epi_bn && a.epi_sums);
     constexpr int NS = (WK > 1 && !TALL) ? FR : TN;
     double s1[NS][4], s2[NS][4];
+    double x1[IB ? NS : 1][4], x2[IB ? NS : 1][4];
 #pragma unroll
     for (int f = 0; f < NS; ++f)
 #pragma unroll
         for (int r = 0; r < 4; ++r) s1[f][r] = s2[f][r] = 0.0;
+    if constexpr (IB) {
+#pragma unroll
+        for (int f = 0; f < NS; ++f)
+#pragma unroll
+            for (int r = 0; r < 4; ++r) x1[f][r] = x2[f][r] = 0.0;
+    }
     const int grp = TALL ? wid : (WK > 1 ? wid % TM : wm);
     constexpr int GU = TALL ? NW : G;
     if constexpr (WK > 1) {
@@ -369,7 +387,11 @@
             floatx4 v = *(const floatx4*)&red[(ri * 16 + li) * RP + col];
 #pragma unroll
             for (int w = 1; w < WK; ++w) v += *(const floatx4*)&red[(w * BM + ri * 16 + li) * RP + col];
-            epi4p<T>(a, (long long)m * cso + n, v, btab + col, epi_bn, etab + col, BN, s1[sl], s2[sl], N - n, pre[f]);
+            if constexpr (IB)
+                epi4p_ib<T>(a, (long long)m * cso + n, v, btab + col, etab + col, BN, s1[sl], s2[sl], x1[sl], x2[sl], n, m,
+                            M, pre[f]);
+            else
+                epi4p<T>(a, (long long)m * cso + n, v, btab + col, epi_bn, etab + col, BN, s1[sl], s2[sl], N - n, pre[f]);
         }
     } else {
 #pragma unroll
@@ -378,12 +400,49 @@
             elem(e, m, col);
             const int n = n0 + col;
             if (m >= M || n >= cso) continue;
-            epi4p<T>(a, (long long)m * cso + n, acc[e / TN][e % TN], btab + col, epi_bn, etab + col, BN, s1[e % TN],
-                     s2[e % TN], N - n, pre[e]);
+            if constexpr (IB)
+                epi4p_ib<T>(a, (long long)m * cso + n, acc[e / TN][e % TN], btab + col, etab + col, BN, s1[e % TN],
+                            s2[e % TN], x1[e % TN], x2[e % TN], n, m, M, pre[e]);
+            else
+                epi4p<T>(a, (long long)m * cso + n, acc[e / TN][e % TN], btab + col, epi_bn, etab + col, BN, s1[e % TN],
+                         s2[e % TN], N - n, pre[e]);
         }
     }
     DEEP_STAMP(4);
-    if (want_sums) {
+    if constexpr (IB) {
+        const int Cb = ib_cb(a);
+#pragma unroll
+        for (int f = 0; f < NS; ++f)
+#pragma unroll
+            for (int r = 0; r < 4; ++r) {
+                const double u1 = row_sum16(s1[f][r]), u2 = row_sum16(s2[f][r]);
+                const double u3 = a.ib_kind == 0 ? row_sum16(x1[f][r]) : u1, u4 = row_sum16(x2[f][r]);
+                if (li == 0) {
+                    const int cb = ((WK > 1 && !TALL) ? ((wid / TM) * FR + f) : f) * 16 + 4 * g;
+                    double* d = sred + (grp * BN + cb + r) * 4;
+                    d[0] = u1; d[1] = u2; d[2] = u3; d[3] = u4;
+                }
+            }
+        __syncthreads();
+        double* sums = ib_shard(a.ib_sums, vb, Cb);
+        double* ext = a.ib_ext ? ib_shard(a.ib_ext, vb, Cb) : nullptr;
+        for (int col = tid; col < BN; col += NT) {
+            const int n = n0 + col;
+            if (n >= 2 * Cb) continue;
+            double t[4] = {0.0, 0.0, 0.0, 0.0};
+#pragma unroll
+            for (int q = 0; q < GU; ++q)
+#pragma unroll
+                for (int k = 0; k < 4; ++k) t[k] += sred[(q * BN + col) * 4 + k];
+            const int cb = ib_chan(n, Cb);
+            atomicAdd(&sums[cb], t[0]);
+            atomicAdd(&sums[Cb + cb], t[1]);
+            if (ext) {
+                atomicAdd(&ext[cb], t[2]);
+                atomicAdd(&ext[Cb + cb], t[3]);
+            }
+        }
+    } else if (want_sums) {
 #pragma unroll
         for (int f = 0; f < NS; ++f)
 #pragma unroll
diff --git a/dl-normalizing-flows_amd/csrc/conv_deep_launch.h b/dl-normalizing-flows_amd/csrc/conv_deep_launch.h
--- a/dl-normalizing-flows_amd/csrc/conv_deep_launch.h
+++ b/dl-normalizing-flows_amd/csrc/conv_deep_launch.h
@@ -4,11 +4,14 @@
 namespace {
 
 template <typename T, int BN, int KSZ, bool PRO, int NW, int WK, int DK, int NC, bool FM = false, int BM = DEEP_BM,
-          bool BP = false>
+          bool BP = false, bool IB = false>
 __global__ __launch_bounds__(64 * NW) void k_conv_deep(rnvp_conv_args a, int shards, int xa, int xb) {
     extern __shared__ __attribute__((aligned(16))) char lds[];
-    deep_tile<T, BN, KSZ, PRO, NW, WK, DK, NC, FM, BM, BP>(a, shards, xa, xb, blockIdx.x, gridDim.x, lds);
+    deep_tile<T, BN, KSZ, PRO, NW, WK, DK, NC, FM, BM, BP, IB>(a, shards, xa, xb, blockIdx.x, gridDim.x, lds);
 }
+
+template <int BN, int NW, int WK, int BM, int KSZ>
+constexpr bool ib_cfg() { return BN == 32 && WK == NW && BM == DEEP_BM && KSZ == 3; }
 
 template <int BN, int NW, int WK, int BM>
 constexpr bool bp_cfg() { return BN == 32 && WK == NW && BM == DEEP_BM; }
@@ -16,7 +19,7 @@
 template <typename T, int BN, int NW, int WK, int DK, int NC, int KSZ, int BM = DEEP_BM>
 int launch_deep_nc(const rnvp_conv_args* a, hipStream_t s, bool dry) {
     const long long M = (long long)a->B * a->H * a->W;
-    const size_t shm = deep_lds_bytes<T, BN, NW, WK, BM>(a->cs_in, a->W, a->ks, a->bp != 0);
+    const size_t shm = deep_lds_bytes<T, BN, NW, WK, BM>(a->cs_in, a->W, a->ks, a->bp != 0, a->ib != 0);
     if (shm > 160 * 1024) return RNVP_E_UNSUPPORTED;
     const long long gm = (M + BM - 1) / BM, gn = (a->n + BN - 1) / BN;
     const unsigned grid = (unsigned)(gm * gn);
@@ -24,6 +27,24 @@
     const dim3 blk(64 * NW);
     int xa, xb;
     xcd_blocks(a, (int)gm, (int)gn, BN, sizeof(T), &xa, &xb, BM);
+    if (a->ib) {
+        if constexpr (ib_cfg<BN, NW, WK, BM, KSZ>()) {
+            if (a->bp || a->pro_bn_relu || a->epi_relu_bn_bwd || a->out_sums) return RNVP_E_UNSUPPORTED;
+            if (dry) return RNVP_OK;
+            if constexpr (sizeof(T) == 2 && NC <= 4) {
+                if (a->w_frag) {
+                    k_conv_deep<T, BN, KSZ, false, NW, WK, DK, NC, true, BM, false, true><<<grid, blk, shm, s>>>(*a, sh, xa, xb);
+                    RNVP_LAUNCH_CHECK();
+                    return RNVP_OK;
+                }
+            }
+            k_conv_deep<T, BN, KSZ, false, NW, WK, DK, NC, false, BM, false, true><<<grid, blk, shm, s>>>(*a, sh, xa, xb);
+            RNVP_LAUNCH_CHECK();
+            return RNVP_OK;
+        } else {
+            return RNVP_E_UNSUPPORTED;
+        }
+    }
     if (a->bp) {
         if constexpr (bp_cfg<BN, NW, WK, BM>()) {
             if (dry) return RNVP_OK;
diff --git a/dl-normalizing-flows_amd/csrc/conv_in_bwd.h b/dl-normalizing-flows_amd/csrc/conv_in_bwd.h
--- /dev/null
+++ b/dl-normalizing-flows_amd/csrc/conv_in_bwd.h
@@ -0,0 +1,76 @@
+#pragma once
+#include "conv_common.h"
+#include "coupling_common.h"
+
+namespace {
+
+__device__ __forceinline__ int ib_cb(const rnvp_conv_args& a) { return a.ib_kind == 0 ? a.ib_C : a.ib_C / 2; }
+
+__device__ __forceinline__ int ib_chan(int n, int Cb) {
+    const int cb = n < Cb ? n : n - Cb;
+    return cb < Cb ? cb : 0;
+}
+
+struct IbPix {
+    int b, p, mk;
+};
+__device__ __forceinline__ IbPix ib_pix(const rnvp_conv_args& a, int m, int M) {
+    const int mm = m < M ? m : 0;
+    const int row = fdiv_small(mm, 1.0f / (float)a.W);
+    const int x = mm - row * a.W;
+    IbPix q;
+    q.b = fdiv_small(row, 1.0f / (float)a.H);
+    const int y = row - q.b * a.H;
+    q.p = y * a.W + x;
+    q.mk = ((a.ib_mask_config ? 1 : 0) + y + x) & 1;
+    return q;
+}
+
+__device__ __forceinline__ void ib_prefetch(const rnvp_conv_args& a, int m, int M, int n, float* xv) {
+    const int Cb = ib_cb(a), HW = a.H * a.W;
+    const IbPix q = ib_pix(a, m, M);
+    const int off = (a.ib_kind != 0 && a.ib_mask_config) ? Cb : 0;
+#pragma unroll
+    for (int r = 0; r < 4; ++r)
+        xv[r] = a.ib_x[((long long)q.b * a.ib_C + off + ib_chan(n + r, Cb)) * HW + q.p];
+}
+
+__device__ __forceinline__ floatx4 ib_tab_load(const rnvp_conv_args& a, int n) {
+    const int Cb = ib_cb(a), cb = ib_chan(n, Cb);
+    return floatx4{a.ib_tab[cb], a.ib_tab[Cb + cb], a.ib_tab[2 * Cb + cb], a.ib_tab[3 * Cb + cb]};
+}
+
+template <typename T>
+__device__ __forceinline__ void epi4p_ib(const rnvp_conv_args& a, long long o, const floatx4& acc, const float* bias,
+                                         const float* et, int pitch, double* s1, double* s2, double* e1, double* e2,
+                                         int n, int m, int M, const EpiPre& p) {
+    float v[4];
+    epi_vals(a, acc, bias, p, v);
+#pragma unroll
+    for (int r = 0; r < 4; ++r)
+        if (n + r >= a.n) v[r] = 0.f;
+    st4((T*)a.y + o, v);
+    const int Cb = ib_cb(a);
+    const IbPix q = ib_pix(a, m, M);
+    const bool kept = a.ib_kind != 0 || q.mk;
+#pragma unroll
+    for (int r = 0; r < 4; ++r) {
+        float g = v[r];
+        if constexpr (sizeof(T) == 2) g = bf2f(f2bf(g));
+        const float xv = p.x[r];
+        float xa, xh;
+        in_bn_xa(kept ? xv : 0.f, et[r], et[pitch + r], et[2 * pitch + r], et[3 * pitch + r], xa, xh);
+        float term = n + r < Cb ? crelu_pos(xa, g) : 0.f - crelu_neg(xa, g);
+        if (n + r >= 2 * Cb) term = 0.f;
+        s1[r] += (double)term;
+        s2[r] += (double)term * xh;
+        if (a.ib_kind == 0) e1[r] += kept ? (double)term : 0.0;
+        e2[r] += kept ? (double)term * xv : 0.0;
+    }
+}
+
+__device__ __forceinline__ double* ib_shard(double* sums, int vb, int Cb) {
+    return sums + (long long)(vb % RNVP_COUPLING_SHARDS) * 2 * Cb;
+}
+
+}
diff --git a/dl-normalizing-flows_amd/csrc/coupling.hip b/dl-normalizing-flows_amd/csrc/coupling.hip
--- a/dl-normalizing-flows_amd/csrc/coupling.hip
+++ b/dl-normalizing-flows_amd/csrc/coupling.hip
@@ -547,35 +547,6 @@
     }
 }
 
-__device__ __forceinline__ void fold_gscale(const rnvp_coupling_args& a) {
-    const int l = threadIdx.x;
-    double v0 = 0.0, v1 = 0.0;
-    if (l < RNVP_COUPLING_SHARDS) {
-        v0 = a.gscale_part[2 * l];
-        v1 = a.gscale_part[2 * l + 1];
-        a.gscale_part[2 * l] = 0.0;
-        a.gscale_part[2 * l + 1] = 0.0;
-    }
-    v0 = wave_sum(v0);
-    v1 = wave_sum(v1);
-    if (l == 0) {
-        *a.g_scale += (float)v0;
-        *a.g_scale_shift += (float)v1;
-    }
-}
-
-template <typename T>
-__device__ __forceinline__ void in_bwd_vals(const rnvp_coupling_args& a, const Geo& g, const Tile& t, const T* gh,
-                                            const float* tab, int cb, int pl, float v, float& gxa, float& xh) {
-    const int p = t.p0 + pl;
-    if (g.kind == 0 && !ckbd_m(g, p)) v = 0.f;
-    const float xa = v * tab[cb] + tab[g.Cb + cb];
-    const float g1 = ldv(&gh[pl * a.cs_gh0 + cb]);
-    const float g2 = ldv(&gh[pl * a.cs_gh0 + g.Cb + cb]);
-    gxa = (xa > 0.f ? g1 : 0.f) - (xa < 0.f ? g2 : 0.f);
-    xh = (v - tab[2 * g.Cb + cb]) * tab[3 * g.Cb + cb];
-}
-
 template <typename T>
 __global__ __launch_bounds__(256) void k_in_bwd_red(rnvp_coupling_args a, int TP, int seg) {
     extern __shared__ double dsm[];
@@ -605,7 +576,7 @@
     } else {
         in_bn_table(a, g, tab);
     }
-    if (blockIdx.x == 0 && a.gscale_part && threadIdx.x < 64) fold_gscale(a);
+    if (blockIdx.x == 0 && a.gscale_part && threadIdx.x < 64) fold_gscale(a, threadIdx.x);
     __syncthreads();
     auto body = [&](int e0, float xv) {
         const int e = e0 + threadIdx.x;
@@ -679,7 +650,7 @@
             if (a.g_in_gamma) a.g_in_gamma[cb] = (float)s2;
         }
     }
-    if (blockIdx.x == 0 && a.gscale_part && threadIdx.x < 64) fold_gscale(a);
+    if (blockIdx.x == 0 && a.gscale_part && threadIdx.x < 64) fold_gscale(a, threadIdx.x);
     tile_copy_in<T>(a.gh0, t.m0, t.tp, a.cs_gh0, gh);
     __syncthreads();
     auto body = [&](int e, float xv, float gxv) {
@@ -858,10 +829,11 @@
     return RNVP_OK;
 }
 
-extern "C" int rnvp_coupling_in_bwd(const rnvp_coupling_args* a, void* stream) {
+namespace {
+int in_bwd(const rnvp_coupling_args* a, void* stream, bool red) {
     int st = check(a);
     if (st) return st;
-    if (!a->gh0 || (!a->gx && !(a->in_bwd_ext && a->training))) return RNVP_E_INVALID;
+    if (!a->gh0 || (!a->gx && !(a->in_bwd_ext && a->training && red))) return RNVP_E_INVALID;
     if (a->training && (!a->in_sums || !a->in_bwd_sums)) return RNVP_E_INVALID;
     if (!a->training && (!a->in_rmean || !a->in_rvar)) return RNVP_E_INVALID;
     const int Cb = cb_of(a);
@@ -871,7 +843,7 @@
     const TileCfg tc = tile_cfg(a);
     const int esz = a->dtype == RNVP_F32 ? 4 : 2;
     const size_t gsh = (size_t)tc.TP * a->cs_gh0 * esz;
-    if (a->training || a->g_in_gamma || a->g_in_beta) {
+    if (red && (a->training || a->g_in_gamma || a->g_in_beta)) {
         if (!a->in_bwd_sums) return RNVP_E_INVALID;
         const size_t shm = (a->in_bwd_ext ? 32 : 16) * Cb + 16 * r4(Cb) + gsh;
         if (a->dtype == RNVP_F32) k_in_bwd_red<float><<<tc.grid, 256, shm, s>>>(*a, tc.TP, tc.seg);
@@ -885,3 +857,11 @@
     RNVP_LAUNCH_CHECK();
     return RNVP_OK;
 }
+}
+
+extern "C" int rnvp_coupling_in_bwd(const rnvp_coupling_args* a, void* stream) { return in_bwd(a, stream, true); }
+
+extern "C" int rnvp_coupling_in_bwd_apply(const rnvp_coupling_args* a, void* stream) {
+    if (!a || !a->gx || !a->in_bwd_sums) return RNVP_E_INVALID;
+    return in_bwd(a, stream, false);
+}
diff --git a/dl-normalizing-flows_amd/csrc/coupling_common.h b/dl-normalizing-flows_amd/csrc/coupling_common.h
--- a/dl-normalizing-flows_amd/csrc/coupling_common.h
+++ b/dl-normalizing-flows_amd/csrc/coupling_common.h
@@ -141,6 +141,41 @@
     }
 }
 
+__device__ __forceinline__ void in_bn_xa(float v, float sc, float sf, float mean, float rstd, float& xa, float& xh) {
+    xa = v * sc + sf;
+    xh = (v - mean) * rstd;
+}
+__device__ __forceinline__ float crelu_pos(float xa, float g1) { return xa > 0.f ? g1 : 0.f; }
+__device__ __forceinline__ float crelu_neg(float xa, float g2) { return xa < 0.f ? g2 : 0.f; }
+
+template <typename T>
+__device__ __forceinline__ void in_bwd_vals(const rnvp_coupling_args& a, const Geo& g, const Tile& t, const T* gh,
+                                            const float* tab, int cb, int pl, float v, float& gxa, float& xh) {
+    const int p = t.p0 + pl;
+    if (g.kind == 0 && !ckbd_m(g, p)) v = 0.f;
+    float xa;
+    in_bn_xa(v, tab[cb], tab[g.Cb + cb], tab[2 * g.Cb + cb], tab[3 * g.Cb + cb], xa, xh);
+    const float g1 = ldv(&gh[pl * a.cs_gh0 + cb]);
+    const float g2 = ldv(&gh[pl * a.cs_gh0 + g.Cb + cb]);
+    gxa = crelu_pos(xa, g1) - crelu_neg(xa, g2);
+}
+
+__device__ __forceinline__ void fold_gscale(const rnvp_coupling_args& a, int l) {
+    double v0 = 0.0, v1 = 0.0;
+    if (l < RNVP_COUPLING_SHARDS) {
+        v0 = a.gscale_part[2 * l];
+        v1 = a.gscale_part[2 * l + 1];
+        a.gscale_part[2 * l] = 0.0;
+        a.gscale_part[2 * l + 1] = 0.0;
+    }
+    v0 = wave_sum(v0);
+    v1 = wave_sum(v1);
+    if (l == 0) {
+        *a.g_scale += (float)v0;
+        *a.g_scale_shift += (float)v1;
+    }
+}
+
 __device__ __forceinline__ float coupling_u(float x, float sh, float r, float sc, float ss, float& lr, float& th,
                                             float& ex) {
     th = tanhf(r);
diff --git a/dl-normalizing-flows_amd/csrc/coupling_link.hip b/dl-normalizing-flows_amd/csrc/coupling_link.hip
--- a/dl-normalizing-flows_amd/csrc/coupling_link.hip
+++ b/dl-normalizing-flows_amd/csrc/coupling_link.hip
@@ -544,6 +544,7 @@
         s = wave_sum(s);
         if (tid == 0) gls_sh = s;
     }
+    if (TO_N && blockIdx.x == 0 && tid < 64 && n.gscale_part && n.g_scale && n.g_scale_shift) fold_gscale(n, tid);
     lds_zero(red, 4 * ga.C);
     for (int e = tid; e < t.tp * a.cs_gst; e += blockDim.x) stv(&gs[e], 0.f);
     __syncthreads();
diff --git a/dl-normalizing-flows_amd/csrc/flow_ops.hip b/dl-normalizing-flows_amd/csrc/flow_ops.hip
--- a/dl-normalizing-flows_amd/csrc/flow_ops.hip
+++ b/dl-normalizing-flows_amd/csrc/flow_ops.hip
@@ -2,7 +2,7 @@
 
 #include "coupling_common.h"
 
-extern "C" int rnvp_version(void) { return 112; }
+extern "C" int rnvp_version(void) { return 113; }
 
 extern "C" int rnvp_struct_size(int which) {
     switch (which) {
diff --git a/dl-normalizing-flows_amd/realnvp_hip/_lib.py b/dl-normalizing-flows_amd/realnvp_hip/_lib.py
--- a/dl-normalizing-flows_amd/realnvp_hip/_lib.py
+++ b/dl-normalizing-flows_amd/realnvp_hip/_lib.py
@@ -41,7 +41,9 @@
                 ("epi_relu_bn_bwd", i32), ("epi_x", vp), ("epi", BNSrc), ("epi_sums", vp),
                 ("ws", vp), ("ws_elems", i64), ("variant", i32), ("w_frag", vp),
                 ("bp", i32), ("bp_x", vp), ("bp_bn", BNSrc), ("bp_sums", vp), ("bp_shards", i32),
-                ("bp_out", vp), ("bp_dgamma", vp), ("bp_dbeta", vp)]
+                ("bp_out", vp), ("bp_dgamma", vp), ("bp_dbeta", vp),
+                ("ib", i32), ("ib_kind", i32), ("ib_C", i32), ("ib_mask_config", i32),
+                ("ib_x", vp), ("ib_tab", vp), ("ib_sums", vp), ("ib_ext", vp)]
 
 
 class BNBwdArgs(C.Structure):
@@ -203,6 +205,7 @@
     "rnvp_coupling_reverse_bwd": (i32, [C.POINTER(CouplingArgs), vp]),
     "rnvp_coupling_out_bwd": (i32, [C.POINTER(CouplingArgs), vp]),
     "rnvp_coupling_in_bwd": (i32, [C.POINTER(CouplingArgs), vp]),
+    "rnvp_coupling_in_bwd_apply": (i32, [C.POINTER(CouplingArgs), vp]),
     "rnvp_link_nclass": (i32, [i32, i32]),
     "rnvp_coupling_out_u": (i32, [C.POINTER(CouplingArgs), vp]),
     "rnvp_coupling_link_fwd": (i32, [C.POINTER(CouplingArgs), C.POINTER(CouplingArgs), C.POINTER(LinkArgs), vp]),
diff --git a/dl-normalizing-flows_amd/realnvp_hip/engine.py b/dl-normalizing-flows_amd/realnvp_hip/engine.py
--- a/dl-normalizing-flows_amd/realnvp_hip/engine.py
+++ b/dl-normalizing-flows_amd/realnvp_hip/engine.py
@@ -19,6 +19,7 @@
 FOLD_BN = True
 BN_TABLES = True
 WGRAD_MULTI = True
+COUPLING_EPILOGUE = True
 
 
 def stream_ptr():
@@ -586,7 +587,7 @@
         return out, ldj
 
 
-    def _net_backward(self, sv, sc, ws, T, training, gp, s):
+    def _net_backward(self, sv, sc, ws, T, training, gp, s, ib=None):
         L = _lib.lib()
         x = sv["x"]
         dt = DTYPES[sv["dtype"]][0]
@@ -612,9 +613,25 @@
                 steps.append(st)
             plan = plan + (plan_launches(steps, x.device, [it[5] for it in items]),)
             sv["bwd_plan"] = plan
+        host = None
+        if plan[2] and plan[2][-1][0] == "single" and items[plan[2][-1][1]][0] == "dgrad":
+            host = items[plan[2][-1][1]][1]
+            host.ib = 0
+            if ib is not None and host.y == sc["arena"].ptr("g:h0"):
+                host.ib, host.ib_kind, host.ib_C, host.ib_mask_config = 1, ib.kind, ib.C, ib.mask_config
+                host.ib_x, host.ib_tab, host.ib_sums, host.ib_ext = ib.x, ib.in_tab, ib.in_bwd_sums, ib.in_bwd_ext
+                ok = sv.get("ib_ok")
+                if ok is None or ok[0] != key:
+                    ok = (key, L.conv2d_check(C.byref(host)) == 0)
+                    sv["ib_ok"] = ok
+                if not ok[1]:
+                    host.ib = 0
+        folded = host is not None and host.ib == 1
         for g in plan[2]:
             if g[0] == "single":
                 kind, c, nb, fl, bn, _ = items[g[1]]
+                if c is host and folded:
+                    nb += 4 * x.numel()
                 if kind == "dgrad":
                     if bn is not None:
                         c.bp_dgamma, c.bp_dbeta = gp(bn + "weight"), gp(bn + "bias")
@@ -627,6 +644,7 @@
                 nb = sum(items[i][2] for i in range(i0, i1))
                 fl = sum(items[i][3] for i in range(i0, i1))
                 _launch("conv_dgrad", nb, fl, L.net_group, C.addressof(tab), i1 - i0, dt, klass, grid, lds, s)
+        return folded
 
     def _wgrad_multi_ok(self, sv, sc, groups, multi):
         if not WGRAD_MULTI or sv["dtype"] != "bf16" or any(it[4] == id(sc) for it in multi):
@@ -933,10 +951,14 @@
             _launch("coupling", nb, 0.0, L.coupling_link_bwd, C.byref(a), C.byref(n), C.byref(link["args"]), s)
         else:
             _launch("coupling", nb, 0.0, L.coupling_link_bwd, C.byref(a), None, C.byref(link["args"]), s)
-        self._net_backward(sv, sc, ws, T, True, gp, s)
-        if not first:
-            a.gx = None
+        folded = self._net_backward(sv, sc, ws, T, True, gp, s, a if COUPLING_EPILOGUE else None)
         cs_h0 = chan_stride(self.P.buf_ch["h0"])
-        _launch("coupling", (8 if first else 4) * n_el + (2 if first else 1) * esz * B * H * W * cs_h0, 0.0,
-                L.coupling_in_bwd, C.byref(a), s)
+        if folded:
+            if first:
+                _launch("coupling", 8 * n_el + esz * B * H * W * cs_h0, 0.0, L.coupling_in_bwd_apply, C.byref(a), s)
+        else:
+            if not first:
+                a.gx = None
+            _launch("coupling", (8 if first else 4) * n_el + (2 if first else 1) * esz * B * H * W * cs_h0, 0.0,
+                    L.coupling_in_bwd, C.byref(a), s)
         self._issue_weight_grads(self._weight_grads(sv, sc, ws, True, opt, after, gbase, multi), defer, None)
diff --git a/include/realnvp_hip.h b/include/realnvp_hip.h
--- a/include/realnvp_hip.h
+++ b/include/realnvp_hip.h
@@ -73,6 +73,8 @@
     const void* w_frag;
     int bp; const void* bp_x; rnvp_bn_src bp_bn; const double* bp_sums; int bp_shards;
     void* bp_out; float* bp_dgamma; float* bp_dbeta;
+    int ib; int ib_kind; int ib_C; int ib_mask_config;
+    const float* ib_x; const float* ib_tab; double* ib_sums; double* ib_ext;
 } rnvp_conv_args;
 int rnvp_conv2d(const rnvp_conv_args* a, void* stream);
 int rnvp_conv2d_check(const rnvp_conv_args* a);
@@ -220,6 +222,7 @@
 int rnvp_coupling_reverse_bwd(const rnvp_coupling_args* a, void* stream);
 int rnvp_coupling_out_bwd(const rnvp_coupling_args* a, void* stream);
 int rnvp_coupling_in_bwd(const rnvp_coupling_args* a, void* stream);
+int rnvp_coupling_in_bwd_apply(const rnvp_coupling_args* a, void* stream);
 
 enum { RNVP_LINK_SAME = 0, RNVP_LINK_SQUEEZE = 1, RNVP_LINK_UNFACTOR = 2, RNVP_LINK_FINAL = 3 };
 typedef struct rnvp_link_args {
```

Result: no change. 3486 images/sec (median of 6 runs) (+0.3%).
